# acg-team/ProGraphMSA

Hardware: AMD Instinct MI355X
Metric: DP cell-updates/sec (GCUPS) + wall-clock on 256 seqs × 1000 aa, WAG (higher is better)
Workload: dtype f32

## Files before the change

### include/pgm_hip.h

```cpp
#ifndef PGM_HIP_H_
#define PGM_HIP_H_

#include <stdint.h>
#include <stddef.h>

#ifdef __cplusplus
extern "C" {
#endif

#define PGM_OK 0
#define PGM_ERR_INVALID 1
#define PGM_ERR_DEVICE 2
#define PGM_ERR_BACKTRACK 3
#define PGM_ERR_NOMEM 4

#define PGM_GAP 0xFFFFFFFFu


typedef struct pgm_graph {
    uint32_t n;
    uint32_t dim;
    const double *sites;
    const int32_t *e_rowptr;
    const uint32_t *e_col;
    const float *e_val;
    const int32_t *r_rowptr;
    const uint32_t *r_col;
    const uint32_t *r_units;
} pgm_graph;

typedef struct pgm_model {
    const double *M;
    const double *pi;
} pgm_model;

typedef struct pgm_scores {
    float gap_init, gap_extend, match_init, end_match, end_gap, end_skip;
    float start_gap, start_init, repeat_init, repeat_ext;
} pgm_scores;

typedef struct pgm_align_out {
    float score;
    uint32_t n_tr_indels;
    uint32_t len;
    int32_t status;
    uint32_t *map1;
    uint32_t *map2;
} pgm_align_out;

typedef struct pgm_ctx pgm_ctx;
typedef struct pgm_align_batch pgm_align_batch;

int pgm_device_count(void);
int pgm_ctx_create(int device, pgm_ctx **out);
void pgm_ctx_destroy(pgm_ctx *ctx);
const char *pgm_last_error(void);
int pgm_ctx_device_info(pgm_ctx *ctx, char *name, size_t name_len, int *cu_count);

int pgm_align_graphs_batch(pgm_ctx *ctx, uint32_t njobs, const pgm_graph *const *g1,
                           const pgm_graph *const *g2, const pgm_model *const *model,
                           const pgm_scores *scores, pgm_align_out *out);

int pgm_align_batch_create(pgm_ctx *ctx, uint32_t njobs, const pgm_graph *const *g1,
                           const pgm_graph *const *g2, const pgm_model *const *model,
                           const pgm_scores *scores, pgm_align_batch **out);
#define PGM_BATCH_KEEP_MATRICES 1u
int pgm_align_batch_create_ex(pgm_ctx *ctx, uint32_t njobs, const pgm_graph *const *g1,
                              const pgm_graph *const *g2, const pgm_model *const *model,
                              const pgm_scores *scores, uint32_t flags, pgm_align_batch **out);
typedef struct pgm_site_ref {
    const double *dev_sites;
    const uint32_t *node_map;
    uint32_t ncols;
} pgm_site_ref;
int pgm_align_batch_create_res(pgm_ctx *ctx, uint32_t njobs, const pgm_graph *const *g1,
                               const pgm_graph *const *g2, const pgm_model *const *model,
                               const pgm_scores *scores, uint32_t flags, const pgm_site_ref *res1,
                               const pgm_site_ref *res2, pgm_align_batch **out);
int pgm_align_graphs_batch_res(pgm_ctx *ctx, uint32_t njobs, const pgm_graph *const *g1,
                               const pgm_graph *const *g2, const pgm_model *const *model,
                               const pgm_scores *scores, const pgm_site_ref *res1,
                               const pgm_site_ref *res2, pgm_align_out *out);
int pgm_align_batch_run(pgm_ctx *ctx, pgm_align_batch *b);
int pgm_align_batch_fetch(pgm_ctx *ctx, pgm_align_batch *b, pgm_align_out *out);
void pgm_align_batch_destroy(pgm_ctx *ctx, pgm_align_batch *b);
uint64_t pgm_align_batch_cells(const pgm_align_batch *b);
int pgm_align_batch_time(pgm_ctx *ctx, pgm_align_batch *b, int reps, float *ms_prep,
                         float *ms_emission, float *ms_fill, float *ms_traceback);
int pgm_align_batch_stage_times(pgm_align_batch *b, int reset, float *ms_prep, float *ms_emission, float *ms_fill,
                                uint32_t *launches);
int pgm_align_batch_job_times(pgm_ctx *ctx, pgm_align_batch *b, uint64_t *ticks);
int pgm_align_batch_test_stall(pgm_align_batch *b, uint32_t job, uint32_t band, uint32_t spin_limit);
int pgm_test_cu_shares(uint32_t cus, double lean_cost, uint32_t nlean, double band_cost, uint32_t nbands, double rest_cost,
                       uint32_t nrest, uint32_t ncrit, double longest_chain, uint32_t *out4);
#define PGM_PLAN_HEAD 23
#define PGM_PLAN_DHEAD 9
#define PGM_PLAN_JOB 19
int pgm_test_batch_plan(uint32_t njobs, const pgm_graph *const *g1, const pgm_graph *const *g2, const pgm_model *const *model,
                        const pgm_scores *scores, uint32_t flags, const pgm_site_ref *res1, const pgm_site_ref *res2, uint32_t cus,
                        uint32_t *head, double *dhead, uint32_t *job_fields, uint32_t *items, uint32_t *bands, uint32_t *lean_list, int32_t *tblist);
int pgm_align_batch_read_matrices(pgm_ctx *ctx, pgm_align_batch *b, uint32_t job, float *M,
                                  float *X, float *Y, float *W, float *S);

int pgm_nw_pairs_batch(pgm_ctx *ctx, uint32_t dim, const int32_t *score, int32_t gap_open,
                       int32_t gap_extend, uint32_t nseq, const int8_t *syms,
                       const uint32_t *offs, uint32_t npairs, const uint32_t *pi,
                       const uint32_t *pj, int32_t *counts, uint32_t *gaps);
#define PGM_NW_REDUCED 1u
int pgm_nw_pairs_submit(pgm_ctx *ctx, uint32_t dim, const int32_t *score, int32_t gap_open,
                        int32_t gap_extend, uint32_t nseq, const int8_t *syms,
                        const uint32_t *offs, uint32_t npairs, const uint32_t *pi,
                        const uint32_t *pj, uint32_t flags, int32_t *counts, uint32_t *gaps, int *ticket);
int pgm_nw_pairs_wait(pgm_ctx *ctx, int ticket);
float pgm_nw_last_kernel_ms(pgm_ctx *ctx);
void *pgm_host_alloc(size_t bytes);
void pgm_host_free(void *p);

int pgm_csprofile_load(pgm_ctx *ctx, uint32_t K, uint32_t ncols, const double *lprofiles,
                       const double *centre, const double *priors);
int pgm_csprofile_create_batch(pgm_ctx *ctx, uint32_t nseq, const int8_t *syms,
                               const uint32_t *offs, const double *tau, const double *pi,
                               const double *p_uniform, double *out, const uint64_t *out_offs);
int pgm_csprofile_create_batch_res(pgm_ctx *ctx, uint32_t nseq, const int8_t *syms,
                                   const uint32_t *offs, const double *tau, const double *pi,
                                   const double *p_uniform, const double **dev);
float pgm_csprofile_last_kernel_ms(pgm_ctx *ctx);

typedef struct pgm_mldist_model {
    uint32_t dim;
    const double *Q, *V, *Vi, *sigma;
    double dist_max, var_max, var_min, cutoff_dist, min_dist, max_dist, indel_rate;
    int32_t mldist, mldist_gap;
} pgm_mldist_model;
int pgm_mldist_batch(pgm_ctx *ctx, const pgm_mldist_model *model, uint32_t npairs, const int32_t *counts,
                     const uint32_t *gaps, const double *seqlen, double *dist, double *var);

int pgm_prealigned_counts_batch(pgm_ctx *ctx, uint32_t dim, uint32_t nrows, uint32_t ncols, const int8_t *rows,
                                uint32_t npairs, const uint32_t *pi, const uint32_t *pj, int32_t *counts,
                                uint32_t *gaps);
int pgm_kmer_cosine(pgm_ctx *ctx, uint32_t nseq, uint32_t ncols, const int32_t *counts, double *cosine);
int pgm_kmer_cosine_multi(pgm_ctx *ctx, uint32_t nfam, const uint32_t *nseq, uint32_t ncols, const int32_t *counts, double *cosine);
int pgm_prealigned_counts_multi(pgm_ctx *ctx, uint32_t dim, uint32_t nfam, const uint32_t *nrows, const uint32_t *ncols,
                                const int8_t *rows, uint32_t npairs, const uint32_t *fam, const uint32_t *pi, const uint32_t *pj,
                                int32_t *counts, uint32_t *gaps);
int pgm_prealigned_counts_resampled(pgm_ctx *ctx, uint32_t dim, uint32_t nrows, uint32_t ncols, const int8_t *rows, uint32_t nrep,
                                    const uint32_t *cols, uint32_t npairs, const uint32_t *pi, const uint32_t *pj, int32_t *counts,
                                    uint32_t *gaps);
float pgm_dist_last_kernel_ms(pgm_ctx *ctx);

typedef struct pgm_merge_job {
    uint32_t dim, n1, n2, nnodes;
    const double *sites1, *sites2;
    const double *P1, *P2;
    const uint32_t *k1, *k2;
    const uint8_t *g2_with_P1;
    double *profiles;
} pgm_merge_job;
int pgm_merge_profiles_batch(pgm_ctx *ctx, uint32_t njobs, const pgm_merge_job *jobs);
#define PGM_MERGE_RESIDENT 1u
int pgm_merge_profiles_batch_ex(pgm_ctx *ctx, uint32_t njobs, const pgm_merge_job *jobs, uint32_t flags,
                                const double **dev_profiles);
int pgm_resident_reset(pgm_ctx *ctx);
int pgm_resident_onehot(pgm_ctx *ctx, uint32_t dim, uint32_t nseq, const int8_t *syms, const uint32_t *offs,
                        const double **dev);
int pgm_resident_import(pgm_ctx *ctx, pgm_ctx *src_ctx, const double *src, uint64_t count, const double **dst);
float pgm_merge_last_kernel_ms(pgm_ctx *ctx);


typedef struct pgm_gapmask_job {
    const uint64_t *src;
    const uint32_t *mapping;
    uint64_t *dst;
    uint32_t nrows, ncols_in, ncols_out;
} pgm_gapmask_job;
int pgm_gapmask_extend_batch(pgm_ctx *ctx, uint32_t njobs, const pgm_gapmask_job *jobs);

typedef struct pgm_parsimony_job {
    const uint64_t *masks;
    const uint32_t *children;
    uint32_t nleaves, ncols;
} pgm_parsimony_job;
int pgm_gap_parsimony_batch(pgm_ctx *ctx, uint32_t njobs, const pgm_parsimony_job *jobs, uint32_t *scores);
float pgm_parsimony_last_kernel_ms(pgm_ctx *ctx);

#define PGM_WLS_MAX_N 32768
int pgm_wls_load(pgm_ctx *ctx, uint32_t n, const double *D, const double *W);

#define PGM_WLS_OUT 20
typedef struct pgm_wls_job {
    const int8_t *label;
    const double *offset;
    uint32_t nsub;
} pgm_wls_job;
int pgm_wls_pair_sums_batch(pgm_ctx *ctx, uint32_t njobs, const pgm_wls_job *jobs, double *out);
float pgm_wls_last_kernel_ms(pgm_ctx *ctx);
uint32_t pgm_wls_last_launches(pgm_ctx *ctx);

typedef struct pgm_bionj_join { uint32_t index1, index2; double dist1, dist2; } pgm_bionj_join;
#define PGM_BIONJ_MAX_N 32768
int pgm_bionj(pgm_ctx *ctx, uint32_t n, const double *D, const double *V, pgm_bionj_join *joins, double *final_d);
int pgm_bionj_multi(pgm_ctx *ctx, uint32_t nfam, const uint32_t *n, const double *D, const double *V,
                    pgm_bionj_join *joins, double *final_d);
uint32_t pgm_bionj_last_launches(pgm_ctx *ctx);
float pgm_bionj_last_kernel_ms(pgm_ctx *ctx);

typedef struct pgm_bionj_pair { uint32_t index1, index2; } pgm_bionj_pair;
int pgm_bionj_plan(pgm_ctx *ctx, uint32_t n, const double *D, const double *V, const pgm_bionj_pair *plan,
                   pgm_bionj_join *joins, double *final_d);
int pgm_bionj_plan_multi(pgm_ctx *ctx, uint32_t nfam, const uint32_t *n, const double *D, const double *V,
                         const pgm_bionj_pair *plan, pgm_bionj_join *joins, double *final_d);

int pgm_msa_agreement(pgm_ctx *ctx, uint32_t nrows, uint32_t ncols, uint32_t nrep, const int32_t *where,
                      uint32_t *res_hits , uint32_t *pair_hits );
float pgm_agreement_last_kernel_ms(pgm_ctx *ctx);

int pgm_transfer_min(pgm_ctx *ctx, uint32_t nleaves, uint32_t nref, const uint64_t *ref ,
                     uint32_t nrep, const uint32_t *rep_off ,
                     const uint64_t *rep , uint32_t *phi );
float pgm_transfer_last_kernel_ms(pgm_ctx *ctx);

#define PGM_TRANSFER_NONE 0xffffffffu
int pgm_transfer_taxa(pgm_ctx *ctx, uint32_t nleaves, uint32_t nref, const uint64_t *ref , const uint32_t *thr ,
                      uint32_t nrep, const uint32_t *rep_off , const uint64_t *rep ,
                      uint32_t *phi , uint32_t *arg , uint32_t *moved ,
                      uint32_t *counted );

#define PGM_TREELIK_CHUNK 16
int pgm_tree_likelihood(pgm_ctx *ctx, uint32_t dim, uint32_t nleaves, uint32_t nnodes, const uint32_t *parent ,
                        uint32_t ncols, const int8_t *rows , const double *pi ,
                        const double *P , int derivs,
                        double *site_l , int32_t *site_k , double *d1, double *d2 );
float pgm_treelik_last_kernel_ms(pgm_ctx *ctx);

#define PGM_TREELIK_MAXCAT 16
int pgm_tree_likelihood_rates(pgm_ctx *ctx, uint32_t dim, uint32_t nleaves, uint32_t nnodes, const uint32_t *parent, uint32_t ncols, const int8_t *rows,
                              const double *pi, uint32_t ncat, const double *w , const double *P ,
                              int derivs, double *site_l , int32_t *site_k , double *post ,
                              double *d1, double *d2 );

int pgm_tree_ancestral(pgm_ctx *ctx, uint32_t dim, uint32_t nleaves, uint32_t nnodes, const uint32_t *parent, uint32_t ncols, const int8_t *rows,
                       const double *pi, uint32_t ncat, const double *w , const double *P ,
                       double *site_l , int32_t *site_k , double *post ,
                       int8_t *anc_state , double *anc_prob ,
                       double *anc_post );
// ... 38 lines not shown
```

### prographmsa_amd/__init__.py

```python
import ctypes as C
import os

_HERE = os.path.dirname(os.path.abspath(__file__))
LIB_PATH = os.path.join(_HERE, "lib", "libpgm_hip.so")
PGMSA_PATH = os.path.join(_HERE, "bin", "pgmsa")

PGM_OK, PGM_ERR_INVALID, PGM_ERR_DEVICE, PGM_ERR_BACKTRACK, PGM_ERR_NOMEM = 0, 1, 2, 3, 4
PGM_GAP = 0xFFFFFFFF
PGM_BATCH_KEEP_MATRICES = 1
PGM_NW_REDUCED = 1
PGM_MERGE_RESIDENT = 1


class pgm_graph(C.Structure):
    _fields_ = [("n", C.c_uint32), ("dim", C.c_uint32), ("sites", C.POINTER(C.c_double)),
                ("e_rowptr", C.POINTER(C.c_int32)), ("e_col", C.POINTER(C.c_uint32)), ("e_val", C.POINTER(C.c_float)),
                ("r_rowptr", C.POINTER(C.c_int32)), ("r_col", C.POINTER(C.c_uint32)), ("r_units", C.POINTER(C.c_uint32))]


class pgm_model(C.Structure):
    _fields_ = [("M", C.POINTER(C.c_double)), ("pi", C.POINTER(C.c_double))]


class pgm_scores(C.Structure):
    _fields_ = [(n, C.c_float) for n in ("gap_init", "gap_extend", "match_init", "end_match", "end_gap", "end_skip",
                                         "start_gap", "start_init", "repeat_init", "repeat_ext")]


class pgm_mldist_model(C.Structure):
    _fields_ = [("dim", C.c_uint32), ("Q", C.POINTER(C.c_double)), ("V", C.POINTER(C.c_double)), ("Vi", C.POINTER(C.c_double)),
                ("sigma", C.POINTER(C.c_double))] + [(n, C.c_double) for n in ("dist_max", "var_max", "var_min", "cutoff_dist", "min_dist", "max_dist", "indel_rate")] \
        + [("mldist", C.c_int32), ("mldist_gap", C.c_int32)]


class pgm_merge_job(C.Structure):
    _fields_ = [("dim", C.c_uint32), ("n1", C.c_uint32), ("n2", C.c_uint32), ("nnodes", C.c_uint32),
                ("sites1", C.POINTER(C.c_double)), ("sites2", C.POINTER(C.c_double)), ("P1", C.POINTER(C.c_double)), ("P2", C.POINTER(C.c_double)),
                ("k1", C.POINTER(C.c_uint32)), ("k2", C.POINTER(C.c_uint32)), ("g2_with_P1", C.POINTER(C.c_uint8)), ("profiles", C.POINTER(C.c_double))]


class pgm_site_ref(C.Structure):
    _fields_ = [("dev_sites", C.POINTER(C.c_double)), ("node_map", C.POINTER(C.c_uint32)), ("ncols", C.c_uint32)]


class pgm_gapmask_job(C.Structure):
    _fields_ = [("src", C.POINTER(C.c_uint64)), ("mapping", C.POINTER(C.c_uint32)), ("dst", C.POINTER(C.c_uint64)),
                ("nrows", C.c_uint32), ("ncols_in", C.c_uint32), ("ncols_out", C.c_uint32)]


class pgm_parsimony_job(C.Structure):
    _fields_ = [("masks", C.POINTER(C.c_uint64)), ("children", C.POINTER(C.c_uint32)), ("nleaves", C.c_uint32), ("ncols", C.c_uint32)]


class pgm_wls_job(C.Structure):
    _fields_ = [("label", C.POINTER(C.c_int8)), ("offset", C.POINTER(C.c_double)), ("nsub", C.c_uint32)]


class pgm_bionj_join(C.Structure):
    _fields_ = [("index1", C.c_uint32), ("index2", C.c_uint32), ("dist1", C.c_double), ("dist2", C.c_double)]


class pgm_bionj_pair(C.Structure):
    _fields_ = [("index1", C.c_uint32), ("index2", C.c_uint32)]


class pgm_align_out(C.Structure):
    _fields_ = [("score", C.c_float), ("n_tr_indels", C.c_uint32), ("len", C.c_uint32), ("status", C.c_int32),
                ("map1", C.POINTER(C.c_uint32)), ("map2", C.POINTER(C.c_uint32))]


EXPORTS = [
    "pgm_device_count", "pgm_ctx_create", "pgm_ctx_destroy", "pgm_last_error", "pgm_ctx_device_info",
    "pgm_align_graphs_batch", "pgm_align_batch_create", "pgm_align_batch_create_ex", "pgm_align_batch_create_res", "pgm_align_graphs_batch_res", "pgm_align_batch_run", "pgm_align_batch_fetch",
    "pgm_align_batch_destroy", "pgm_align_batch_cells", "pgm_align_batch_test_stall", "pgm_test_cu_shares", "pgm_test_batch_plan", "pgm_align_batch_stage_times", "pgm_align_batch_job_times", "pgm_align_batch_time", "pgm_align_batch_read_matrices",
    "pgm_nw_pairs_batch", "pgm_nw_pairs_submit", "pgm_nw_pairs_wait", "pgm_nw_last_kernel_ms", "pgm_host_alloc", "pgm_host_free", "pgm_csprofile_load", "pgm_csprofile_create_batch", "pgm_csprofile_create_batch_res",
    "pgm_csprofile_last_kernel_ms", "pgm_mldist_batch", "pgm_prealigned_counts_batch", "pgm_kmer_cosine", "pgm_dist_last_kernel_ms",
    "pgm_kmer_cosine_multi", "pgm_prealigned_counts_multi", "pgm_prealigned_counts_resampled",
    "pgm_merge_profiles_batch", "pgm_merge_profiles_batch_ex", "pgm_resident_reset", "pgm_resident_onehot", "pgm_resident_import", "pgm_merge_last_kernel_ms",
    "pgm_gapmask_extend_batch", "pgm_gap_parsimony_batch", "pgm_parsimony_last_kernel_ms",
    "pgm_wls_load", "pgm_wls_pair_sums_batch", "pgm_wls_last_kernel_ms", "pgm_wls_last_launches",
    "pgm_bionj", "pgm_bionj_multi", "pgm_bionj_last_launches", "pgm_bionj_last_kernel_ms",
    "pgm_bionj_plan", "pgm_bionj_plan_multi",
    "pgm_msa_agreement", "pgm_agreement_last_kernel_ms",
    "pgm_transfer_min", "pgm_transfer_last_kernel_ms", "pgm_transfer_taxa",
    "pgm_tree_likelihood", "pgm_treelik_last_kernel_ms", "pgm_tree_likelihood_rates", "pgm_tree_ancestral", "pgm_tree_nni", "pgm_tree_nni_edge", "pgm_tree_spr",
    "pgm_tree_ancestral_joint", "pgm_tree_ancestral_sample",
    "pgm_resampled_sums", "pgm_resample_last_kernel_ms",
]


def _load():
    if not os.path.exists(LIB_PATH):
        raise ImportError("libpgm_hip.so is not built (%s); run `python -c 'import __graft_entry__ as g; g.build()'` "
                          "— there is no CPU fallback for the hot path" % LIB_PATH)
    lib = C.CDLL(LIB_PATH)
    vp, u32, i32 = C.c_void_p, C.c_uint32, C.c_int32
    PG, PM = C.POINTER(C.POINTER(pgm_graph)), C.POINTER(C.POINTER(pgm_model))
    sig = {
        "pgm_device_count": (C.c_int, []),
        "pgm_ctx_create": (C.c_int, [C.c_int, C.POINTER(vp)]),
        "pgm_ctx_destroy": (None, [vp]),
        "pgm_last_error": (C.c_char_p, []),
        "pgm_ctx_device_info": (C.c_int, [vp, C.c_char_p, C.c_size_t, C.POINTER(C.c_int)]),
        "pgm_align_graphs_batch": (C.c_int, [vp, u32, PG, PG, PM, C.POINTER(pgm_scores), C.POINTER(pgm_align_out)]),
        "pgm_align_batch_create": (C.c_int, [vp, u32, PG, PG, PM, C.POINTER(pgm_scores), C.POINTER(vp)]),
        "pgm_align_batch_create_ex": (C.c_int, [vp, u32, PG, PG, PM, C.POINTER(pgm_scores), u32, C.POINTER(vp)]),
        "pgm_align_batch_create_res": (C.c_int, [vp, u32, PG, PG, PM, C.POINTER(pgm_scores), u32, C.POINTER(pgm_site_ref), C.POINTER(pgm_site_ref), C.POINTER(vp)]),
        "pgm_align_graphs_batch_res": (C.c_int, [vp, u32, PG, PG, PM, C.POINTER(pgm_scores), C.POINTER(pgm_site_ref), C.POINTER(pgm_site_ref), C.POINTER(pgm_align_out)]),
        "pgm_align_batch_run": (C.c_int, [vp, vp]),
        "pgm_align_batch_fetch": (C.c_int, [vp, vp, C.POINTER(pgm_align_out)]),
        "pgm_align_batch_destroy": (None, [vp, vp]),
        "pgm_align_batch_cells": (C.c_uint64, [vp]),
        "pgm_align_batch_test_stall": (C.c_int, [vp, u32, u32, u32]),
        "pgm_test_cu_shares": (C.c_int, [u32, C.c_double, u32, C.c_double, u32, C.c_double, u32, u32, C.c_double, C.POINTER(C.c_uint32)]),
        "pgm_test_batch_plan": (C.c_int, [u32, PG, PG, PM, C.POINTER(pgm_scores), u32, C.POINTER(pgm_site_ref), C.POINTER(pgm_site_ref), u32,
                                          C.POINTER(u32), C.POINTER(C.c_double)] + [C.POINTER(u32)] * 4 + [C.POINTER(i32)]),
        "pgm_align_batch_stage_times": (C.c_int, [vp, C.c_int] + [C.POINTER(C.c_float)] * 3 + [C.POINTER(u32)]),
        "pgm_align_batch_job_times": (C.c_int, [vp, vp, C.POINTER(C.c_uint64)]),
        "pgm_align_batch_time": (C.c_int, [vp, vp, C.c_int] + [C.POINTER(C.c_float)] * 4),
        "pgm_align_batch_read_matrices": (C.c_int, [vp, vp, u32] + [C.POINTER(C.c_float)] * 5),
        "pgm_nw_pairs_batch": (C.c_int, [vp, u32, C.POINTER(i32), i32, i32, u32, C.POINTER(C.c_int8), C.POINTER(u32), u32,
                                         C.POINTER(u32), C.POINTER(u32), C.POINTER(i32), C.POINTER(u32)]),
        "pgm_nw_pairs_submit": (C.c_int, [vp, u32, C.POINTER(i32), i32, i32, u32, C.POINTER(C.c_int8), C.POINTER(u32), u32,
                                          C.POINTER(u32), C.POINTER(u32), u32, C.POINTER(i32), C.POINTER(u32), C.POINTER(C.c_int)]),
        "pgm_nw_pairs_wait": (C.c_int, [vp, C.c_int]),
        "pgm_host_alloc": (vp, [C.c_size_t]),
        "pgm_host_free": (None, [vp]),
        "pgm_nw_last_kernel_ms": (C.c_float, [vp]),
        "pgm_csprofile_load": (C.c_int, [vp, u32, u32] + [C.POINTER(C.c_double)] * 3),
        "pgm_csprofile_create_batch": (C.c_int, [vp, u32, C.POINTER(C.c_int8), C.POINTER(u32)] + [C.POINTER(C.c_double)] * 4
                                       + [C.POINTER(C.c_uint64)]),
        "pgm_csprofile_create_batch_res": (C.c_int, [vp, u32, C.POINTER(C.c_int8), C.POINTER(u32)] + [C.POINTER(C.c_double)] * 3
                                           + [C.POINTER(C.POINTER(C.c_double))]),
        "pgm_csprofile_last_kernel_ms": (C.c_float, [vp]),
        "pgm_mldist_batch": (C.c_int, [vp, C.POINTER(pgm_mldist_model), u32, C.POINTER(i32), C.POINTER(u32)] + [C.POINTER(C.c_double)] * 3),
        "pgm_prealigned_counts_batch": (C.c_int, [vp, u32, u32, u32, C.POINTER(C.c_int8), u32, C.POINTER(u32), C.POINTER(u32), C.POINTER(i32), C.POINTER(u32)]),
        "pgm_kmer_cosine": (C.c_int, [vp, u32, u32, C.POINTER(i32), C.POINTER(C.c_double)]),
        "pgm_dist_last_kernel_ms": (C.c_float, [vp]),
        "pgm_kmer_cosine_multi": (C.c_int, [vp, u32, C.POINTER(u32), u32, C.POINTER(i32), C.POINTER(C.c_double)]),
        "pgm_prealigned_counts_multi": (C.c_int, [vp, u32, u32, C.POINTER(u32), C.POINTER(u32), C.POINTER(C.c_int8), u32, C.POINTER(u32), C.POINTER(u32),
                                                  C.POINTER(u32), C.POINTER(i32), C.POINTER(u32)]),
        "pgm_prealigned_counts_resampled": (C.c_int, [vp, u32, u32, u32, C.POINTER(C.c_int8), u32, C.POINTER(u32), u32, C.POINTER(u32), C.POINTER(u32),
                                                      C.POINTER(i32), C.POINTER(u32)]),
        "pgm_merge_profiles_batch": (C.c_int, [vp, u32, C.POINTER(pgm_merge_job)]),
        "pgm_merge_profiles_batch_ex": (C.c_int, [vp, u32, C.POINTER(pgm_merge_job), u32, C.POINTER(C.POINTER(C.c_double))]),
        "pgm_resident_reset": (C.c_int, [vp]),
        "pgm_resident_onehot": (C.c_int, [vp, u32, u32, C.POINTER(C.c_int8), C.POINTER(u32), C.POINTER(C.POINTER(C.c_double))]),
        "pgm_resident_import": (C.c_int, [vp, vp, C.POINTER(C.c_double), C.c_uint64, C.POINTER(C.POINTER(C.c_double))]),
        "pgm_merge_last_kernel_ms": (C.c_float, [vp]),
        "pgm_gapmask_extend_batch": (C.c_int, [vp, u32, C.POINTER(pgm_gapmask_job)]),
        "pgm_gap_parsimony_batch": (C.c_int, [vp, u32, C.POINTER(pgm_parsimony_job), C.POINTER(u32)]),
        "pgm_parsimony_last_kernel_ms": (C.c_float, [vp]),
        "pgm_wls_load": (C.c_int, [vp, u32, C.POINTER(C.c_double), C.POINTER(C.c_double)]),
        "pgm_wls_pair_sums_batch": (C.c_int, [vp, u32, C.POINTER(pgm_wls_job), C.POINTER(C.c_double)]),
        "pgm_wls_last_kernel_ms": (C.c_float, [vp]),
        "pgm_wls_last_launches": (C.c_uint32, [vp]),
        "pgm_bionj": (C.c_int, [vp, u32, C.POINTER(C.c_double), C.POINTER(C.c_double), C.POINTER(pgm_bionj_join), C.POINTER(C.c_double)]),
        "pgm_bionj_multi": (C.c_int, [vp, u32, C.POINTER(u32), C.POINTER(C.c_double), C.POINTER(C.c_double), C.POINTER(pgm_bionj_join), C.POINTER(C.c_double)]),
        "pgm_bionj_last_launches": (C.c_uint32, [vp]),
        "pgm_bionj_last_kernel_ms": (C.c_float, [vp]),
        "pgm_bionj_plan": (C.c_int, [vp, u32, C.POINTER(C.c_double), C.POINTER(C.c_double), C.POINTER(pgm_bionj_pair), C.POINTER(pgm_bionj_join), C.POINTER(C.c_double)]),
        "pgm_bionj_plan_multi": (C.c_int, [vp, u32, C.POINTER(u32), C.POINTER(C.c_double), C.POINTER(C.c_double), C.POINTER(pgm_bionj_pair), C.POINTER(pgm_bionj_join), C.POINTER(C.c_double)]),
        "pgm_msa_agreement": (C.c_int, [vp, u32, u32, u32, C.POINTER(i32), C.POINTER(u32), C.POINTER(u32)]),
        "pgm_agreement_last_kernel_ms": (C.c_float, [vp]),
        "pgm_transfer_min": (C.c_int, [vp, u32, u32, C.POINTER(C.c_uint64), u32, C.POINTER(u32), C.POINTER(C.c_uint64), C.POINTER(u32)]),
        "pgm_transfer_last_kernel_ms": (C.c_float, [vp]),
        "pgm_transfer_taxa": (C.c_int, [vp, u32, u32, C.POINTER(C.c_uint64), C.POINTER(u32), u32, C.POINTER(u32), C.POINTER(C.c_uint64),
                                        C.POINTER(u32), C.POINTER(u32), C.POINTER(u32), C.POINTER(u32)]),
        "pgm_tree_likelihood": (C.c_int, [vp, u32, u32, u32, C.POINTER(u32), u32, C.POINTER(C.c_int8), C.POINTER(C.c_double), C.POINTER(C.c_double), C.c_int,
                                          C.POINTER(C.c_double), C.POINTER(i32), C.POINTER(C.c_double), C.POINTER(C.c_double)]),
        "pgm_treelik_last_kernel_ms": (C.c_float, [vp]),
        "pgm_tree_likelihood_rates": (C.c_int, [vp, u32, u32, u32, C.POINTER(u32), u32, C.POINTER(C.c_int8), C.POINTER(C.c_double), u32, C.POINTER(C.c_double),
                                                C.POINTER(C.c_double), C.c_int, C.POINTER(C.c_double), C.POINTER(i32), C.POINTER(C.c_double), C.POINTER(C.c_double),
                                                C.POINTER(C.c_double)]),
        "pgm_tree_ancestral": (C.c_int, [vp, u32, u32, u32, C.POINTER(u32), u32, C.POINTER(C.c_int8), C.POINTER(C.c_double), u32, C.POINTER(C.c_double),
                                         C.POINTER(C.c_double), C.POINTER(C.c_double), C.POINTER(i32), C.POINTER(C.c_double), C.POINTER(C.c_int8),
                                         C.POINTER(C.c_double), C.POINTER(C.c_double)]),
        "pgm_tree_nni": (C.c_int, [vp, u32, u32, u32, C.POINTER(u32), u32, C.POINTER(C.c_int8), C.POINTER(C.c_double), u32, C.POINTER(C.c_double),
                                   C.POINTER(C.c_double), u32, C.POINTER(u32), C.POINTER(u32), C.POINTER(u32), C.POINTER(C.c_double), C.POINTER(i32),
                                   C.POINTER(C.c_double), C.POINTER(C.c_double)]),
        "pgm_tree_nni_edge": (C.c_int, [vp, u32, u32, u32, C.POINTER(u32), u32, C.POINTER(C.c_int8), C.POINTER(C.c_double), u32, C.POINTER(C.c_double),
                                        C.POINTER(C.c_double), u32, C.POINTER(u32), C.POINTER(u32), C.POINTER(u32), C.POINTER(C.c_double), C.POINTER(C.c_double),
                                        C.POINTER(i32), C.POINTER(C.c_double), C.POINTER(C.c_double), C.POINTER(C.c_double), C.POINTER(C.c_double)]),
        "pgm_tree_spr": (C.c_int, [vp, u32, u32, u32, C.POINTER(u32), u32, C.POINTER(C.c_int8), C.POINTER(C.c_double), u32, C.POINTER(C.c_double),
                                   C.POINTER(C.c_double), C.POINTER(C.c_double), u32, C.POINTER(u32), C.POINTER(u32), C.POINTER(C.c_double), C.POINTER(i32),
                                   C.POINTER(C.c_double), C.POINTER(C.c_double)]),
        "pgm_tree_ancestral_joint": (C.c_int, [vp, u32, u32, u32, C.POINTER(u32), u32, C.POINTER(C.c_int8), C.POINTER(C.c_double), u32, C.POINTER(C.c_double),
                                               C.POINTER(C.c_double), C.POINTER(C.c_double), C.POINTER(i32), C.POINTER(C.c_double), C.POINTER(C.c_uint8),
                                               C.POINTER(C.c_int8), C.POINTER(C.c_double), C.POINTER(i32)]),
        "pgm_tree_ancestral_sample": (C.c_int, [vp, u32, u32, u32, C.POINTER(u32), u32, C.POINTER(C.c_int8), C.POINTER(C.c_double), u32, C.POINTER(C.c_double),
                                                C.POINTER(C.c_double), u32, C.c_uint64, C.c_uint64, C.POINTER(C.c_double), C.POINTER(i32), C.POINTER(C.c_double),
                                                C.POINTER(C.c_uint8), C.POINTER(C.c_int8)]),
        "pgm_resampled_sums": (C.c_int, [vp, u32, u32, C.POINTER(C.c_double), u32, C.POINTER(u32), C.POINTER(C.c_double)]),
        "pgm_resample_last_kernel_ms": (C.c_float, [vp]),
    }
    for name, (res, args) in sig.items():
        fn = getattr(lib, name)
        fn.restype = res
        fn.argtypes = args
    return lib


lib = _load()


class PgmError(RuntimeError):
    pass


def check(rc, what="libpgm_hip"):
    if rc != PGM_OK:
        raise PgmError("%s failed (%d): %s" % (what, rc, lib.pgm_last_error().decode()))


class Context:

    def __init__(self, device=0):
        self.handle = C.c_void_p()
        check(lib.pgm_ctx_create(device, C.byref(self.handle)), "pgm_ctx_create")

    def device_info(self):
        buf = C.create_string_buffer(256)
        cu = C.c_int()
        check(lib.pgm_ctx_device_info(self.handle, buf, 256, C.byref(cu)))
        return buf.value.decode(), cu.value

    def prealigned_counts_resampled(self, dim, rows, cols, pi, pj):
        import numpy as np
        rows = np.ascontiguousarray(rows, np.int8)
        cols = np.ascontiguousarray(cols, np.uint32)
        pi = np.ascontiguousarray(pi, np.uint32)
        pj = np.ascontiguousarray(pj, np.uint32)
        nrep, npairs = cols.shape[0], len(pi)
        counts = np.zeros((nrep, npairs, dim * dim), np.int32)
        gaps = np.zeros((nrep, npairs), np.uint32)
        P = lambda a, t: a.ctypes.data_as(C.POINTER(t))
        check(lib.pgm_prealigned_counts_resampled(self.handle, dim, rows.shape[0], rows.shape[1], P(rows, C.c_int8), nrep, P(cols, C.c_uint32), npairs,
                                                  P(pi, C.c_uint32), P(pj, C.c_uint32), P(counts, C.c_int32), P(gaps, C.c_uint32)), "pgm_prealigned_counts_resampled")
        return counts, gaps

    def msa_agreement(self, where, res_hits=None, pair_hits=None):
        import numpy as np
        where = np.ascontiguousarray(where, np.int32)
        nrep, nrows, ncols = where.shape
        if res_hits is None: res_hits = np.zeros((nrows, ncols), np.uint32)
        if pair_hits is None: pair_hits = np.zeros((nrows, nrows), np.uint32)
        for o, shape in ((res_hits, (nrows, ncols)), (pair_hits, (nrows, nrows))):
            if o.dtype != np.uint32 or o.shape != shape or not o.flags.c_contiguous: raise ValueError("msa_agreement: output array of the wrong kind")
        P = lambda a, t: a.ctypes.data_as(C.POINTER(t))
        check(lib.pgm_msa_agreement(self.handle, nrows, ncols, nrep, P(where, C.c_int32), P(res_hits, C.c_uint32), P(pair_hits, C.c_uint32)), "pgm_msa_agreement")
        return res_hits, pair_hits

    def transfer_min(self, nleaves, ref, rep_off, rep, phi=None):
        import numpy as np
        words = (nleaves + 63) // 64
        ref = np.ascontiguousarray(ref, np.uint64)
        rep_off = np.ascontiguousarray(rep_off, np.uint32)
        rep = np.ascontiguousarray(rep, np.uint64).reshape(-1, words)
        if ref.ndim != 2 or ref.shape[1] != words or rep_off.ndim != 1 or len(rep_off) < 1 or rep.shape[0] != int(rep_off[-1]):
            raise ValueError("transfer_min: input array of the wrong shape")
        nref, nrep = ref.shape[0], len(rep_off) - 1
        if phi is None: phi = np.zeros((nref, nrep), np.uint32)
        if phi.dtype != np.uint32 or phi.shape != (nref, nrep) or not phi.flags.c_contiguous: raise ValueError("transfer_min: output array of the wrong kind")
        P = lambda a, t: a.ctypes.data_as(C.POINTER(t))
        check(lib.pgm_transfer_min(self.handle, nleaves, nref, P(ref, C.c_uint64), nrep, P(rep_off, C.c_uint32), P(rep, C.c_uint64) if rep.size else None,
                                   P(phi, C.c_uint32)), "pgm_transfer_min")
        return phi

    def transfer_taxa(self, nleaves, ref, thr, rep_off, rep, out=None):
        import numpy as np
        words = (nleaves + 63) // 64
# ... 219 lines not shown
```

### prographmsa_amd/csrc/pgm_align_kernels.h

```cpp
#ifndef PGM_ALIGN_KERNELS_H_
#define PGM_ALIGN_KERNELS_H_

#include <hip/hip_runtime.h>
#include <math.h>
#include <type_traits>
#include "pgm_device.h"

#define PGM_NEG_INF (-INFINITY)

__device__ __forceinline__ float pgm_ls_log_add(float x, float add) {
    const float a = 2.44247459618085927548717403238913328776812604856113966238617812902399112761292613763080658235564f;
    const float b = -4.2040783745848554315883301529007786406310628696382695994938550046831869207082846248658671f;
    const float c = -0.72123729809042963774358701619456664388406302428056983119308906451199556380646306f;
    const uint32_t bits = __float_as_uint(x);
    const float e = (float)((int32_t)(bits >> 23) - 126);
    const float d = __uint_as_float(((bits << 9) >> 9) ^ 0x3f000000u);
    float t = __fdiv_rn(b, __fsub_rn(d, c));
    const float u = __fadd_rn(e, a);
    t = __fadd_rn(t, add);
    t = __fadd_rn(t, u);
    return t;
}

__device__ __forceinline__ float pgm_emission_finish(float num, float ay, float bx, float match_init) {
// ... 248 lines not shown
    }
    for (int i = threadIdx.x; i < COLS; i += 4 * PGM_ROWS) {
        const int col = cbase + i;
        bq[i] = (col >= 0 && col <= (int)J.ncol) ? J.b2[col] : 0.f;
    }
    __syncthreads();
    const uint32_t b0 = (4u * blockIdx.y + threadIdx.x / PGM_ROWS) * RB;
    const int l = PGM_HALO + (int)(threadIdx.x % PGM_ROWS);
    if (b0 >= nvb) return;
    float gy[RB][DP], ay[RB];
#pragma unroll
    for (int r = 0; r < RB; ++r) {
        const uint32_t y = row_of(b0 + (uint32_t)r, (uint32_t)(l - PGM_HALO));
        const uint32_t yc = (y + 1 < J.n1) ? y : 0u;
        const float4 *src = (const float4 *)(J.g1f + (size_t)DP * yc);
#pragma unroll
        for (int q = 0; q < NT; ++q) {
            const float4 v = src[q];
            gy[r][4 * q] = v.x; gy[r][4 * q + 1] = v.y; gy[r][4 * q + 2] = v.z; gy[r][4 * q + 3] = v.w;
        }
        ay[r] = J.a1[yc];
    }
    const float mi = J.sc.match_init;
    const uint32_t nblk = J.nblk;
    PGM_GLOBAL pgm_v4f *const Sq = (PGM_GLOBAL pgm_v4f *)(uintptr_t)J.S;
#pragma unroll 1
    for (int w = 0; w < PGM_EM_TB; ++w) {
        const uint32_t tb = tb0 + w;
        if (tb >= nblk) break;
        float out[RB][PGM_BLOCK];
#pragma unroll
        for (int i = 0; i < PGM_BLOCK; i += 2) {
            const int ci = (int)(tb * PGM_BLOCK) + i - l - cbase;
            const pgm_v2f *tc = tp + ci * STR;
            pgm_v2f acc[RB];
#pragma unroll
            for (int r = 0; r < RB; ++r) acc[r] = pgm_v2f{0.0f, 0.0f};
#pragma unroll
            for (int k = 0; k < DP; ++k) {
                const pgm_v2f tk = tc[k];
#pragma unroll
                for (int r = 0; r < RB; ++r) {
                    const pgm_v2f g = {gy[r][k], gy[r][k]};
                    acc[r] = acc[r] + g * tk;
                }
            }
#pragma unroll
            for (int r = 0; r < RB; ++r) {
                out[r][i] = pgm_emission_finish(acc[r].x, ay[r], bq[ci], mi);
                out[r][i + 1] = pgm_emission_finish(acc[r].y, ay[r], bq[ci + 1], mi);
            }
        }
#pragma unroll
        for (int r = 0; r < RB; ++r) {
            if (b0 + (uint32_t)r < nvb) {
                PGM_GLOBAL pgm_v4f *dst = Sq + (sblock_of(b0 + (uint32_t)r, tb) * 64u + (uint32_t)l) * (PGM_BLOCK / 4);
#pragma unroll
                for (int q = 0; q < PGM_BLOCK / 4; ++q) dst[q] = pgm_v4f{out[r][4 * q], out[r][4 * q + 1], out[r][4 * q + 2], out[r][4 * q + 3]};
            }
        }
    }
}

__device__ __forceinline__ int pgm_wave_max8(uint32_t v) {
    int m = __builtin_amdgcn_ballot_w64(v >= 8u) != 0 ? 8 : 0;
    m += __builtin_amdgcn_ballot_w64(v >= (uint32_t)(m + 4)) != 0 ? 4 : 0;
    m += __builtin_amdgcn_ballot_w64(v >= (uint32_t)(m + 2)) != 0 ? 2 : 0;
    m += __builtin_amdgcn_ballot_w64(v >= (uint32_t)(m + 1)) != 0 ? 1 : 0;
    return m;
}

__device__ __forceinline__ __amdgpu_buffer_rsrc_t pgm_band_rsrc(float4 *base, uint32_t bytes) {
    const uint64_t p = (uint64_t)base;
    const uint32_t lo = __builtin_amdgcn_readfirstlane((uint32_t)p), hi = __builtin_amdgcn_readfirstlane((uint32_t)(p >> 32));
    return __builtin_amdgcn_make_buffer_rsrc((void *)(((uint64_t)hi << 32) | lo), 0, __builtin_amdgcn_readfirstlane(bytes), 0x00020000);
}
__device__ __forceinline__ void pgm_store_cell_masked(__amdgpu_buffer_rsrc_t rsrc, uint32_t t, int lane, bool on, float Mv, float Xv, float Wv, float Yv) {
    typedef uint32_t pgm_v4u __attribute__((ext_vector_type(4)));
    pgm_v4u v;
    v.x = __float_as_uint(Mv); v.y = __float_as_uint(Xv); v.z = __float_as_uint(Wv); v.w = __float_as_uint(Yv);
    __builtin_amdgcn_raw_buffer_store_b128(v, rsrc, (on ? (uint32_t)lane * 16u : 0x80000000u) + t * 1024u, 0, 16);
}
__device__ __forceinline__ float4 pgm_gload4(const float4 *p) {
    const pgm_v4f v = *(const PGM_GLOBAL pgm_v4f *)(uintptr_t)p;
    return make_float4(v.x, v.y, v.z, v.w);
}
__device__ __forceinline__ float2 pgm_gload_cell_wy(const float4 *p) {
    const unsigned long long v = __hip_atomic_load((const PGM_GLOBAL unsigned long long *)(uintptr_t)p + 1, __ATOMIC_RELAXED, __HIP_MEMORY_SCOPE_AGENT);
    return make_float2(__uint_as_float((uint32_t)v), __uint_as_float((uint32_t)(v >> 32)));
}
__device__ __forceinline__ float2 pgm_load_cell_mx(const float4 *p) {
    const unsigned long long v = __hip_atomic_load((const PGM_GLOBAL unsigned long long *)(uintptr_t)p, __ATOMIC_RELAXED, __HIP_MEMORY_SCOPE_AGENT);
    return make_float2(__uint_as_float((uint32_t)v), __uint_as_float((uint32_t)(v >> 32)));
}
__device__ __forceinline__ float2 pgm_load_cell_wy(const float4 *p) {
    const unsigned long long v = __hip_atomic_load((const PGM_GLOBAL unsigned long long *)(uintptr_t)p + 1, __ATOMIC_RELAXED, __HIP_MEMORY_SCOPE_AGENT);
    return make_float2(__uint_as_float((uint32_t)v), __uint_as_float((uint32_t)(v >> 32)));
}

struct PgmPred {
    const int32_t *pp; const uint32_t *pc; const float *pv; const uint32_t *pu;
};
__device__ __forceinline__ float pgm_mark_value(const PgmPred &P, int32_t e) {
    const uint32_t u = P.pu[e];
    if (u == 0) return P.pv[e];
    const uint32_t units = u & 0x7fffffffu;
    if (units == 0) return INFINITY;
    return __fadd_rn(INFINITY, __fmul_rn(INFINITY, (float)(units - 1)));
}

struct PgmMapOut {
    uint32_t *m1, *m2;
    uint32_t len, cap;
    __device__ __forceinline__ void push(uint32_t y, uint32_t x) {
        if (len < cap) { m1[len] = y; m2[len] = x; }
        ++len;
    }
};

__device__ static void pgm_mark_alternative_path(const PgmJob &J, uint32_t start, uint32_t end, const PgmPred &P, PgmMapOut &mo, bool first) {
    const uint32_t len = end - start + 1;
    float *score = J.mark_score;
    uint32_t *prev = J.mark_prev;
    for (uint32_t i = 0; i < len; ++i) { score[i] = PGM_NEG_INF; prev[i] = 0xFFFFFFFFu; }
    score[0] = 0.0f;
    for (uint32_t i = 1; i < len; ++i) {
        const uint32_t real_ix = i + start;
        for (int32_t e = P.pp[real_ix]; e < P.pp[real_ix + 1]; ++e) {
            const uint32_t p = P.pc[e];
            if (p >= start && p <= end) {
                const uint32_t i2 = p - start;
                const float cand = __fsub_rn(score[i2], pgm_mark_value(P, e));
                if (score[i] <= cand) { score[i] = cand; prev[i] = i2; }
            }
        }
    }
    if (score[len - 1] > PGM_NEG_INF) {
        uint32_t i = prev[len - 1];
        while (i != 0) {
            if (first) mo.push(i + start, 0xFFFFFFFFu); else mo.push(0xFFFFFFFFu, i + start);
            i = prev[i];
        }
    }
}

__device__ __forceinline__ float pgm_emission_at(const PgmJob &J, uint32_t y, uint32_t x) {
    const uint32_t b = y / PGM_ROWS, l = PGM_HALO + (y - b * PGM_ROWS), t = x + l;
    return J.S[(((size_t)b * J.nblk + (t / PGM_BLOCK)) * 64u + l) * PGM_BLOCK + (t % PGM_BLOCK)];
}

#define PGM_TB_T 32
#define PGM_TB_BAND 6
#define PGM_TB_LK 4
struct PgmTbLds {
    float4 cell[PGM_TB_T * PGM_TB_T];
    float S[PGM_TB_T * PGM_TB_T];
    uint32_t p_cnt[2 * PGM_TB_T];
    uint32_t p_c[2 * PGM_TB_T * PGM_TB_PK];
    float p_v[2 * PGM_TB_T * PGM_TB_PK];
    uint32_t p_u[2 * PGM_TB_T * PGM_TB_PK];
    uint16_t succ[3 * PGM_TB_T * PGM_TB_T];
    uint32_t ty0, tx0;
    uint32_t ay, ax;
    int req;
    uint32_t len;
    int nbig;
    uint16_t big[128];
    uint16_t gtab[PGM_LK_NR][PGM_LK_W * PGM_LK_TAB] __attribute__((aligned(16)));
    uint2 mbuf[64];
    uint32_t grow, gcnt;
    uint32_t gnext[PGM_LK_NR];
};

#define PGM_LK_HW (PGM_LK_T + PGM_LK_H)
struct PgmLkLds {
    float4 cell[PGM_LK_HW * PGM_LK_HW];
    float S[PGM_LK_T * PGM_LK_T];
    uint32_t p_cnt[2 * PGM_LK_T];
    uint32_t p_c[2 * PGM_LK_T * PGM_TB_PK];
    float p_v[2 * PGM_LK_T * PGM_TB_PK];
    uint32_t p_u[2 * PGM_LK_T * PGM_TB_PK];
    uint16_t tab[PGM_LK_TAB] __attribute__((aligned(16)));
    int nbig;
    uint16_t big[PGM_LK_T * PGM_LK_T];
};
__device__ __forceinline__ uint16_t pgm_lk_code(uint32_t st, uint32_t dy, uint32_t dx) { return (uint16_t)(0x8000u | (st << 12) | (dy << 6) | dx); }

struct PgmPredView {
    uint32_t cnt;
    bool lds;
    uint32_t base;
};

__device__ static void pgm_traceback_publish(const PgmJob &J, const uint32_t len, const int tid, const int nthreads) {
    for (uint32_t i = (uint32_t)tid; i < len; i += (uint32_t)nthreads) {
        const uint32_t j = len - 1 - i;
        J.hmap1[i] = J.map1[j];
        J.hmap2[i] = J.map2[j];
    }
    __threadfence_system();
    __syncthreads();
    if (tid == 0) {
        const PgmJob::Result r = *J.result;
        J.hresult->score = r.score; J.hresult->n_tr_indels = r.n_tr_indels; J.hresult->len = r.len;
        __threadfence_system();
        __hip_atomic_store(&J.hresult->status, r.status, __ATOMIC_RELEASE, __HIP_MEMORY_SCOPE_SYSTEM);
    }
}

__device__ __attribute__((noinline)) static void pgm_traceback_job(const PgmJob &J, PgmTbLds &T, const int tid, const int nthreads,
                                         int *lq, int *lq_ids, const uint32_t jid) {
    constexpr uint32_t TT = PGM_TB_T;
    const uint32_t n1 = J.n1, n2 = J.n2;

    const PgmPred P1 = {J.pp1, J.pc1, J.pv1, J.pu1};
    const PgmPred P2 = {J.pp2, J.pc2, J.pv2, J.pu2};

    const bool loader = tid >= 64;
    auto stage = [&]() {
        const uint32_t ty0 = T.ty0, tx0 = T.tx0;
        constexpr uint32_t NT = 64u * PGM_WAVES;
        constexpr int NC = (int)((TT * TT) / NT), NP = (int)((2 * TT * PGM_TB_PK) / NT);
        static_assert(NC * NT == TT * TT && NP * NT == 2 * TT * PGM_TB_PK, "tile staging: whole rounds of the workgroup");
        float4 cv[NC];
        float sv[NC];
        uint32_t cslot[NC];
#pragma unroll
        for (int u = 0; u < NC; ++u) {
            const uint32_t i = (uint32_t)tid + NT * u;
            const uint32_t half = TT * (TT + 1u) / 2u;
            const bool up = i < half;
            const uint32_t m = up ? i : TT * TT - 1u - i;
            uint32_t d = (uint32_t)((sqrtf(8.0f * (float)m + 1.0f) - 1.0f) * 0.5f);
            while (d * (d + 1u) / 2u > m) --d;
            while ((d + 1u) * (d + 2u) / 2u <= m) ++d;
            const uint32_t k = m - d * (d + 1u) / 2u;
            const uint32_t ly = up ? k : TT - 1u - k, lx = up ? d - k : TT - 1u - (d - k);
            cslot[u] = ly * TT + lx;
            const uint32_t yy = min(ty0 + ly, n1 - 2), xx = min(tx0 + lx, n2 - 2);
            cv[u] = J.cells[pgm_cell_index(J, yy, xx)];
            const uint32_t ys = min(ty0 + i / TT, n1 - 2), xs = min(tx0 + i % TT, n2 - 2);
            sv[u] = pgm_emission_at(J, ys, xs);
        }
        uint32_t cnt[NP], ec[NP], eu[NP];
        float ev[NP];
#pragma unroll
        for (int u = 0; u < NP; ++u) {
            const uint32_t i = (uint32_t)tid + NT * u, slot = i / PGM_TB_PK, k = i % PGM_TB_PK;
            const bool row = slot < TT;
            const uint32_t v = min(row ? ty0 + slot : tx0 + (slot - TT), (row ? n1 : n2) - 1);
            const PgmTbNode *r = (row ? J.tb1 : J.tb2) + v;
            cnt[u] = r->cnt; ec[u] = r->c[k]; ev[u] = r->v[k]; eu[u] = r->u[k];
        }
#pragma unroll
        for (int u = 0; u < NC; ++u) {
            const uint32_t i = (uint32_t)tid + NT * u;
            T.cell[cslot[u]] = cv[u];
            T.S[i] = sv[u];
        }
        for (uint32_t i = (uint32_t)tid; i < 3u * TT * TT / 2u; i += NT) ((uint32_t *)T.succ)[i] = 0u;
        if (tid == 0) T.nbig = 0;
#pragma unroll
        for (int u = 0; u < NP; ++u) {
            const uint32_t i = (uint32_t)tid + NT * u, slot = i / PGM_TB_PK, k = i % PGM_TB_PK;
            const bool row = slot < TT;
            const bool inr = (row ? ty0 + slot : tx0 + (slot - TT)) < (row ? n1 : n2);
            if (k == 0) T.p_cnt[slot] = inr ? cnt[u] : 0xFFFFFFFFu;
            T.p_c[i] = ec[u]; T.p_v[i] = ev[u]; T.p_u[i] = eu[u];
        }
    };
    const pgm_scores sc = J.sc;
    const int band = J.has_extras ? PGM_TB_BAND : PGM_TB_BAND / 2;
    auto links = [&]() {
        const uint32_t ty0 = T.ty0, tx0 = T.tx0;
        const int adiag = (int)(T.ay - ty0) - (int)(T.ax - tx0);
        const uint32_t NDIAG = 2u * (uint32_t)band + 1u;
        for (uint32_t task = (uint32_t)tid; task < 3u * NDIAG * TT; task += (uint32_t)nthreads) {
            const uint32_t lx = task % TT, st_task = task / (NDIAG * TT);
            const int lyi = (int)lx + adiag + (int)((task / TT) % NDIAG) - band;
            if (lyi < 0 || lyi >= (int)TT) continue;
            const uint32_t ly = (uint32_t)lyi, ci = ly * TT + lx, y = ty0 + ly, x = tx0 + lx;
            uint16_t lm = 0, lxs = 0, lys = 0;
            if (y + 1 < n1 && x + 1 < n2 && (y | x) != 0u) {
                const float4 c0 = T.cell[ci];
                const uint32_t cy = T.p_cnt[ly], cx = T.p_cnt[TT + lx];
                auto pick = [&](const float4 &c, uint32_t yp, uint32_t xp) -> uint16_t {
                    uint32_t st;
                    if ((yp | xp) == 0u) st = 0u;
                    else if (c.z == c.x) st = 0u;
                    else if (c.z == c.w) st = 2u;
                    else if (c.z == c.y) st = 1u;
                    else return (uint16_t)0;
                    return (uint16_t)(0x8000u | (st << 10) | ((yp - ty0) << 5) | (xp - tx0));
                };
                const int doff = (int)((task / TT) % NDIAG) - band;
                if (st_task == 0u && doff >= -1 && doff <= 1 && (cy > PGM_TB_LK || cx > PGM_TB_LK) && cy <= PGM_TB_PK && cx <= PGM_TB_PK && cy != 0u && cx != 0u && c0.x > PGM_NEG_INF) {
                    const int slot = __hip_atomic_fetch_add(&T.nbig, 1, __ATOMIC_RELAXED, __HIP_MEMORY_SCOPE_WORKGROUP);
                    if (slot < 128) T.big[slot] = (uint16_t)ci;
                }
                if (st_task == 0u && cy <= PGM_TB_LK && cx <= PGM_TB_LK && cy != 0u && cx != 0u && c0.x > PGM_NEG_INF) {
                    const float S = T.S[ci];
                    uint32_t yp[PGM_TB_LK], xp[PGM_TB_LK];
                    float yv[PGM_TB_LK], xv[PGM_TB_LK];
                    bool ok = true;
#pragma unroll
                    for (int k = 0; k < PGM_TB_LK; ++k) {
                        yp[k] = T.p_c[ly * PGM_TB_PK + k]; yv[k] = T.p_v[ly * PGM_TB_PK + k];
                        xp[k] = T.p_c[(TT + lx) * PGM_TB_PK + k]; xv[k] = T.p_v[(TT + lx) * PGM_TB_PK + k];
                        ok = ok && ((uint32_t)k >= cy || yp[k] >= ty0) && ((uint32_t)k >= cx || xp[k] >= tx0);
                    }
                    float wz[PGM_TB_LK][PGM_TB_LK];
#pragma unroll
                    for (int ky = 0; ky < PGM_TB_LK; ++ky)
#pragma unroll
                        for (int kx = 0; kx < PGM_TB_LK; ++kx)
                            wz[ky][kx] = T.cell[min((yp[ky] - ty0) * TT + (xp[kx] - tx0), TT * TT - 1u)].z;
                    float best = INFINITY;
                    uint32_t wy = 0, wx = 0, wky = 0, wkx = 0;
#pragma unroll
                    for (int ky = 0; ky < PGM_TB_LK; ++ky)
#pragma unroll
                        for (int kx = 0; kx < PGM_TB_LK; ++kx) {
                            const float d = fabsf(__fsub_rn(c0.x, __fsub_rn(__fsub_rn(__fadd_rn(wz[ky][kx], S), yv[ky]), xv[kx])));
                            if ((uint32_t)ky < cy && (uint32_t)kx < cx && best > d) { best = d; wy = yp[ky]; wx = xp[kx]; wky = ky; wkx = kx; }
                        }
                    bool rep_edge = false;
                    float4 wc = c0;
                    if (ok && best < INFINITY) {
                        rep_edge = (T.p_u[ly * PGM_TB_PK + wky] | T.p_u[(TT + lx) * PGM_TB_PK + wkx]) != 0u;
                        wc = T.cell[(wy - ty0) * TT + (wx - tx0)];
                    }
                    if (ok && best < INFINITY && !rep_edge) lm = pick(wc, wy, wx);
                }
                if (st_task == 2u && cy == 1u && c0.w > PGM_NEG_INF) {
                    float best = INFINITY;
                    bool ok = true, rep_edge = false, open = false;
                    uint32_t wy = 0;
                    float4 wc = c0;
                    for (uint32_t k = 0; k < cy; ++k) {
                        const uint32_t yp = T.p_c[ly * PGM_TB_PK + k];
                        if (yp < ty0) { ok = false; break; }
                        const float yv = T.p_v[ly * PGM_TB_PK + k];
                        const float4 c = T.cell[(yp - ty0) * TT + lx];
                        const bool ru = T.p_u[ly * PGM_TB_PK + k] != 0u;
                        float d = fabsf(__fsub_rn(c0.w, __fsub_rn(__fadd_rn(c.w, sc.gap_extend), yv)));
                        if (best > d) { best = d; wy = yp; wc = c; rep_edge = ru; open = false; }
                        d = fabsf(__fsub_rn(c0.w, __fsub_rn(__fadd_rn(c.z, sc.gap_init), yv)));
                        if (best > d) { best = d; wy = yp; wc = c; rep_edge = ru; open = true; }
                    }
                    if (ok && best < INFINITY && !rep_edge)
                        lys = open ? pick(wc, wy, x) : (uint16_t)(0x8000u | (2u << 10) | ((wy - ty0) << 5) | lx);
                }
                if (st_task == 1u && cx == 1u && c0.y > PGM_NEG_INF) {
                    float best = INFINITY;
                    bool ok = true, rep_edge = false, open = false;
                    uint32_t wx = 0;
                    float4 wc = c0;
                    for (uint32_t k = 0; k < cx; ++k) {
                        const uint32_t xp = T.p_c[(TT + lx) * PGM_TB_PK + k];
                        if (xp < tx0) { ok = false; break; }
                        const float xv = T.p_v[(TT + lx) * PGM_TB_PK + k];
                        const float4 c = T.cell[ly * TT + (xp - tx0)];
                        const bool ru = T.p_u[(TT + lx) * PGM_TB_PK + k] != 0u;
                        float d = fabsf(__fsub_rn(c0.y, __fsub_rn(__fadd_rn(c.y, sc.gap_extend), xv)));
                        if (best > d) { best = d; wx = xp; wc = c; rep_edge = ru; open = false; }
                        d = fabsf(__fsub_rn(c0.y, __fsub_rn(__fadd_rn(c.z, sc.gap_init), xv)));
                        if (best > d) { best = d; wx = xp; wc = c; rep_edge = ru; open = true; }
                    }
                    if (ok && best < INFINITY && !rep_edge)
                        lxs = open ? pick(wc, y, wx) : (uint16_t)(0x8000u | (1u << 10) | (ly << 5) | (wx - tx0));
                }
            }
            T.succ[st_task * (TT * TT) + ci] = st_task == 0u ? lm : (st_task == 1u ? lxs : lys);
        }
    };
    auto links_big = [&]() {
        const int wave = tid >> 6, lane_b = tid & 63, nwaves = nthreads >> 6;
        const uint32_t ty0 = T.ty0, tx0 = T.tx0;
        const int nbig = min(T.nbig, 128);
        for (int i = wave; i < nbig; i += nwaves) {
            const uint32_t ci = T.big[i], ly = ci / TT, lx = ci % TT;
            const uint32_t cy = T.p_cnt[ly], cx = T.p_cnt[TT + lx];
            const uint32_t ky = (uint32_t)lane_b >> 3, kx = (uint32_t)lane_b & 7u;
            const bool valid = ky < cy && kx < cx;
            const uint32_t yp = T.p_c[ly * PGM_TB_PK + ky], xp = T.p_c[(TT + lx) * PGM_TB_PK + kx];
            const float yv = T.p_v[ly * PGM_TB_PK + ky], xv = T.p_v[(TT + lx) * PGM_TB_PK + kx];
            const uint32_t rep = T.p_u[ly * PGM_TB_PK + ky] | T.p_u[(TT + lx) * PGM_TB_PK + kx];
            const bool inside = yp >= ty0 && xp >= tx0;
            if (__builtin_amdgcn_ballot_w64(valid && !inside) != 0ull) continue;
            const float4 c0 = T.cell[ci];
            const float S = T.S[ci];
            const float4 c = T.cell[(valid && inside) ? (yp - ty0) * TT + (xp - tx0) : ci];
            const float d = fabsf(__fsub_rn(c0.x, __fsub_rn(__fsub_rn(__fadd_rn(c.z, S), yv), xv)));
            const unsigned long long zero = __builtin_amdgcn_ballot_w64(valid && d == 0.0f);
            if (zero == 0ull) continue;
            const int win = __ffsll((long long)zero) - 1;
            if (lane_b == win && rep == 0u) {
                uint32_t st = 3u;
                if ((yp | xp) == 0u) st = 0u;
                else if (c.z == c.x) st = 0u;
                else if (c.z == c.w) st = 2u;
                else if (c.z == c.y) st = 1u;
                if (st != 3u) T.succ[ci] = (uint16_t)(0x8000u | (st << 10) | ((yp - ty0) << 5) | (xp - tx0));
            }
        }
    };
    const bool use_links = true;
    auto load_rows = [&]() {
        const uint32_t gy = T.grow, cnt = T.gcnt;
        constexpr uint32_t NW = PGM_LK_W * PGM_LK_TAB * 2u / 8u, NT = 64u * PGM_WAVES, PER = NW / NT;
        static_assert(NW % NT == 0u, "row table: whole rounds of the workgroup");
        unsigned long long v[PGM_LK_NR][PER];
#pragma unroll
        for (uint32_t r = 0; r < PGM_LK_NR; ++r) {
            const PGM_GLOBAL unsigned long long *src = (const PGM_GLOBAL unsigned long long *)(uintptr_t)(J.ltab + (size_t)(gy - min(r, cnt - 1u)) * (PGM_LK_W * PGM_LK_TAB));
#pragma unroll
            for (uint32_t q = 0; q < PER; ++q) v[r][q] = r < cnt ? __hip_atomic_load(src + (uint32_t)tid + NT * q, __ATOMIC_RELAXED, __HIP_MEMORY_SCOPE_AGENT) : 0ull;
        }
        uint32_t nx = 0u;
        const uint32_t k = (uint32_t)tid - 64u;
        if (k < PGM_LK_NR && gy >= cnt + k) nx = (uint32_t)__hip_atomic_load(J.lready + (gy - cnt - k), __ATOMIC_RELAXED, __HIP_MEMORY_SCOPE_AGENT) >= min(J.lcols, PGM_LK_W) ? 1u : 0u;
#pragma unroll
        for (uint32_t r = 0; r < PGM_LK_NR; ++r)
            if (r < cnt) {
#pragma unroll
                for (uint32_t q = 0; q < PER; ++q) ((unsigned long long *)T.gtab[(gy - r) % PGM_LK_NR])[(uint32_t)tid + NT * q] = v[r][q];
            }
        if (k < PGM_LK_NR) T.gnext[k] = nx;
    };
    if (tid == 0) {
        T.grow = 0xFFFFFFFFu; T.gcnt = 0u;
        if (J.lrows != 0u) __hip_atomic_store(J.lready + J.lrows + 1, (int)(J.lrows - 1u), __ATOMIC_RELAXED, __HIP_MEMORY_SCOPE_AGENT);
        T.ty0 = n1 - 2 >= TT - 1 ? n1 - 2 - (TT - 1) : 0u;
        T.tx0 = n2 - 2 >= TT - 1 ? n2 - 2 - (TT - 1) : 0u;
        T.ay = n1 - 2; T.ax = n2 - 2;
        T.req = 1;
        if (J.lrows != 0u && lq) {
            const int slot = __hip_atomic_fetch_add(lq, 1, __ATOMIC_RELAXED, __HIP_MEMORY_SCOPE_AGENT);
            __hip_atomic_store(lq_ids + slot, (int)(jid + 1u), __ATOMIC_RELEASE, __HIP_MEMORY_SCOPE_AGENT);
        }
    }
    __syncthreads();
    stage();
    __syncthreads();
    if (use_links) {
        links();
        __syncthreads();
        links_big();
        __syncthreads();
    }

    if (loader) {
        for (;;) {
            __syncthreads();
            if (T.req == 2) break;
            if (T.req == 3) { load_rows(); __syncthreads(); continue; }
            stage();
            __syncthreads();
            if (use_links) {
                links();
                __syncthreads();
                links_big();
                __syncthreads();
            }
        }
    } else {
        const int lane = tid;
        const pgm_scores s = J.sc;
        uint32_t ty0 = T.ty0, tx0 = T.tx0, ay = T.ay, ax = T.ax;
        int adiag = (int)(ay - ty0) - (int)(ax - tx0);
        auto in_tile = [&](uint32_t y, uint32_t x) { return (y - ty0) < TT && (x - tx0) < TT; };
        auto cell_at = [&](uint32_t y, uint32_t x) -> float4 {
            if (in_tile(y, x)) return T.cell[(y - ty0) * TT + (x - tx0)];
            return pgm_load_cell(J, y, x);
        };
        auto s_at = [&](uint32_t y, uint32_t x) -> float {
            if (in_tile(y, x)) return T.S[(y - ty0) * TT + (x - tx0)];
            return pgm_emission_at(J, y, x);
        };
        auto preds = [&](bool row, uint32_t v) -> PgmPredView {
            const uint32_t slot = row ? v - ty0 : (v - tx0) + TT;
            if ((row ? v - ty0 : v - tx0) < TT) {
                const uint32_t cnt = T.p_cnt[slot];
                if (cnt <= PGM_TB_PK) return PgmPredView{cnt, true, slot * PGM_TB_PK};
            }
            const PgmPred &P = row ? P1 : P2;
            const int32_t eb = P.pp[v];
            return PgmPredView{(uint32_t)(P.pp[v + 1] - eb), false, (uint32_t)eb};
        };
        auto pc_of = [&](bool row, const PgmPredView &V, uint32_t k) { return V.lds ? T.p_c[V.base + k] : (row ? P1 : P2).pc[V.base + k]; };
        auto pv_of = [&](bool row, const PgmPredView &V, uint32_t k) { return V.lds ? T.p_v[V.base + k] : (row ? P1 : P2).pv[V.base + k]; };
        auto pu_of = [&](bool row, const PgmPredView &V, uint32_t k) { return V.lds ? T.p_u[V.base + k] : (row ? P1 : P2).pu[V.base + k]; };

        int status = PGM_OK;
        uint32_t n_tr = 0;
        enum { State_m = 0, State_x = 1, State_y = 2 };
        int current_state = State_m;
        float current_score = PGM_NEG_INF, Wend = PGM_NEG_INF;
        uint32_t y = n1 - 1, x = n2 - 1;
        PgmMapOut mo = {J.map1, J.map2, 0u, n1 + n2};
        if (lane == 0) {
            const PgmPredView Ey = preds(true, n1 - 1), Ex = preds(false, n2 - 1);
            for (uint32_t ky = 0; ky < Ey.cnt; ++ky) {
                for (uint32_t kx = 0; kx < Ex.cnt; ++kx) {
                    const uint32_t yp = pc_of(true, Ey, ky), xp = pc_of(false, Ex, kx);
                    const float yv = pv_of(true, Ey, ky), xv = pv_of(false, Ex, kx);
                    if (xp == 0 && yp == 0) {
                        Wend = fmaxf(__fsub_rn(__fsub_rn(s.end_skip, yv), xv), Wend);
                    } else {
                        const float4 c = cell_at(yp, xp);
                        Wend = fmaxf(__fsub_rn(__fsub_rn(__fadd_rn(c.y, s.end_gap), yv), xv), Wend);
                        Wend = fmaxf(__fsub_rn(__fsub_rn(__fadd_rn(c.w, s.end_gap), yv), xv), Wend);
                        Wend = fmaxf(__fsub_rn(__fsub_rn(__fadd_rn(c.x, s.end_match), yv), xv), Wend);
                    }
                }
            }
            mo.push(n1 - 1, n2 - 1);
            bool tr_x = false, tr_y = false;
            float best = INFINITY;
            for (uint32_t ky = 0; ky < Ey.cnt; ++ky) {
                for (uint32_t kx = 0; kx < Ex.cnt; ++kx) {
                    const uint32_t yp = pc_of(true, Ey, ky), xp = pc_of(false, Ex, kx);
                    const float yv = pv_of(true, Ey, ky), xv = pv_of(false, Ex, kx);
                    const bool ry = pu_of(true, Ey, ky) != 0, rx = pu_of(false, Ex, kx) != 0;
                    const float4 c = cell_at(yp, xp);
                    float d = fabsf(__fsub_rn(Wend, __fsub_rn(__fsub_rn(__fadd_rn(c.x, s.end_match), yv), xv)));
                    if (best > d) { best = d; tr_x = rx; tr_y = ry; current_score = c.x; current_state = State_m; y = yp; x = xp; }
                    d = fabsf(__fsub_rn(Wend, __fsub_rn(__fsub_rn(__fadd_rn(c.w, s.end_gap), yv), xv)));
                    if (best > d) { best = d; tr_x = rx; tr_y = ry; current_score = c.w; current_state = State_y; y = yp; x = xp; }
                    d = fabsf(__fsub_rn(Wend, __fsub_rn(__fsub_rn(__fadd_rn(c.y, s.end_gap), yv), xv)));
                    if (best > d) { best = d; tr_x = rx; tr_y = ry; current_score = c.y; current_state = State_x; y = yp; x = xp; }
                    d = fabsf(__fsub_rn(Wend, __fsub_rn(__fsub_rn(s.end_skip, yv), xv)));
                    if (xp == 0 && yp == 0 && best > d) { best = d; tr_x = rx; tr_y = ry; y = yp; x = xp; }
                }
            }
            n_tr += (uint32_t)tr_x + (uint32_t)tr_y;
            if (tr_y) pgm_mark_alternative_path(J, y, n1 - 1, P1, mo, true);
            if (tr_x) pgm_mark_alternative_path(J, x, n2 - 1, P2, mo, false);
            if (x != 0 || y != 0) {
                if (current_state == State_m) mo.push(y, x);
                else if (current_state == State_x) mo.push(0xFFFFFFFFu, x);
                else mo.push(y, 0xFFFFFFFFu);
            }
        }
        y = __builtin_amdgcn_readfirstlane(y); x = __builtin_amdgcn_readfirstlane(x);
        current_state = __builtin_amdgcn_readfirstlane(current_state);
        current_score = __uint_as_float(__builtin_amdgcn_readfirstlane(__float_as_uint(current_score)));
        Wend = __uint_as_float(__builtin_amdgcn_readfirstlane(__float_as_uint(Wend)));
        n_tr = __builtin_amdgcn_readfirstlane(n_tr);
        mo.len = __builtin_amdgcn_readfirstlane(mo.len);

        auto rl_u = [](uint32_t v, int l) { return (uint32_t)__builtin_amdgcn_readlane((int)v, l); };
        auto rl_f = [](float v, int l) { return __uint_as_float((uint32_t)__builtin_amdgcn_readlane((int)__float_as_uint(v), l)); };
        uint32_t nbuf = 0;
        auto buf_flush = [&]() {
            if (nbuf != 0u) {
                if ((uint32_t)lane < nbuf && mo.len + (uint32_t)lane < mo.cap) { const uint2 v = T.mbuf[lane]; mo.m1[mo.len + (uint32_t)lane] = v.x; mo.m2[mo.len + (uint32_t)lane] = v.y; }
                mo.len += nbuf;
                nbuf = 0u;
            }
        };
        auto buf_push = [&](uint32_t a, uint32_t b2) {
            if (lane == 0) T.mbuf[nbuf] = make_uint2(a, b2);
            if (++nbuf == 64u) buf_flush();
        };
        const uint32_t margin = J.has_extras ? 4u : 1u;
        uint32_t guard = 0;
        bool score_stale = false;
        uint32_t nl_y = 0xFFFFFFFFu, nl_x = 0xFFFFFFFFu;
        uint32_t glo = 1u, ghi = 0u;
        uint32_t known = 0u;
        while ((x != 0 || y != 0) && status == PGM_OK) {
            if (++guard > n1 + n2 + 4) { status = PGM_ERR_BACKTRACK; break; }
            y = __builtin_amdgcn_readfirstlane(y); x = __builtin_amdgcn_readfirstlane(x);
            current_state = __builtin_amdgcn_readfirstlane(current_state);
            const int offb = ((int)(y - ty0) - (int)(x - tx0)) - adiag;
            const bool reload = ((y - ty0) >= TT || ((y - ty0) < margin && ty0 != 0)) || ((x - tx0) >= TT || ((x - tx0) < margin && tx0 != 0)) ||
                                (use_links && (offb < -band || offb > band) && (y != ay || x != ax));
            bool nolink = false;
            if (reload && J.lrows != 0u && !(y == nl_y && x == nl_x)) {
                bool moved = false;
                uint32_t st = (uint32_t)(current_state == State_m ? 0 : (current_state == State_x ? 1 : 2));
                const uint32_t gw = min(J.lcols, PGM_LK_W);
                for (;;) {
                    const uint32_t gy = y >> 5;
                    if (gy >= J.lrows) break;
                    const uint32_t first = pgm_lk_first(n1, n2, J.lcols, gy);
                    if ((x >> 5) - first >= gw) break;
                    if (!(gy >= glo && gy <= ghi)) {
                        const bool cont = gy + 1u == glo && known != 0u;
                        if (!cont) {
                            if ((uint32_t)__hip_atomic_load(J.lready + gy, __ATOMIC_RELAXED, __HIP_MEMORY_SCOPE_AGENT) < gw) break;
                            known = 1u;
                        }
                        const uint32_t cnt = min(min(known, (uint32_t)PGM_LK_NR), gy + 1u);
                        if (lane == 0) {
                            T.grow = gy; T.gcnt = cnt; T.req = 3;
                            __hip_atomic_store(J.lready + J.lrows + 1, (int)(gy >= cnt ? gy - cnt : 0u), __ATOMIC_RELAXED, __HIP_MEMORY_SCOPE_AGENT);
                        }
                        __syncthreads();
                        load_rows();
                        __syncthreads();
                        ghi = gy; glo = gy + 1u - cnt;
                        known = 0u;
                        while (known < (uint32_t)PGM_LK_NR && T.gnext[known] != 0u) ++known;
                    }
                    bool left_row = false;
                    const uint16_t *tab = T.gtab[gy % PGM_LK_NR];
                    for (;;) {
                        const uint32_t j = (x >> 5) - first;
                        if (j >= gw) break;
                        const uint32_t code = tab[j * PGM_LK_TAB + st * (TT * TT) + (y & 31u) * TT + (x & 31u)];
                        if (!(code & 0x8000u)) { nolink = true; break; }
                        y -= (code >> 6) & 63u; x -= code & 63u; st = (code >> 12) & 3u;
                        moved = true;
                        if ((y | x) == 0u) break;
                        buf_push(st == 1u ? 0xFFFFFFFFu : y, st == 2u ? 0xFFFFFFFFu : x);
                        if ((y >> 5) != gy) { left_row = true; break; }
                    }
                    y = __builtin_amdgcn_readfirstlane(y); x = __builtin_amdgcn_readfirstlane(x); st = __builtin_amdgcn_readfirstlane(st);
                    if (!left_row) break;
                }
                buf_flush();
                if (moved) {
                    current_state = st == 0u ? State_m : (st == 1u ? State_x : State_y);
                    score_stale = true;
                    continue;
                }
                nl_y = y; nl_x = x;
            }
            if (reload && !(nolink && y == nl_y && x == nl_x)) {
                ty0 = y >= TT - 1 ? y - (TT - 1) : 0u;
                tx0 = x >= TT - 1 ? x - (TT - 1) : 0u;
                ay = y; ax = x; adiag = (int)(y - ty0) - (int)(x - tx0);
                if (lane == 0) { T.ty0 = ty0; T.tx0 = tx0; T.ay = y; T.ax = x; T.req = 1; }
                __syncthreads();
                stage();
                __syncthreads();
                if (use_links) {
                    links();
                    __syncthreads();
                    links_big();
                    __syncthreads();
                }
            }
            if (in_tile(y, x)) {
                uint32_t pos = (uint32_t)(current_state == State_m ? 0 : (current_state == State_x ? 1 : 2)) * (TT * TT) + (y - ty0) * TT + (x - tx0);
                bool moved = false;
                for (;;) {
                    const uint32_t code = T.succ[pos];
                    if (!(code & 0x8000u)) break;
                    pos = code & 0xfffu;
                    moved = true;
                    const uint32_t ny = ty0 + ((pos >> 5) & 31u), nx = tx0 + (pos & 31u), st = pos >> 10;
                    if ((ny | nx) == 0u) break;
                    buf_push(st == 1u ? 0xFFFFFFFFu : ny, st == 2u ? 0xFFFFFFFFu : nx);
                }
                buf_flush();
                if (moved) {
                    y = ty0 + ((pos >> 5) & 31u); x = tx0 + (pos & 31u);
                    const uint32_t st = pos >> 10;
                    current_state = st == 0u ? State_m : (st == 1u ? State_x : State_y);
                    score_stale = true;
                    continue;
                }
            }
            if (in_tile(y, x)) {
                const uint32_t ly = y - ty0, lx = x - tx0, ci = ly * TT + lx;
                const uint32_t cy = T.p_cnt[ly], cx = T.p_cnt[TT + lx];
                const bool in_m = current_state == State_m, in_y = current_state == State_y;
                if ((in_m || in_y ? cy - 1u < (uint32_t)PGM_TB_PK : true) && (in_m || !in_y ? cx - 1u < (uint32_t)PGM_TB_PK : true)) {
                    const float4 c0 = T.cell[ci];
                    const float S0 = T.S[ci];
                    const uint32_t ka = in_m ? (uint32_t)lane >> 3 : (uint32_t)lane >> 1, kb = in_m ? (uint32_t)lane & 7u : (uint32_t)lane & 1u;
                    const bool valid = in_m ? (ka < cy && kb < cx) : (ka < (in_y ? cy : cx));
                    const uint32_t yi = ly * PGM_TB_PK + (ka & 7u), xi = (TT + lx) * PGM_TB_PK + ((in_m ? kb : ka) & 7u);
                    uint32_t yp = y, xp = x, uu = 0u;
                    float yv = 0.0f, xv = 0.0f;
                    if (in_m || in_y) { yp = T.p_c[yi]; yv = T.p_v[yi]; uu |= T.p_u[yi]; }
                    if (in_m || !in_y) { xp = T.p_c[xi]; xv = T.p_v[xi]; uu |= T.p_u[xi]; }
                    const bool inside = yp >= ty0 && xp >= tx0;
                    if (__builtin_amdgcn_ballot_w64(valid && !inside) == 0ull) {
                        const float4 c = T.cell[valid ? (yp - ty0) * TT + (xp - tx0) : ci];
                        float d;
                        if (in_m) d = fabsf(__fsub_rn(c0.x, __fsub_rn(__fsub_rn(__fadd_rn(c.z, S0), yv), xv)));
                        else if (in_y) d = fabsf(__fsub_rn(c0.w, __fsub_rn(__fadd_rn(kb == 0u ? c.w : c.z, kb == 0u ? s.gap_extend : s.gap_init), yv)));
                        else d = fabsf(__fsub_rn(c0.y, __fsub_rn(__fadd_rn(kb == 0u ? c.y : c.z, kb == 0u ? s.gap_extend : s.gap_init), xv)));
                        const unsigned long long zero = __builtin_amdgcn_ballot_w64(valid && d == 0.0f);
                        if (zero != 0ull) {
                            const int win = __ffsll((long long)zero) - 1;
                            const uint32_t w_yp = rl_u(yp, win), w_xp = rl_u(xp, win), w_rep = rl_u(uu, win), w_kind = rl_u(kb, win);
                            const float wz = rl_f(c.z, win), wm = rl_f(c.x, win), wx = rl_f(c.y, win), wy = rl_f(c.w, win);
                            int next_state = current_state;
                            bool ok = w_rep == 0u;
                            if ((in_m || w_kind == 1u) && (w_yp | w_xp) != 0u) {
                                if (wz == wm) next_state = State_m;
                                else if (wz == wy) next_state = State_y;
                                else if (wz == wx) next_state = State_x;
                                else ok = false;
                            }
                            if (ok) {
                                y = w_yp; x = w_xp;
                                current_state = next_state;
                                score_stale = true;
                                if (x != 0 || y != 0) {
                                    if (lane == 0 && mo.len < mo.cap) {
                                        mo.m1[mo.len] = current_state == State_x ? 0xFFFFFFFFu : y;
                                        mo.m2[mo.len] = current_state == State_y ? 0xFFFFFFFFu : x;
                                    }
                                    ++mo.len;
                                }
                                continue;
                            }
                        }
                    }
                }
            }
            if (score_stale) {
                const float4 c = cell_at(y, x);
                current_score = current_state == State_m ? c.x : (current_state == State_x ? c.y : c.w);
                score_stale = false;
            }
            const bool need_y = current_state != State_x, need_x = current_state != State_y;
            PgmPredView Vy = {1u, false, 0u}, Vx = {1u, false, 0u};
            if (need_y) Vy = preds(true, y);
            if (need_x) Vx = preds(false, x);
            const float S = (current_state == State_m) ? s_at(y, x) : 0.0f;
            const uint32_t per = (current_state == State_m) ? Vx.cnt : 2u;
            const bool small = Vy.cnt <= 8u && Vx.cnt <= 8u;
            const uint32_t total = (current_state == State_m) ? (small ? (Vy.cnt && Vx.cnt ? 64u : 0u) : Vy.cnt * Vx.cnt) : 2u * (need_y ? Vy.cnt : Vx.cnt);
            float best = INFINITY;
            uint32_t w_yp = 0xFFFFFFFFu, w_xp = 0xFFFFFFFFu, w_uy = 0, w_ux = 0, w_kind = 0;
            float4 w_c = make_float4(0.f, 0.f, 0.f, 0.f);
            bool found = false;
            for (uint32_t base = 0; base < total; base += 64u) {
                const uint32_t i = base + (uint32_t)lane;
                const bool valid = (current_state == State_m && small) ? (((uint32_t)lane >> 3) < Vy.cnt && ((uint32_t)lane & 7u) < Vx.cnt) : i < total;
                uint32_t ka, kb;
                if (current_state != State_m) { ka = i >> 1; kb = i & 1u; }
                else if (small) { ka = (uint32_t)lane >> 3; kb = (uint32_t)lane & 7u; }
                else { ka = valid ? i / per : 0u; kb = valid ? i % per : 0u; }
                uint32_t yp = y, xp = x, uy = 0, ux = 0;
                float yv = 0.0f, xv = 0.0f;
                if (need_y) { const uint32_t k = ka; if (valid) { yp = pc_of(true, Vy, k); yv = pv_of(true, Vy, k); uy = pu_of(true, Vy, k); } }
                if (need_x) { const uint32_t k = (current_state == State_m) ? kb : ka; if (valid) { xp = pc_of(false, Vx, k); xv = pv_of(false, Vx, k); ux = pu_of(false, Vx, k); } }
                float4 c = make_float4(0.f, 0.f, 0.f, 0.f);
                if (valid) c = cell_at(yp, xp);
                float d;
                if (current_state == State_m) d = fabsf(__fsub_rn(current_score, __fsub_rn(__fsub_rn(__fadd_rn(c.z, S), yv), xv)));
                else if (current_state == State_y) d = fabsf(__fsub_rn(current_score, __fsub_rn(__fadd_rn(kb == 0 ? c.w : c.z, kb == 0 ? s.gap_extend : s.gap_init), yv)));
                else d = fabsf(__fsub_rn(current_score, __fsub_rn(__fadd_rn(kb == 0 ? c.y : c.z, kb == 0 ? s.gap_extend : s.gap_init), xv)));
                if (!valid) d = INFINITY;
                int win = -1;
                const unsigned long long zero = __builtin_amdgcn_ballot_w64(valid && d == 0.0f);
                if (zero != 0ull) {
                    if (best > 0.0f) { win = __ffsll((long long)zero) - 1; best = 0.0f; }
                } else {
                    float m = best;
                    for (int l = 0; l < 64; ++l) { const float dl = rl_f(d, l); if (m > dl) { m = dl; win = l; } }
                    best = m;
                }
                if (win >= 0) {
                    found = true;
                    w_yp = rl_u(yp, win); w_xp = rl_u(xp, win); w_uy = rl_u(uy, win); w_ux = rl_u(ux, win); w_kind = rl_u(kb, win);
                    w_c = make_float4(rl_f(c.x, win), rl_f(c.y, win), rl_f(c.z, win), rl_f(c.w, win));
                }
                if (best == 0.0f) break;
            }
            if (!found) { status = PGM_ERR_BACKTRACK; break; }
            const uint32_t next_y = w_yp, next_x = w_xp;
            int next_state = current_state;
            float next_score = INFINITY;
            bool tr_x = false, tr_y = false;
            const bool from_w = (current_state == State_m) || w_kind == 1u;
            if (current_state != State_x) tr_y = w_uy != 0;
            if (current_state != State_y) tr_x = w_ux != 0;
            if (!from_w) {
                next_score = (current_state == State_y) ? w_c.w : w_c.y;
            } else if (next_x != 0 || next_y != 0) {
                if (w_c.z == w_c.x) { next_score = w_c.x; next_state = State_m; }
                else if (w_c.z == w_c.w) { next_score = w_c.w; next_state = State_y; }
                else if (w_c.z == w_c.y) { next_score = w_c.y; next_state = State_x; }
                else { status = PGM_ERR_BACKTRACK; break; }
            }
            n_tr += (uint32_t)tr_x + (uint32_t)tr_y;
            if (tr_y || tr_x) {
                if (lane == 0) {
                    if (tr_y) pgm_mark_alternative_path(J, next_y, y, P1, mo, true);
                    if (tr_x) pgm_mark_alternative_path(J, next_x, x, P2, mo, false);
                }
                mo.len = __builtin_amdgcn_readfirstlane(mo.len);
            }
            x = next_x; y = next_y;
            current_state = next_state;
            current_score = next_score;
            if (x != 0 || y != 0) {
                uint32_t py = y, px = x;
                if (current_state == State_x) py = 0xFFFFFFFFu;
                else if (current_state == State_y) px = 0xFFFFFFFFu;
                if (lane == 0 && mo.len < mo.cap) { mo.m1[mo.len] = py; mo.m2[mo.len] = px; }
                ++mo.len;
            }
        }
        if (lane == 0 && mo.len < mo.cap) { mo.m1[mo.len] = 0u; mo.m2[mo.len] = 0u; }
        ++mo.len;
        if (mo.len > mo.cap) { status = PGM_ERR_BACKTRACK; mo.len = mo.cap; }
        if (lane == 0) {
            J.result->score = Wend;
            J.result->n_tr_indels = n_tr;
            J.result->len = mo.len;
            J.result->status = status;
            T.len = mo.len;
            T.req = 2;
        }
        __syncthreads();
    }
    __threadfence_block();
    __syncthreads();
    pgm_traceback_publish(J, T.len, tid, nthreads);
    if (tid == 0 && lq) {
        if (J.lrows != 0u) __hip_atomic_store(J.lready + J.lrows, (int)(J.lrows * PGM_LK_W), __ATOMIC_RELAXED, __HIP_MEMORY_SCOPE_AGENT);
        __hip_atomic_fetch_add(lq + (PGM_SY_TB_DONE - PGM_SY_LQ_N), 1, __ATOMIC_RELEASE, __HIP_MEMORY_SCOPE_AGENT);
    }
}

__device__ __attribute__((noinline)) static void pgm_prelink_tile(const PgmJob &J, PgmLkLds &G, const uint32_t k, const int tid) {
    constexpr uint32_t TT = PGM_LK_T, HW = PGM_LK_HW, NT = 64u * PGM_WAVES, PK = PGM_TB_PK;
    const uint32_t n1 = J.n1, n2 = J.n2;
    const uint32_t w = min(J.lcols, PGM_LK_W), r = k / PGM_LK_W, jj = k % PGM_LK_W;
    if (jj >= w || r >= J.lrows) return;
    const uint32_t gx = pgm_lk_first(n1, n2, J.lcols, r) + jj;
    const uint32_t cy0 = TT * r, cx0 = TT * gx;
    const uint32_t hy0 = cy0 >= PGM_LK_H ? cy0 - PGM_LK_H : 0u, hx0 = cx0 >= PGM_LK_H ? cx0 - PGM_LK_H : 0u;
    const pgm_scores sc = J.sc;
    __builtin_amdgcn_fence(__ATOMIC_ACQUIRE, "agent");
    __syncthreads();
    {
        constexpr int NC = (int)((HW * HW + NT - 1) / NT);
        float4 cv[NC];
        uint32_t cslot[NC];
#pragma unroll
        for (int u = 0; u < NC; ++u) {
            const uint32_t i = min((uint32_t)tid + NT * u, HW * HW - 1u);
            const uint32_t half = HW * (HW + 1u) / 2u;
            const bool up = i < half;
            const uint32_t m = up ? i : HW * HW - 1u - i;
            uint32_t d = (uint32_t)((sqrtf(8.0f * (float)m + 1.0f) - 1.0f) * 0.5f);
            while (d * (d + 1u) / 2u > m) --d;
            while ((d + 1u) * (d + 2u) / 2u <= m) ++d;
            const uint32_t kk = m - d * (d + 1u) / 2u;
            const uint32_t ly = up ? kk : HW - 1u - kk, lx = up ? d - kk : HW - 1u - (d - kk);
            cslot[u] = ly * HW + lx;
            cv[u] = J.cells[pgm_cell_index(J, min(hy0 + ly, n1 - 2), min(hx0 + lx, n2 - 2))];
        }
        float sv[2];
#pragma unroll
        for (int u = 0; u < 2; ++u) {
            const uint32_t i = (uint32_t)tid + NT * u;
            sv[u] = pgm_emission_at(J, min(cy0 + i / TT, n1 - 2), min(cx0 + i % TT, n2 - 2));
        }
        const uint32_t slot = (uint32_t)tid / PK, kk = (uint32_t)tid % PK;
        const bool row = slot < TT;
        const uint32_t v = row ? cy0 + slot : cx0 + (slot - TT);
        const PgmTbNode *rec = (row ? J.tb1 : J.tb2) + min(v, (row ? n1 : n2) - 1);
        const uint32_t cnt = rec->cnt, ec = rec->c[kk], eu = rec->u[kk];
        const float ev = rec->v[kk];
#pragma unroll
        for (int u = 0; u < NC; ++u)
            if ((uint32_t)tid + NT * u < HW * HW) G.cell[cslot[u]] = cv[u];
#pragma unroll
        for (int u = 0; u < 2; ++u) G.S[(uint32_t)tid + NT * u] = sv[u];
        if (kk == 0) G.p_cnt[slot] = v < (row ? n1 : n2) ? cnt : 0xFFFFFFFFu;
        G.p_c[tid] = ec; G.p_v[tid] = ev; G.p_u[tid] = eu;
        if (tid == 0) G.nbig = 0;
    }
    __syncthreads();
    auto hc = [&](uint32_t yy, uint32_t xx) { return min((yy - hy0) * HW + (xx - hx0), HW * HW - 1u); };
    auto pick = [&](const float4 &c, uint32_t y, uint32_t x, uint32_t yp, uint32_t xp) -> uint16_t {
        uint32_t st;
        if ((yp | xp) == 0u) st = 0u;
        else if (c.z == c.x) st = 0u;
        else if (c.z == c.w) st = 2u;
        else if (c.z == c.y) st = 1u;
        else return (uint16_t)0;
        return pgm_lk_code(st, y - yp, x - xp);
    };
    for (uint32_t task = (uint32_t)tid; task < PGM_LK_TAB; task += NT) {
        const uint32_t st_task = task / (TT * TT), ci = task % (TT * TT), ly = ci / TT, lx = ci % TT, y = cy0 + ly, x = cx0 + lx;
        uint16_t link = 0;
        if (y + 1 < n1 && x + 1 < n2 && (y | x) != 0u) {
            const float4 c0 = G.cell[hc(y, x)];
            const uint32_t cy = G.p_cnt[ly], cx = G.p_cnt[TT + lx];
            if (st_task == 0u && cy - 1u < PK && cx - 1u < PK && c0.x > PGM_NEG_INF) {
                if (cy > PGM_TB_LK || cx > PGM_TB_LK) {
                    const int slot = __hip_atomic_fetch_add(&G.nbig, 1, __ATOMIC_RELAXED, __HIP_MEMORY_SCOPE_WORKGROUP);
                    G.big[slot] = (uint16_t)ci;
                } else {
                    const float S = G.S[ci];
                    uint32_t yp[PGM_TB_LK], xp[PGM_TB_LK];
                    float yv[PGM_TB_LK], xv[PGM_TB_LK];
                    bool ok = true;
#pragma unroll
                    for (int q = 0; q < PGM_TB_LK; ++q) {
                        yp[q] = G.p_c[ly * PK + q]; yv[q] = G.p_v[ly * PK + q];
                        xp[q] = G.p_c[(TT + lx) * PK + q]; xv[q] = G.p_v[(TT + lx) * PK + q];
                        ok = ok && ((uint32_t)q >= cy || yp[q] >= hy0) && ((uint32_t)q >= cx || xp[q] >= hx0);
                    }
                    float wz[PGM_TB_LK][PGM_TB_LK];
#pragma unroll
                    for (int ky = 0; ky < PGM_TB_LK; ++ky)
#pragma unroll
                        for (int kx = 0; kx < PGM_TB_LK; ++kx) wz[ky][kx] = G.cell[hc(yp[ky], xp[kx])].z;
                    float best = INFINITY;
                    uint32_t wy = 0, wx = 0, wky = 0, wkx = 0;
#pragma unroll
                    for (int ky = 0; ky < PGM_TB_LK; ++ky)
#pragma unroll
                        for (int kx = 0; kx < PGM_TB_LK; ++kx) {
                            const float d = fabsf(__fsub_rn(c0.x, __fsub_rn(__fsub_rn(__fadd_rn(wz[ky][kx], S), yv[ky]), xv[kx])));
                            if ((uint32_t)ky < cy && (uint32_t)kx < cx && best > d) { best = d; wy = yp[ky]; wx = xp[kx]; wky = ky; wkx = kx; }
                        }
                    if (ok && best < INFINITY && (G.p_u[ly * PK + wky] | G.p_u[(TT + lx) * PK + wkx]) == 0u) link = pick(G.cell[hc(wy, wx)], y, x, wy, wx);
                }
            }
            if (st_task == 2u && cy - 1u < PK && c0.w > PGM_NEG_INF) {
                float best = INFINITY;
                bool ok = true, rep_edge = false, open = false;
                uint32_t wy = 0;
                float4 wc = c0;
                for (uint32_t q = 0; q < cy; ++q) {
                    const uint32_t yp = G.p_c[ly * PK + q];
                    if (yp < hy0) { ok = false; break; }
                    const float yv = G.p_v[ly * PK + q];
                    const float4 c = G.cell[hc(yp, x)];
                    const bool ru = G.p_u[ly * PK + q] != 0u;
                    float d = fabsf(__fsub_rn(c0.w, __fsub_rn(__fadd_rn(c.w, sc.gap_extend), yv)));
                    if (best > d) { best = d; wy = yp; wc = c; rep_edge = ru; open = false; }
                    d = fabsf(__fsub_rn(c0.w, __fsub_rn(__fadd_rn(c.z, sc.gap_init), yv)));
                    if (best > d) { best = d; wy = yp; wc = c; rep_edge = ru; open = true; }
                }
                if (ok && best < INFINITY && !rep_edge) link = open ? pick(wc, y, x, wy, x) : pgm_lk_code(2u, y - wy, 0u);
            }
            if (st_task == 1u && cx - 1u < PK && c0.y > PGM_NEG_INF) {
                float best = INFINITY;
                bool ok = true, rep_edge = false, open = false;
                uint32_t wx = 0;
                float4 wc = c0;
                for (uint32_t q = 0; q < cx; ++q) {
                    const uint32_t xp = G.p_c[(TT + lx) * PK + q];
                    if (xp < hx0) { ok = false; break; }
                    const float xv = G.p_v[(TT + lx) * PK + q];
                    const float4 c = G.cell[hc(y, xp)];
                    const bool ru = G.p_u[(TT + lx) * PK + q] != 0u;
                    float d = fabsf(__fsub_rn(c0.y, __fsub_rn(__fadd_rn(c.y, sc.gap_extend), xv)));
                    if (best > d) { best = d; wx = xp; wc = c; rep_edge = ru; open = false; }
                    d = fabsf(__fsub_rn(c0.y, __fsub_rn(__fadd_rn(c.z, sc.gap_init), xv)));
                    if (best > d) { best = d; wx = xp; wc = c; rep_edge = ru; open = true; }
                }
                if (ok && best < INFINITY && !rep_edge) link = open ? pick(wc, y, x, y, wx) : pgm_lk_code(1u, 0u, x - wx);
            }
        }
        G.tab[task] = link;
    }
    __syncthreads();
// ... 1359 lines not shown
```

### prographmsa_amd/csrc/pgm_capi.hip

```cpp
#include <hip/hip_runtime.h>

#include <algorithm>
#include <cmath>
#include <cstdio>
#include <thread>
#include <atomic>
#include <chrono>
#include <queue>
#include <cstdlib>
#include <cstring>
#include <numeric>
#include <optional>
#include <mutex>
#include <string>
#include <unordered_set>
#include <vector>
#include <sys/mman.h>

#include "pgm_align_kernels.h"
#include "pgm_crit_kernels.h"
#include "pgm_nw_kernels.h"
#include "pgm_csprofile_kernels.h"
#include "pgm_dist_kernels.h"
#include "pgm_merge_kernels.h"
// ... 1 lines not shown
#include "pgm_wls_kernels.h"
#include "pgm_bionj_kernels.h"
#include "pgm_agreement_kernels.h"
#include "pgm_transfer_kernels.h"
#include "pgm_treelik_kernels.h"
#include "pgm_resample_kernels.h"
#include "pgm_pool.h"
#include "pgm_plan.h"
#include "pgm_treelik_check.h"
#include "pgm_treelik_plan.h"
static_assert(kC3Bytes == PGM_C3_BYTES, "pgm_plan.h plans the LDS of a crit3 sweep with PGM_C3_BYTES");

static thread_local std::string g_err;
static int fail(int code, const std::string &m) { g_err = m; return code; }
#define HIPCHK(x)                                                                                   \
    do {                                                                                            \
        hipError_t e_ = (x);                                                                        \
        if (e_ != hipSuccess)                                                                       \
            return fail(PGM_ERR_DEVICE, std::string(#x) + ": " + hipGetErrorString(e_));            \
    } while (0)

struct PgmNwState;
struct pgm_ctx {
    int device = 0;
    PgmNwState *nw = nullptr;
    int nw_per_cu = 0;
    struct ResChunk { uint8_t *p; size_t cap; };
    std::vector<ResChunk> res_chunks;
    size_t res_chunk = 0, res_off = 0;
    hipStream_t stream = nullptr;
    hipStream_t stream2 = nullptr;
    hipStream_t stream3 = nullptr;
    hipStream_t stream4 = nullptr;
    enum { C_IN, C_WORK, C_CELLS, C_OUT, C_S, C_HOST, C_HIN, C_SMALL, C_SLOTS };
    void *cache_ptr[C_SLOTS] = {};
    size_t cache_bytes[C_SLOTS] = {};
    hipDeviceProp_t prop;
    float nw_ms = 0, cs_ms = 0, ml_ms = 0, merge_ms = 0, pars_ms = 0, wls_ms = 0;
    uint32_t wls_n = 0, wls_launches = 0;
    float bionj_ms = 0;
    float agree_ms = 0;
    float transfer_ms = 0;
    float treelik_ms = 0;
    float resample_ms = 0;
    uint32_t bionj_launches = 0;
    enum {
        SC_DIST,
        SC_DIST_END = SC_DIST + 9,
        SC_CS = SC_DIST_END,
        SC_CS_END = SC_CS + 8,
        SC_MERGE_OUT = SC_CS_END,
        SC_PARS_IN,
        SC_PARS_OUT,
        SC_WLS_MAT,
        SC_WLS_IN,
        SC_WLS_PART,
        SC_WLS_OUT,
        SC_BIONJ_MAT,
        SC_BIONJ_VEC,
        SC_BIONJ_OUT,
        SC_AGREE_IN,
        SC_AGREE_OUT,
        SC_TRANSFER_REF,
        SC_TRANSFER_REP,
        SC_TRANSFER_OUT,
        SC_TREELIK_TREE,
        SC_TREELIK_P,
        SC_TREELIK_U,
        SC_TREELIK_G,
        SC_TREELIK_OUT,
        SC_RESAMPLE_X,
        SC_RESAMPLE_XT,
        SC_RESAMPLE_COLS,
        SC_RESAMPLE_OUT,
        SC_DEV
    };
    enum {
        SH_PROFILES_OUT,
        SC_HOST
    };
    void *sc_dev[SC_DEV] = {};
    size_t sc_dev_bytes[SC_DEV] = {};
    void *sc_host[SC_HOST] = {};
    size_t sc_host_bytes[SC_HOST] = {};
    hipEvent_t sc_ev[2] = {nullptr, nullptr};
    uint32_t csK = 0, csC = 0;
    double *cs_lprofiles = nullptr, *cs_centre = nullptr, *cs_priors = nullptr;
};

static pgm_pool::Pool &lib_pool() {
    static pgm_pool::Pool pool(std::max(1u, std::min(16u, std::thread::hardware_concurrency())));
    return pool;
}

static std::mutex g_pinned_mu;
static std::unordered_set<void *> g_pinned_registered;
static hipError_t pinned_alloc(size_t bytes, void **out) {
    const size_t H = (size_t)2 << 20, len = (std::max<size_t>(bytes, 1) + H - 1) / H * H;
    void *p = getenv("PGM_PINNED_MALLOC") ? nullptr : aligned_alloc(H, len);
    if (p) {
        (void)madvise(p, len, MADV_HUGEPAGE);
        (void)lib_pool().run(len / H, len >= 8 * H ? 16u : 1u, [&](size_t c) { for (size_t o = 0; o < H; o += 4096) ((volatile char *)p)[c * H + o] = 0; });
        if (hipHostRegister(p, len, hipHostRegisterDefault) == hipSuccess) {
            std::lock_guard<std::mutex> g(g_pinned_mu);
            g_pinned_registered.insert(p);
            *out = p;
            return hipSuccess;
        }
        (void)hipGetLastError();
        free(p);
    }
    return hipHostMalloc(out, bytes, hipHostMallocDefault);
}
static void pinned_free(void *p) {
    if (!p) return;
    bool reg;
    { std::lock_guard<std::mutex> g(g_pinned_mu); reg = g_pinned_registered.erase(p) != 0; }
    if (reg) { (void)hipHostUnregister(p); free(p); }
    else (void)hipHostFree(p);
}
static void slot_free(int slot, void *p) {
    if (slot == pgm_ctx::C_HIN) pinned_free(p);
    else if (slot == pgm_ctx::C_HOST) (void)hipHostFree(p);
    else (void)hipFree(p);
}

struct pgm_align_batch {
    uint32_t njobs = 0;
    uint64_t cells = 0;
    uint32_t maxdim = 0, maxnb = 0, maxn = 0, maxnblk = 0;
    std::vector<PgmJob> jobs;
    std::vector<uint32_t> order;
    BatchSchedule sched;
    uint8_t *d_in = nullptr;
    uint8_t *d_work = nullptr;
    uint8_t *d_cells = nullptr;
    uint8_t *d_out = nullptr;
    uint8_t *d_S = nullptr;
    uint8_t *d_small = nullptr;
    size_t in_bytes = 0, work_bytes = 0, cell_bytes = 0, out_bytes = 0, s_bytes = 0, small_bytes = 0;
    size_t cap[8] = {0, 0, 0, 0, 0, 0, 0, 0};
    uint8_t *h_out = nullptr;
    uint8_t *h_in = nullptr;
    int *h_flag = nullptr;
    int *d_sync = nullptr;
    size_t sync_ints = 0;
    uint32_t lq_off = 0;
    PgmJob *d_jobs = nullptr;
    uint32_t *d_order = nullptr;
    PgmItem *d_items = nullptr;
    uint32_t *d_lean = nullptr;
    PgmItem *d_bands = nullptr;
    int2 *d_tblist = nullptr;
    unsigned long long *d_times = nullptr;
    int *d_tabhdr = nullptr;
    hipEvent_t ev_fork = nullptr, ev_join = nullptr;
    hipEvent_t ev_join_b = nullptr, ev_join_c = nullptr;
    uint32_t test_spin_limit = 0, test_stall_job = 0xFFFFFFFFu, test_stall_band = 0;
    double acc_ms[3] = {0, 0, 0};
    uint32_t acc_n = 0;
    bool ev_pending = false;
    std::vector<size_t> res_off, map1_off, map2_off;
    hipEvent_t ev[5] = {nullptr, nullptr, nullptr, nullptr, nullptr};
};
static const struct BatchBuffer { int slot; size_t reserve_mb; uint8_t *pgm_align_batch::*ptr; size_t pgm_align_batch::*bytes; } kBatchBuffers[6] = {
    {pgm_ctx::C_IN, 128, &pgm_align_batch::d_in, &pgm_align_batch::in_bytes}, {pgm_ctx::C_WORK, 256, &pgm_align_batch::d_work, &pgm_align_batch::work_bytes},
    {pgm_ctx::C_CELLS, 2048, &pgm_align_batch::d_cells, &pgm_align_batch::cell_bytes}, {pgm_ctx::C_OUT, 8, &pgm_align_batch::d_out, &pgm_align_batch::out_bytes},
    {pgm_ctx::C_S, 1024, &pgm_align_batch::d_S, &pgm_align_batch::s_bytes}, {pgm_ctx::C_SMALL, 4, &pgm_align_batch::d_small, &pgm_align_batch::small_bytes}};

extern "C" {

const char *pgm_last_error(void) { return g_err.c_str(); }

int pgm_device_count(void) {
    int n = 0;
    if (hipGetDeviceCount(&n) != hipSuccess) return 0;
    return n;
}

__global__ void pgm_warm_kernel() {}

int pgm_ctx_create(int device, pgm_ctx **out) {
    if (!out) return fail(PGM_ERR_INVALID, "null out");
    *out = nullptr;
    int n = 0;
    HIPCHK(hipGetDeviceCount(&n));
    if (device < 0 || device >= n) return fail(PGM_ERR_DEVICE, "no such HIP device");
    HIPCHK(hipSetDevice(device));
    pgm_ctx *c = new pgm_ctx;
    c->device = device;
    HIPCHK(hipGetDeviceProperties(&c->prop, device));
    HIPCHK(hipStreamCreateWithFlags(&c->stream, hipStreamNonBlocking));
    HIPCHK(hipStreamCreateWithFlags(&c->stream2, hipStreamNonBlocking));
    HIPCHK(hipStreamCreateWithFlags(&c->stream3, hipStreamNonBlocking));
    {
        int lo = 0, hi = 0;
        if (hipDeviceGetStreamPriorityRange(&lo, &hi) != hipSuccess) { (void)hipGetLastError(); lo = hi = 0; }
        if (hipStreamCreateWithPriority(&c->stream4, hipStreamNonBlocking, hi) != hipSuccess) {
            (void)hipGetLastError();
            HIPCHK(hipStreamCreateWithFlags(&c->stream4, hipStreamNonBlocking));
        }
    }
    hipLaunchKernelGGL(pgm_warm_kernel, dim3(1), dim3(64), 0, c->stream);
    HIPCHK(hipGetLastError());
    HIPCHK(hipStreamSynchronize(c->stream));
    {
        void *h = nullptr, *d = nullptr;
        const size_t wb = (size_t)1 << 20;
        if (hipHostMalloc(&h, wb, hipHostMallocDefault) == hipSuccess && hipMalloc(&d, wb) == hipSuccess) {
            (void)hipMemcpyAsync(d, h, wb, hipMemcpyHostToDevice, c->stream);
            (void)hipMemcpyAsync(h, d, wb, hipMemcpyDeviceToHost, c->stream);
            (void)hipStreamSynchronize(c->stream);
        }
        if (h) (void)hipHostFree(h);
        if (d) (void)hipFree(d);
    }
    (void)lib_pool().run(64, 16u, [](size_t) {});
    {
        void *p = nullptr;
        const size_t sb = (size_t)128 << 20;
        if (!getenv("PGM_NO_STAGING_RESERVE") && pinned_alloc(sb, &p) == hipSuccess) { c->cache_ptr[pgm_ctx::C_HIN] = p; c->cache_bytes[pgm_ctx::C_HIN] = sb; }
        else (void)hipGetLastError();
        const size_t rb = (size_t)8 << 20;
        if (!getenv("PGM_NO_STAGING_RESERVE") && hipHostMalloc(&p, rb, hipHostMallocDefault) == hipSuccess) { c->cache_ptr[pgm_ctx::C_HOST] = p; c->cache_bytes[pgm_ctx::C_HOST] = rb; }
        else (void)hipGetLastError();
        if (!getenv("PGM_NO_STAGING_RESERVE") && !getenv("PGM_NO_DEVICE_RESERVE")) {
            for (const BatchBuffer &e : kBatchBuffers) {
                void *d = nullptr;
                if (hipMalloc(&d, e.reserve_mb << 20) == hipSuccess) { c->cache_ptr[e.slot] = d; c->cache_bytes[e.slot] = e.reserve_mb << 20; }
                else { (void)hipGetLastError(); break; }
            }
        }
    }
    *out = c;
    return PGM_OK;
}

static void nw_state_free(PgmNwState *st);
void pgm_ctx_destroy(pgm_ctx *ctx) {
    if (!ctx) return;
    (void)hipSetDevice(ctx->device);
    nw_state_free(ctx->nw);
    for (auto &c : ctx->res_chunks) if (c.p) (void)hipFree(c.p);
    if (ctx->cs_lprofiles) (void)hipFree(ctx->cs_lprofiles);
    if (ctx->cs_centre) (void)hipFree(ctx->cs_centre);
    if (ctx->cs_priors) (void)hipFree(ctx->cs_priors);
    for (int k = 0; k < pgm_ctx::SC_DEV; ++k) if (ctx->sc_dev[k]) (void)hipFree(ctx->sc_dev[k]);
    for (int k = 0; k < pgm_ctx::SC_HOST; ++k) if (ctx->sc_host[k]) pinned_free(ctx->sc_host[k]);
    for (int k = 0; k < 2; ++k) if (ctx->sc_ev[k]) (void)hipEventDestroy(ctx->sc_ev[k]);
    for (int k = 0; k < pgm_ctx::C_SLOTS; ++k)
        if (ctx->cache_ptr[k]) slot_free(k, ctx->cache_ptr[k]);
    if (ctx->stream4) (void)hipStreamDestroy(ctx->stream4);
    if (ctx->stream3) (void)hipStreamDestroy(ctx->stream3);
    if (ctx->stream2) (void)hipStreamDestroy(ctx->stream2);
    if (ctx->stream) (void)hipStreamDestroy(ctx->stream);
    delete ctx;
}

int pgm_ctx_device_info(pgm_ctx *ctx, char *name, size_t name_len, int *cu_count) {
    if (!ctx) return fail(PGM_ERR_INVALID, "null ctx");
    if (name && name_len) snprintf(name, name_len, "%s (%s)", ctx->prop.name, ctx->prop.gcnArchName);
    if (cu_count) *cu_count = ctx->prop.multiProcessorCount;
    return PGM_OK;
}

}

namespace {
static hipError_t cache_take(pgm_ctx *ctx, int slot, size_t bytes, void **out, size_t *got) {
    if (ctx->cache_ptr[slot] && ctx->cache_bytes[slot] >= bytes) {
        *out = ctx->cache_ptr[slot]; *got = ctx->cache_bytes[slot];
        ctx->cache_ptr[slot] = nullptr; ctx->cache_bytes[slot] = 0;
        return hipSuccess;
    }
    if (ctx->cache_ptr[slot]) {
        slot_free(slot, ctx->cache_ptr[slot]);
        ctx->cache_ptr[slot] = nullptr; ctx->cache_bytes[slot] = 0;
    }
    *got = bytes;
    if (slot == pgm_ctx::C_HIN) return pinned_alloc(bytes, out);
    return slot == pgm_ctx::C_HOST ? hipHostMalloc(out, bytes, hipHostMallocDefault) : hipMalloc(out, bytes);
}
static void cache_give(pgm_ctx *ctx, int slot, void *p, size_t bytes) {
    if (!p) return;
    if (ctx && (!ctx->cache_ptr[slot] || ctx->cache_bytes[slot] < bytes)) {
        if (ctx->cache_ptr[slot]) slot_free(slot, ctx->cache_ptr[slot]);
        ctx->cache_ptr[slot] = p; ctx->cache_bytes[slot] = bytes;
    } else {
        slot_free(slot, p);
    }
}

static hipError_t scratch_dev(pgm_ctx *ctx, int slot, size_t bytes, void **out) {
    bytes = std::max<size_t>(bytes, 16);
    if (ctx->sc_dev_bytes[slot] < bytes) {
        if (ctx->sc_dev[slot]) (void)hipFree(ctx->sc_dev[slot]);
        ctx->sc_dev[slot] = nullptr; ctx->sc_dev_bytes[slot] = 0;
        const size_t want = bytes + bytes / 4;
        hipError_t e = hipMalloc(&ctx->sc_dev[slot], want);
        if (e != hipSuccess) return e;
        ctx->sc_dev_bytes[slot] = want;
    }
    *out = ctx->sc_dev[slot];
    return hipSuccess;
}
static hipError_t scratch_host(pgm_ctx *ctx, int slot, size_t bytes, void **out) {
// ... 14 lines not shown
        if (!ctx->sc_ev[k]) { hipError_t e = hipEventCreate(&ctx->sc_ev[k]); if (e != hipSuccess) return e; }
    return hipSuccess;
}

static hipError_t resident_alloc(pgm_ctx *ctx, size_t bytes, uint8_t **out) {
    bytes = (bytes + 255) / 256 * 256;
    while (ctx->res_chunk < ctx->res_chunks.size() && ctx->res_off + bytes > ctx->res_chunks[ctx->res_chunk].cap) { ++ctx->res_chunk; ctx->res_off = 0; }
    if (ctx->res_chunk == ctx->res_chunks.size()) {
        pgm_ctx::ResChunk c{nullptr, std::max<size_t>(bytes, (size_t)96 << 20)};
        const hipError_t e = hipMalloc((void **)&c.p, c.cap);
        if (e != hipSuccess) return e;
        ctx->res_chunks.push_back(c); ctx->res_off = 0;
    }
    *out = ctx->res_chunks[ctx->res_chunk].p + ctx->res_off;
    ctx->res_off += bytes;
    return hipSuccess;
}

struct HostImage {
    size_t align;
    std::vector<uint8_t> bytes;
    explicit HostImage(size_t a = 256) : align(a) {}
    size_t put(const void *src, size_t n) {
        const size_t o = bytes.size();
        bytes.resize(o + (n + align - 1) / align * align);
        if (src && n) memcpy(bytes.data() + o, src, n);
        return o;
    }
};

struct Buf { void **p; size_t bytes; const void *src; void *dst; bool zero; };

struct StageCall {
    pgm_ctx *ctx;
    const char *what;
    float *ms;
    hipStream_t s;
    hipError_t e;
    bool alloc_failed = false, queued = false, timed = false;
    StageCall(pgm_ctx *c, const char *w, float *t) : ctx(c), what(w), ms(t), s(c->stream), e(hipSetDevice(c->device)) {}
    bool ok() const { return e == hipSuccess; }
    void alloc(hipError_t r) { e = r; alloc_failed = r != hipSuccess; }
    template <class T> void buf(int slot, size_t bytes, T **p) { if (ok()) alloc(scratch_dev(ctx, slot, bytes, (void **)p)); }
    template <class T> void host(int slot, size_t bytes, T **p) { if (ok()) alloc(scratch_host(ctx, slot, bytes, (void **)p)); }
    template <class T> void resident(size_t bytes, T **p) { if (ok()) alloc(resident_alloc(ctx, bytes, (uint8_t **)p)); }
    void up(void *dst, const void *src, size_t bytes) { if (ok() && bytes) { queued = true; e = hipMemcpyAsync(dst, src, bytes, hipMemcpyHostToDevice, s); } }
    void zero(void *dst, size_t bytes) { if (ok() && bytes) { queued = true; e = hipMemsetAsync(dst, 0, bytes, s); } }
    void down(void *dst, const void *src, size_t bytes) { if (ok() && bytes) { queued = true; e = hipMemcpyAsync(dst, src, bytes, hipMemcpyDeviceToHost, s); } }
    void bufs(int first, int end, std::initializer_list<Buf> list) {
        if (ok() && (size_t)(end - first) < list.size()) e = hipErrorInvalidValue;
        for (const Buf &b : list) { buf(first++, b.bytes, b.p); if (b.src) up(*b.p, b.src, b.bytes); }
    }
    bool begin() {
        if (ok()) e = scratch_events(ctx);
        if (ok()) { queued = true; e = hipEventRecord(ctx->sc_ev[0], s); }
        return ok();
    }
    void end() {
        if (ok()) e = hipGetLastError();
        if (ok()) e = hipEventRecord(ctx->sc_ev[1], s);
        timed = ok();
    }
    int finish() {
        if (queued) { const hipError_t es = hipStreamSynchronize(s); if (ok()) e = es; }
        if (ok() && timed && ms) (void)hipEventElapsedTime(ms, ctx->sc_ev[0], ctx->sc_ev[1]);
        if (ok()) return PGM_OK;
        (void)hipGetLastError();
        return fail(alloc_failed && e == hipErrorOutOfMemory ? PGM_ERR_NOMEM : PGM_ERR_DEVICE, std::string(what) + ": " + hipGetErrorString(e));
    }
};

static hipError_t classify_lean_jobs(pgm_ctx *ctx, pgm_align_batch *b) {
    if (!b->d_tabhdr || b->njobs == 0) return hipSuccess;
    hipError_t e = hipMemsetAsync(b->d_tabhdr, 0, 4 * (size_t)PGM_TAB_HDR * b->njobs, ctx->stream);
    if (e != hipSuccess) return e;
    hipLaunchKernelGGL(pgm_classify_kernel, dim3(b->njobs, 2, (b->maxn + 1023) / 1024), dim3(256), 0, ctx->stream, b->d_jobs);
    return hipGetLastError();
}

#define PGM_STATUS_PENDING 0x7ffffff0
struct PrepTier { uint32_t tier, threads; size_t lds; };
static PrepTier prep_tier(uint32_t maxdim) {
    const uint32_t tier = alphabet_tier(maxdim), threads = tier == 64u ? 64u : 256u;
    return {tier, threads, ((size_t)maxdim * maxdim + maxdim + threads * ((size_t)maxdim + 1)) * sizeof(float)};
}
static hipError_t launch_all(pgm_ctx *ctx, pgm_align_batch *b, bool timed) {
    hipStream_t s = ctx->stream;
    const BatchSchedule &S = b->sched;
    hipError_t e;
    for (uint32_t i = 0; i < b->njobs; ++i) ((PgmJob::Result *)(b->h_out + b->res_off[i]))->status = PGM_STATUS_PENDING;
    if (timed && (e = hipEventRecord(b->ev[0], s)) != hipSuccess) return e;
    const PrepTier T = prep_tier(b->maxdim);
    const dim3 pg(b->njobs, 2, (b->maxn + T.threads - 1) / T.threads);
    if (T.tier == 4) hipLaunchKernelGGL((pgm_prep_kernel<4, 256>), pg, dim3(256), T.lds, s, b->d_jobs, b->d_sync, (uint32_t)b->sync_ints);
    else if (T.tier == 20) hipLaunchKernelGGL((pgm_prep_kernel<20, 256>), pg, dim3(256), T.lds, s, b->d_jobs, b->d_sync, (uint32_t)b->sync_ints);
    else hipLaunchKernelGGL((pgm_prep_kernel<64, 64>), pg, dim3(64), T.lds, s, b->d_jobs, b->d_sync, (uint32_t)b->sync_ints);
    if ((e = hipGetLastError()) != hipSuccess) return e;
    if (timed && (e = hipEventRecord(b->ev[1], s)) != hipSuccess) return e;
    const dim3 eg((b->maxnblk + PGM_EM_TB - 1) / PGM_EM_TB, (b->maxnb + 3) / 4, b->njobs);
    if (T.tier == 4) hipLaunchKernelGGL((pgm_emission_skew_kernel<4, 1>), eg, dim3(4 * PGM_ROWS), 0, s, b->d_jobs);
    else if (T.tier == 20) hipLaunchKernelGGL((pgm_emission_skew_kernel<20, 1>), eg, dim3(4 * PGM_ROWS), 0, s, b->d_jobs);
    else hipLaunchKernelGGL((pgm_emission_skew_kernel<64, 1>), eg, dim3(4 * PGM_ROWS), 0, s, b->d_jobs);
    if ((e = hipGetLastError()) != hipSuccess) return e;
    if (timed && (e = hipEventRecord(b->ev[2], s)) != hipSuccess) return e;
    const uint32_t spin_limit = b->test_spin_limit ? b->test_spin_limit : PGM_SPIN_LIMIT, stall_job = b->test_stall_job, stall_band = b->test_stall_band;
    const bool fork = S.nlean != 0;
    const bool bandk = S.nbands != 0;
    const bool tbk = (S.nitems != 0 || bandk) && (S.ntb + S.ntb_c + S.ntb_b) != 0;
    const bool critk = S.ncrit != 0;
    if ((fork || bandk || critk) && (e = hipEventRecord(b->ev_fork, s)) != hipSuccess) return e;
    if (critk && (e = hipStreamWaitEvent(ctx->stream4, b->ev_fork, 0)) != hipSuccess) return e;
    if (fork && (e = hipStreamWaitEvent(ctx->stream2, b->ev_fork, 0)) != hipSuccess) return e;
    if (bandk && (e = hipStreamWaitEvent(ctx->stream3, b->ev_fork, 0)) != hipSuccess) return e;
    const uint32_t nrest = S.nitems - S.ncrit;
    hipStream_t sc = critk ? s : ctx->stream4, sr = critk ? ctx->stream4 : s;
    auto sweep = [&](hipStream_t st, uint32_t workers, const PgmItem *list, uint32_t n, bool c3, uint32_t ticket_off) {
        if (c3) hipLaunchKernelGGL(pgm_crit_kernel, dim3(workers), dim3(64 * PGM_C3_WAVES), 0, st, b->d_jobs, list, n, b->d_sync, spin_limit, stall_job, stall_band, ticket_off);
        else hipLaunchKernelGGL(pgm_fill_kernel, dim3(workers), dim3(64 * PGM_WAVES), 0, st, b->d_jobs, list, n, b->d_sync, spin_limit, stall_job, stall_band, ticket_off);
    };
    auto tracebacks = [&](hipStream_t st, uint32_t workers, uint32_t first, uint32_t n, uint32_t lq_off, uint32_t sybase) {
        hipLaunchKernelGGL(pgm_tb_kernel, dim3(workers), dim3(64 * PGM_WAVES), 0, st, b->d_jobs, b->d_tblist + first, n, b->d_sync, b->test_spin_limit, lq_off, sybase, 1u);
    };
    if (critk) sweep(sc, S.ncrit_workers, b->d_items, S.ncrit, S.crit_c3, (uint32_t)PGM_SY_CRIT_TICKET);
    if (nrest != 0) sweep(sr, S.nworkers, b->d_items + S.ncrit, nrest, S.rest_c3, 1u);
    if ((e = hipGetLastError()) != hipSuccess) return e;
    if (fork) {
        hipLaunchKernelGGL((pgm_lean_kernel<2>), dim3(S.nlean_workers), dim3(64 * PGM_WAVES), 0, ctx->stream2, b->d_jobs, b->d_lean, S.nlean, b->d_sync, spin_limit);
        if ((e = hipGetLastError()) != hipSuccess) return e;
    }
    const uint32_t njp = (b->njobs + 3u) / 4u * 4u;
    if (bandk) {
        hipLaunchKernelGGL(pgm_band_kernel, dim3(S.nband_workers), dim3(64 * PGM_WAVES), 0, ctx->stream3, b->d_jobs, b->d_bands, S.nbands_narrow, S.nbands, S.nband_workers - S.nwide_workers, b->d_sync, spin_limit, stall_job, stall_band);
        if ((e = hipGetLastError()) != hipSuccess) return e;
        if (tbk && S.ntb_b) tracebacks(ctx->stream3, S.ntb_b_workers, S.ntb + S.ntb_c, S.ntb_b, b->lq_off + njp, 8u);
        if ((e = hipGetLastError()) != hipSuccess) return e;
        if ((e = hipEventRecord(b->ev_join_b, ctx->stream3)) != hipSuccess) return e;
    }
    if (critk) {
        if (tbk && S.ntb_c) tracebacks(sc, S.ncrit_workers, S.ntb, S.ntb_c, b->lq_off + 2 * njp, 16u);
        if ((e = hipGetLastError()) != hipSuccess) return e;
    }
    if (tbk && S.ntb) {
        tracebacks(sr, S.ntb_workers, 0u, S.ntb, b->lq_off, 0u);
        if ((e = hipGetLastError()) != hipSuccess) return e;
    }
    if (critk && (e = hipEventRecord(b->ev_join_c, ctx->stream4)) != hipSuccess) return e;
    if (bandk && (e = hipStreamWaitEvent(s, b->ev_join_b, 0)) != hipSuccess) return e;
    if (critk && (e = hipStreamWaitEvent(s, b->ev_join_c, 0)) != hipSuccess) return e;
    if (fork && ((e = hipEventRecord(b->ev_join, ctx->stream2)) != hipSuccess || (e = hipStreamWaitEvent(s, b->ev_join, 0)) != hipSuccess)) return e;
    if (timed && (e = hipEventRecord(b->ev[3], s)) != hipSuccess) return e;
    if (timed && (e = hipEventRecord(b->ev[4], s)) != hipSuccess) return e;
    return hipSuccess;
}
struct SmallLayout { size_t sync, jobs, order, items, lean, tblist, bands, times, tabhdr, total_bands; bool any_lean; };
static SmallLayout layout_small(pgm_align_batch *b) {
    SmallLayout s;
    const uint32_t njobs = b->njobs;
    s.total_bands = 0; s.any_lean = false;
    for (const PgmJob &J : b->jobs) { s.total_bands += J.nb; s.any_lean = s.any_lean || (J.lean && !J.keep_cells); }
    DevLayout SM;
    s.sync = SM.take(b->sync_ints * sizeof(int)); s.jobs = SM.take(sizeof(PgmJob) * std::max(1u, njobs));
    s.order = SM.take(4 * (size_t)std::max(1u, njobs)); s.items = SM.take(sizeof(PgmItem) * std::max<size_t>(1, s.total_bands));
    s.lean = SM.take(4 * (size_t)std::max(1u, njobs)); s.tblist = SM.take(8 * (size_t)std::max(1u, njobs));
    s.bands = SM.take(sizeof(PgmItem) * std::max<size_t>(1, s.total_bands)); s.times = SM.take(16 * (size_t)std::max(1u, njobs) + 16);
    s.tabhdr = SM.take(s.any_lean ? 4 * (size_t)PGM_TAB_HDR * njobs : 16);
    b->small_bytes = SM.bytes;
    return s;
}

static double now_ms() { return std::chrono::duration<double, std::milli>(std::chrono::steady_clock::now().time_since_epoch()).count(); }

struct BatchAlloc {
    std::atomic<int> state{0};
    hipError_t err = hipSuccess, host_err = hipSuccess;
    uint8_t *h_out_dev = nullptr;
    double ms_dev = 0, ms_host = 0, ms_slot[6] = {0, 0, 0, 0, 0, 0};
};
static void take_batch_buffers(pgm_ctx *ctx, pgm_align_batch *b, SmallLayout sm, BatchAlloc *A) {
    const double ta0 = now_ms();
    hipError_t e2 = hipSetDevice(ctx->device);
    double tprev = ta0;
    for (int k = 0; k < 6 && e2 == hipSuccess; ++k) {
        const BatchBuffer &s = kBatchBuffers[k];
        e2 = cache_take(ctx, s.slot, b->*s.bytes, (void **)&(b->*s.ptr), &b->cap[s.slot]);
        const double t = now_ms(); A->ms_slot[k] = t - tprev; tprev = t;
    }
    if (e2 == hipSuccess) {
        b->d_sync = (int *)(b->d_small + sm.sync);
        b->d_jobs = (PgmJob *)(b->d_small + sm.jobs);
        b->d_order = (uint32_t *)(b->d_small + sm.order);
        b->d_items = (PgmItem *)(b->d_small + sm.items);
        b->d_lean = (uint32_t *)(b->d_small + sm.lean);
        b->d_tblist = (int2 *)(b->d_small + sm.tblist);
        b->d_bands = (PgmItem *)(b->d_small + sm.bands);
        b->d_times = (unsigned long long *)(b->d_small + sm.times);
        b->d_tabhdr = sm.any_lean ? (int *)(b->d_small + sm.tabhdr) : nullptr;
    }
    A->err = e2;
    A->state.store(e2 == hipSuccess ? 1 : -1, std::memory_order_release);
    A->ms_dev = now_ms() - ta0;
    if (e2 == hipSuccess) {
        hipError_t e3 = cache_take(ctx, pgm_ctx::C_HOST, b->out_bytes + 64, (void **)&b->h_out, &b->cap[pgm_ctx::C_HOST]);
        if (e3 == hipSuccess) b->h_flag = (int *)(b->h_out + (b->out_bytes + 15) / 16 * 16);
        if (e3 == hipSuccess) e3 = hipHostGetDevicePointer((void **)&A->h_out_dev, b->h_out, 0);
        A->host_err = e3;
    }
    A->ms_host = now_ms() - ta0 - A->ms_dev;
}

struct CreateGuard {
    pgm_ctx *ctx;
    pgm_align_batch *b;
    std::thread alloc;
    ~CreateGuard() { if (alloc.joinable()) alloc.join(); if (b) pgm_align_batch_destroy(ctx, b); }
    pgm_align_batch *release() { pgm_align_batch *r = b; b = nullptr; return r; }
};

static void bind_job_pointers(pgm_align_batch *b, const std::vector<JobOff> &off, const pgm_site_ref *res1, const pgm_site_ref *res2, uint8_t *h_out_dev) {
    for (uint32_t i = 0; i < b->njobs; ++i) {
        PgmJob &J = b->jobs[i];
        const JobOff &o = off[i];
        uint8_t *in = b->d_in, *w = b->d_work, *ob = b->d_out;
        J.sites1 = site_ref_of(res1, i) ? res1[i].dev_sites : (const double *)(in + o.s1.sites);
        J.sites2 = site_ref_of(res2, i) ? res2[i].dev_sites : (const double *)(in + o.s2.sites);
        J.smap1 = o.s1.has_smap ? (const uint32_t *)(in + o.s1.smap) : nullptr;
        J.smap2 = o.s2.has_smap ? (const uint32_t *)(in + o.s2.smap) : nullptr;
        J.M = (const double *)(in + o.M); J.pi = (const double *)(in + o.pi);
        J.ni1 = (const PgmNode2 *)(in + o.s1.ni); J.ni2 = (const PgmNode2 *)(in + o.s2.ni);
        J.xp1 = (const int32_t *)(in + o.s1.xp); J.xp2 = (const int32_t *)(in + o.s2.xp);
        J.xc1 = (const uint32_t *)(in + o.s1.xc); J.xc2 = (const uint32_t *)(in + o.s2.xc);
        J.xv1 = (const float *)(in + o.s1.xv); J.xv2 = (const float *)(in + o.s2.xv);
        J.fp1 = (const int32_t *)(in + o.s1.fp); J.fe1 = (const uint2 *)(in + o.s1.fe);
        J.ov2 = (const uint2 *)(in + o.s2.ov);
        J.pp1 = (const int32_t *)(in + o.s1.pp); J.pp2 = (const int32_t *)(in + o.s2.pp);
        J.pc1 = (const uint32_t *)(in + o.s1.pc); J.pc2 = (const uint32_t *)(in + o.s2.pc);
        J.pv1 = (const float *)(in + o.s1.pv); J.pv2 = (const float *)(in + o.s2.pv);
        J.pu1 = (const uint32_t *)(in + o.s1.pu); J.pu2 = (const uint32_t *)(in + o.s2.pu);
        J.g1f = (float *)(w + o.g1f); J.a1 = (float *)(w + o.a1);
        J.t2 = (float *)(w + o.t2); J.b2 = (float *)(w + o.aux2);
        J.map1 = (uint32_t *)(ob + o.map1); J.map2 = (uint32_t *)(ob + o.map2);
        J.mark_score = (float *)(w + o.ms); J.mark_prev = (uint32_t *)(w + o.mp);
        J.tb1 = (PgmTbNode *)(w + o.tb1); J.tb2 = (PgmTbNode *)(w + o.tb2);
        J.result = (PgmJob::Result *)(ob + o.res);
        J.hmap1 = (uint32_t *)(h_out_dev + o.map1); J.hmap2 = (uint32_t *)(h_out_dev + o.map2);
        J.hresult = (PgmJob::Result *)(h_out_dev + o.res);
        J.cells = (float4 *)(b->d_cells + o.cells);
        J.codes = (uint32_t *)(w + o.codes);
        J.endcell = (float4 *)(w + o.endcell);
        if (J.lean && !J.keep_cells && b->d_tabhdr) { J.cls1 = w + o.cls; J.cls2 = w + o.cls + J.n1; J.tabhdr = b->d_tabhdr + (size_t)PGM_TAB_HDR * i; }
        else { J.cls1 = nullptr; J.cls2 = nullptr; J.tabhdr = nullptr; }
        J.S = (float *)(b->d_S + o.S);
        J.prog = b->d_sync + o.prog;
        J.ltab = (uint16_t *)(w + o.ltab); J.lready = b->d_sync + o.lready; J.lrows = o.lrows; J.lcols = o.lcols;
        J.times = b->d_times + 2 * (size_t)i;
    }
}

static std::vector<uint32_t> size_order(const std::vector<PgmJob> &jobs) {
    std::vector<uint32_t> order(jobs.size());
    std::iota(order.begin(), order.end(), 0u);
    std::stable_sort(order.begin(), order.end(), [&](uint32_t x, uint32_t y) { return (uint64_t)jobs[x].n1 * jobs[x].n2 > (uint64_t)jobs[y].n1 * jobs[y].n2; });
    return order;
}
}

extern "C" {

int pgm_test_cu_shares(uint32_t cus, double lean_cost, uint32_t nlean, double band_cost, uint32_t nbands, double rest_cost, uint32_t nrest,
                       uint32_t ncrit, double longest_chain, uint32_t *out4) {
    if (!out4) return fail(PGM_ERR_INVALID, "null argument");
    const CuShares r = cu_shares(cus, lean_cost, nlean, band_cost, nbands, rest_cost, nrest, ncrit, longest_chain);
    out4[0] = r.lean; out4[1] = r.band; out4[2] = r.crit; out4[3] = r.rest;
    return PGM_OK;
}

int pgm_test_batch_plan(uint32_t njobs, const pgm_graph *const *g1, const pgm_graph *const *g2, const pgm_model *const *model,
                        const pgm_scores *scores, uint32_t flags, const pgm_site_ref *res1, const pgm_site_ref *res2, uint32_t cus,
                        uint32_t *head, double *dhead, uint32_t *job_fields, uint32_t *items, uint32_t *bands, uint32_t *lean_list, int32_t *tblist) {
    if (!head || !dhead || !items || !bands || (njobs && (!g1 || !g2 || !model || !scores || !job_fields || !lean_list || !tblist))) return fail(PGM_ERR_INVALID, "null argument");
    std::vector<char> two_chains(njobs, 0);
    for (uint32_t i = 0; i < njobs; ++i) two_chains[i] = job_is_two_chains(g1[i], g2[i]) ? 1 : 0;
    std::vector<PgmJob> jobs;
    BatchSizes Z;
    const int invalid = plan_sizes(njobs, g1, g2, model, scores, flags, res1, res2, two_chains, cus, jobs, Z);
    if (invalid >= 0) return fail(PGM_ERR_INVALID, "invalid job " + std::to_string(invalid));
    std::vector<uint8_t> image(std::max<size_t>(Z.in_base[njobs], 16));
    for (uint32_t i = 0; i < njobs; ++i)
        if (!plan_flatten_job(image.data(), Z.in_base[i], Z.in_base[i + 1], g1[i], g2[i], model[i], site_ref_of(res1, i), site_ref_of(res2, i), Z.pro, jobs[i], Z.off[i]))
            return fail(PGM_ERR_INVALID, "invalid graph in job " + std::to_string(i));
    const BatchSchedule S = plan_schedule(jobs, size_order(jobs), cus);
    const uint32_t h[PGM_PLAN_HEAD] = {njobs ? Z.pro.batch_dp : 0u, Z.pro.promote_bands, S.nitems, S.ncrit, S.nbands, S.nbands_narrow, S.nlean, S.ntb, S.ntb_c, S.ntb_b,
                                       S.nworkers, S.nlean_workers, S.nband_workers, S.nwide_workers, S.ncrit_workers, S.ntb_workers, S.ntb_b_workers,
                                       S.crit_c3, S.rest_c3, S.capacity, (uint32_t)S.total_b, (uint32_t)S.total, (uint32_t)S.total_c};
    const double d[PGM_PLAN_DHEAD] = {S.rsweep, S.t_goal, S.lean_cost, S.band_cost, S.band_end, S.other_cost, S.fill_end, S.crit_end, Z.pro.longest_crit_chain};
    memcpy(head, h, sizeof h);
    memcpy(dhead, d, sizeof d);
    for (uint32_t i = 0; i < njobs; ++i) {
        const PgmJob &J = jobs[i];
        const uint32_t f[PGM_PLAN_JOB] = {J.lean, J.has_extras, J.mode2, J.hD, J.hDX, J.slot_bytes, J.aux_off, J.ov_off, J.rh_off, J.c3_off, J.nov2, J.has_far, J.long1, J.long2,
                                          J.crit3, J.far_slack, J.nslots, Z.off[i].s1.ngeneric + Z.off[i].s2.ngeneric, Z.off[i].s1.nkill + Z.off[i].s2.nkill};
        memcpy(job_fields + (size_t)PGM_PLAN_JOB * i, f, sizeof f);
    }
    if (S.nitems) memcpy(items, S.items.data(), sizeof(PgmItem) * S.nitems);
    if (S.nbands) memcpy(bands, S.bands.data(), sizeof(PgmItem) * S.nbands);
    if (S.nlean) memcpy(lean_list, S.lean_list.data(), 4 * (size_t)S.nlean);
    if (S.ntb + S.ntb_c + S.ntb_b) memcpy(tblist, S.tblist.data(), 8 * (size_t)(S.ntb + S.ntb_c + S.ntb_b));
    return PGM_OK;
}

int pgm_align_batch_create(pgm_ctx *ctx, uint32_t njobs, const pgm_graph *const *g1, const pgm_graph *const *g2,
                           const pgm_model *const *model, const pgm_scores *scores, pgm_align_batch **out) {
    return pgm_align_batch_create_ex(ctx, njobs, g1, g2, model, scores, 0u, out);
}

int pgm_align_batch_create_ex(pgm_ctx *ctx, uint32_t njobs, const pgm_graph *const *g1, const pgm_graph *const *g2,
                              const pgm_model *const *model, const pgm_scores *scores, uint32_t flags, pgm_align_batch **out) {
    return pgm_align_batch_create_res(ctx, njobs, g1, g2, model, scores, flags, nullptr, nullptr, out);
}

int pgm_align_batch_create_res(pgm_ctx *ctx, uint32_t njobs, const pgm_graph *const *g1, const pgm_graph *const *g2,
                               const pgm_model *const *model, const pgm_scores *scores, uint32_t flags,
                               const pgm_site_ref *res1, const pgm_site_ref *res2, pgm_align_batch **out) {
    if (!ctx || !out || (njobs && (!g1 || !g2 || !model || !scores))) return fail(PGM_ERR_INVALID, "null argument");
    *out = nullptr;
    HIPCHK(hipSetDevice(ctx->device));
    const double tcs = now_ms();
    const bool cprof = getenv("PGM_HOST_PROFILE") != nullptr;
    const uint32_t cus = (uint32_t)ctx->prop.multiProcessorCount;
    BatchAlloc A;
    CreateGuard G{ctx, new pgm_align_batch, {}};
    pgm_align_batch *b = G.b;
    b->njobs = njobs;
    std::vector<char> two_chains(njobs, 0);
    (void)lib_pool().run(njobs, njobs >= 16 ? 16u : 1u, [&](size_t i) { two_chains[i] = job_is_two_chains(g1[i], g2[i]) ? 1 : 0; });
    BatchSizes Z;
    const int invalid = plan_sizes(njobs, g1, g2, model, scores, flags, res1, res2, two_chains, cus, b->jobs, Z);
    if (invalid >= 0) return fail(PGM_ERR_INVALID, "invalid job " + std::to_string(invalid));
    const std::vector<size_t> &in_base = Z.in_base;
    b->maxdim = Z.maxdim; b->maxnb = Z.maxnb; b->maxn = Z.maxn; b->maxnblk = Z.maxnblk; b->cells = Z.cells;
    b->res_off.resize(njobs); b->map1_off.resize(njobs); b->map2_off.resize(njobs);
    for (uint32_t i = 0; i < njobs; ++i) { b->res_off[i] = Z.off[i].res; b->map1_off[i] = Z.off[i].map1; b->map2_off[i] = Z.off[i].map2; }
    b->in_bytes = std::max<size_t>(in_base[njobs], 16);
    b->work_bytes = std::max<size_t>(Z.L.W.bytes, 16);
    b->cell_bytes = std::max<size_t>(Z.L.C.bytes, 16);
    b->out_bytes = std::max<size_t>(Z.L.O.bytes, 16);
    b->s_bytes = std::max<size_t>(Z.L.SL.bytes, 16);
    b->lq_off = (uint32_t)Z.L.sync_ints;
    b->sync_ints = Z.L.sync_ints + 3 * (((size_t)njobs + 3) / 4 * 4);
    const double tc0 = now_ms();
    const SmallLayout sm = layout_small(b);
    G.alloc = std::thread(take_batch_buffers, ctx, b, sm, &A);
    hipError_t e;
    if ((e = cache_take(ctx, pgm_ctx::C_HIN, b->in_bytes, (void **)&b->h_in, &b->cap[pgm_ctx::C_HIN])) != hipSuccess)
        return fail(PGM_ERR_DEVICE, std::string("hipHostMalloc: ") + hipGetErrorString(e));
    const double tc1 = now_ms();
    std::atomic<int> bad(-1), upload_err((int)hipSuccess);
    const uint32_t chunk_jobs = (uint32_t)std::max<size_t>(1, ((size_t)8 << 20) / std::max<size_t>(1, in_base[njobs] / std::max(1u, njobs)));
    std::vector<std::atomic<uint32_t>> chunk_done((njobs + chunk_jobs - 1) / chunk_jobs + 1);
    for (auto &cd : chunk_done) cd.store(0);
    (void)lib_pool().run(njobs, 16, [&](size_t job_index) {
        const uint32_t i = (uint32_t)job_index;
        if (!plan_flatten_job(b->h_in, in_base[i], in_base[i + 1], g1[i], g2[i], model[i], site_ref_of(res1, i), site_ref_of(res2, i), Z.pro, b->jobs[i], Z.off[i])) { bad.store((int)i); return; }
        const uint32_t c = i / chunk_jobs, c0 = c * chunk_jobs, c1 = std::min(njobs, c0 + chunk_jobs);
        if (chunk_done[c].fetch_add(1, std::memory_order_acq_rel) + 1 == c1 - c0) {
            int st;
            while ((st = A.state.load(std::memory_order_acquire)) == 0) std::this_thread::yield();
            if (st == 1) {
                (void)hipSetDevice(ctx->device);
                const hipError_t eu = hipMemcpyAsync(b->d_in + in_base[c0], b->h_in + in_base[c0], in_base[c1] - in_base[c0], hipMemcpyHostToDevice, ctx->stream);
                if (eu != hipSuccess) upload_err.store((int)eu);
            }
        }
    });
    if (bad.load() >= 0) return fail(PGM_ERR_INVALID, "invalid graph in job " + std::to_string(bad.load()));
    const double tc2 = now_ms();
    G.alloc.join();
    const double tc3 = now_ms();
    if (A.err != hipSuccess) return fail(A.err == hipErrorOutOfMemory ? PGM_ERR_NOMEM : PGM_ERR_DEVICE, std::string("hipMalloc: ") + hipGetErrorString(A.err));
    if (A.host_err != hipSuccess) return fail(PGM_ERR_DEVICE, std::string("hipHostMalloc: ") + hipGetErrorString(A.host_err));
    bind_job_pointers(b, Z.off, res1, res2, A.h_out_dev);
    b->order = size_order(b->jobs);
    b->sched = plan_schedule(b->jobs, b->order, cus);
    const BatchSchedule &S = b->sched;
    if (cprof && njobs)
        fprintf(stderr, "    work lists: longest chain of sweeps %.0f us, goal %.0f us; lean %zu jobs %.0f us-worker on %u CUs; bands %zu, %.0f us-worker on %u CUs (simulated end %.0f us); items %zu, %.0f us-worker on %u CUs (simulated end %.0f us), of the longest chains %zu on %u CUs (%.0f us)\n",
                S.rsweep, S.t_goal, (size_t)S.nlean, S.lean_cost, S.nlean_workers, S.total_b, S.band_cost, S.nband_workers, S.band_end, S.total, S.other_cost, S.capacity, S.fill_end, S.total_c, S.ncrit_workers, S.crit_end);
    const double tc4 = now_ms();
    if (S.nitems > std::max<size_t>(1, sm.total_bands)) return fail(PGM_ERR_DEVICE, "work list longer than the number of bands");
    if ((e = (hipError_t)upload_err.load()) != hipSuccess ||
        (e = hipMemcpyAsync(b->d_tblist, S.tblist.data(), 8 * S.tblist.size(), hipMemcpyHostToDevice, ctx->stream)) != hipSuccess ||
        (e = hipMemcpyAsync(b->d_jobs, b->jobs.data(), sizeof(PgmJob) * njobs, hipMemcpyHostToDevice, ctx->stream)) != hipSuccess ||
        (e = hipMemcpyAsync(b->d_order, b->order.data(), 4 * (size_t)njobs, hipMemcpyHostToDevice, ctx->stream)) != hipSuccess ||
        (e = hipMemcpyAsync(b->d_items, S.items.data(), sizeof(PgmItem) * S.items.size(), hipMemcpyHostToDevice, ctx->stream)) != hipSuccess ||
        (e = hipMemcpyAsync(b->d_lean, S.lean_list.data(), 4 * S.lean_list.size(), hipMemcpyHostToDevice, ctx->stream)) != hipSuccess ||
        (e = hipMemcpyAsync(b->d_bands, S.bands.data(), sizeof(PgmItem) * S.bands.size(), hipMemcpyHostToDevice, ctx->stream)) != hipSuccess ||
        (e = classify_lean_jobs(ctx, b)) != hipSuccess ||
        (e = hipStreamSynchronize(ctx->stream)) != hipSuccess)
        return fail(PGM_ERR_DEVICE, std::string("upload: ") + hipGetErrorString(e));
    for (int k = 0; k < 5; ++k) (void)hipEventCreate(&b->ev[k]);
    (void)hipEventCreateWithFlags(&b->ev_fork, hipEventDisableTiming);
    (void)hipEventCreateWithFlags(&b->ev_join, hipEventDisableTiming);
    (void)hipEventCreateWithFlags(&b->ev_join_b, hipEventDisableTiming);
    (void)hipEventCreateWithFlags(&b->ev_join_c, hipEventDisableTiming);
    if (cprof)
        fprintf(stderr, "    create: sizes %.2f ms, pinned input block %.2f, flatten %.2f, wait for the allocations %.2f (device %.2f, pinned results %.2f), work list %.2f, upload of %.1f MB %.2f\n",
                tc0 - tcs, tc1 - tc0, tc2 - tc1, tc3 - tc2, A.ms_dev, A.ms_host, tc4 - tc3, b->in_bytes / 1e6, now_ms() - tc4);
    if (cprof)
        fprintf(stderr, "    device buffers: inputs %.1f MB %.2f ms, work %.1f MB %.2f, cells %.1f MB %.2f, results %.1f MB %.2f, S %.1f MB %.2f, small %.2f\n",
                b->in_bytes / 1e6, A.ms_slot[0], b->work_bytes / 1e6, A.ms_slot[1], b->cell_bytes / 1e6, A.ms_slot[2], b->out_bytes / 1e6, A.ms_slot[3], b->s_bytes / 1e6, A.ms_slot[4], A.ms_slot[5]);
    *out = G.release();
    return PGM_OK;
}

int pgm_align_batch_run(pgm_ctx *ctx, pgm_align_batch *b) {
    if (!ctx || !b) return fail(PGM_ERR_INVALID, "null argument");
    if (b->njobs == 0) return PGM_OK;
    HIPCHK(hipSetDevice(ctx->device));
    HIPCHK(launch_all(ctx, b, true));
    b->ev_pending = true;
    return PGM_OK;
}

int pgm_align_batch_time(pgm_ctx *ctx, pgm_align_batch *b, int reps, float *ms_prep, float *ms_emission, float *ms_fill,
                         float *ms_traceback) {
    if (!ctx || !b || reps <= 0) return fail(PGM_ERR_INVALID, "bad argument");
    HIPCHK(hipSetDevice(ctx->device));
    double acc[4] = {0, 0, 0, 0};
    for (int r = 0; r < reps && b->njobs; ++r) {
        HIPCHK(launch_all(ctx, b, true));
        b->ev_pending = false;
        HIPCHK(hipEventSynchronize(b->ev[4]));
        for (int k = 0; k < 4; ++k) {
            float ms = 0;
            HIPCHK(hipEventElapsedTime(&ms, b->ev[k], b->ev[k + 1]));
            acc[k] += ms;
        }
    }
    if (ms_prep) *ms_prep = (float)(acc[0] / reps);
    if (ms_emission) *ms_emission = (float)(acc[1] / reps);
    if (ms_fill) *ms_fill = (float)(acc[2] / reps);
    if (ms_traceback) *ms_traceback = (float)(acc[3] / reps);
    return PGM_OK;
}

int pgm_align_batch_job_times(pgm_ctx *ctx, pgm_align_batch *b, uint64_t *ticks) {
    if (!ctx || !b || !ticks) return fail(PGM_ERR_INVALID, "null argument");
    HIPCHK(hipSetDevice(ctx->device));
    HIPCHK(hipStreamSynchronize(ctx->stream));
    if (b->njobs) HIPCHK(hipMemcpy(ticks, b->d_times, 16 * (size_t)b->njobs, hipMemcpyDeviceToHost));
    return PGM_OK;
}

int pgm_align_batch_fetch(pgm_ctx *ctx, pgm_align_batch *b, pgm_align_out *out) {
    if (!ctx || !b || (b->njobs && !out)) return fail(PGM_ERR_INVALID, "null argument");
    HIPCHK(hipSetDevice(ctx->device));
    if (b->njobs == 0) { HIPCHK(hipStreamSynchronize(ctx->stream)); return PGM_OK; }
    int rc = PGM_OK;
    HIPCHK(hipMemcpyAsync(b->h_flag, b->d_sync, sizeof(int), hipMemcpyDeviceToHost, ctx->stream));
    std::vector<uint8_t> copied(b->njobs, 0);
    auto collect = [&]() -> int {
        uint32_t n = 0;
        for (uint32_t i = 0; i < b->njobs; ++i) {
            if (copied[i]) { ++n; continue; }
            const PgmJob::Result *hr = (const PgmJob::Result *)(b->h_out + b->res_off[i]);
            const int32_t st = __atomic_load_n(&hr->status, __ATOMIC_ACQUIRE);
            if (st == PGM_STATUS_PENDING) continue;
            if (!out[i].map1 || !out[i].map2) return -1;
            const uint32_t len = hr->len;
            if (len > b->jobs[i].n1 + b->jobs[i].n2) return -2;
            out[i].score = hr->score; out[i].n_tr_indels = hr->n_tr_indels; out[i].len = len; out[i].status = st;
            memcpy(out[i].map1, b->h_out + b->map1_off[i], 4 * (size_t)len);
            memcpy(out[i].map2, b->h_out + b->map2_off[i], 4 * (size_t)len);
            copied[i] = 1; ++n;
        }
        return (int)n;
    };
    for (;;) {
        const int n = collect();
        if (n < 0) { (void)hipStreamSynchronize(ctx->stream); return fail(n == -1 ? PGM_ERR_INVALID : PGM_ERR_DEVICE, n == -1 ? "null mapping buffer" : "corrupt result length"); }
        if ((uint32_t)n == b->njobs) break;
        const hipError_t q = hipStreamQuery(ctx->stream);
        if (q == hipSuccess) break;
        if (q != hipErrorNotReady) return fail(PGM_ERR_DEVICE, std::string("fill kernel: ") + hipGetErrorString(q));
    }
    HIPCHK(hipStreamSynchronize(ctx->stream));
    if (b->ev_pending) {
        b->ev_pending = false;
        float ms[3] = {0, 0, 0};
        bool ok = true;
        for (int k = 0; k < 3; ++k) ok = ok && hipEventElapsedTime(&ms[k], b->ev[k], b->ev[k + 1]) == hipSuccess;
        if (ok) { for (int k = 0; k < 3; ++k) b->acc_ms[k] += ms[k]; ++b->acc_n; }
        else (void)hipGetLastError();
    }
    const int aborted = *b->h_flag;
    if (aborted) return fail(PGM_ERR_DEVICE, "fill kernel: a band hand-off timed out");
    for (uint32_t i = 0; i < b->njobs; ++i) {
        PgmJob::Result res;
        memcpy(&res, b->h_out + b->res_off[i], sizeof res);
        if (res.status == PGM_STATUS_PENDING) return fail(PGM_ERR_DEVICE, "fill kernel: a job's result record was never written");
        if (res.status != PGM_OK) rc = res.status;
        if (copied[i]) continue;
        out[i].score = res.score;
        out[i].n_tr_indels = res.n_tr_indels;
        out[i].len = res.len;
        out[i].status = res.status;
        if (res.status != PGM_OK) rc = res.status;
        if (!out[i].map1 || !out[i].map2) return fail(PGM_ERR_INVALID, "null mapping buffer");
        if (res.len > b->jobs[i].n1 + b->jobs[i].n2) return fail(PGM_ERR_DEVICE, "corrupt result length");
        memcpy(out[i].map1, b->h_out + b->map1_off[i], 4 * (size_t)res.len);
        memcpy(out[i].map2, b->h_out + b->map2_off[i], 4 * (size_t)res.len);
    }
    if (rc != PGM_OK) g_err = "backtracking failed";
    return rc;
}

void pgm_align_batch_destroy(pgm_ctx *ctx, pgm_align_batch *b) {
    if (!b) return;
    if (ctx) { (void)hipSetDevice(ctx->device); (void)hipStreamSynchronize(ctx->stream); }
    if (ctx && ctx->stream2) (void)hipStreamSynchronize(ctx->stream2);
    if (ctx && ctx->stream3) (void)hipStreamSynchronize(ctx->stream3);
    if (ctx && ctx->stream4) (void)hipStreamSynchronize(ctx->stream4);
    for (int k = 0; k < 5; ++k)
        if (b->ev[k]) (void)hipEventDestroy(b->ev[k]);
    if (b->ev_fork) (void)hipEventDestroy(b->ev_fork);
    if (b->ev_join) (void)hipEventDestroy(b->ev_join);
    if (b->ev_join_b) (void)hipEventDestroy(b->ev_join_b);
    if (b->ev_join_c) (void)hipEventDestroy(b->ev_join_c);
    for (const BatchBuffer &e : kBatchBuffers) cache_give(ctx, e.slot, b->*e.ptr, b->cap[e.slot]);
    cache_give(ctx, pgm_ctx::C_HOST, b->h_out, b->cap[pgm_ctx::C_HOST]);
    cache_give(ctx, pgm_ctx::C_HIN, b->h_in, b->cap[pgm_ctx::C_HIN]);
    delete b;
}

uint64_t pgm_align_batch_cells(const pgm_align_batch *b) { return b ? b->cells : 0; }

int pgm_align_batch_stage_times(pgm_align_batch *b, int reset, float *ms_prep, float *ms_emission, float *ms_fill, uint32_t *launches) {
    if (!b) return fail(PGM_ERR_INVALID, "null batch");
    const double n = b->acc_n ? (double)b->acc_n : 1.0;
    if (ms_prep) *ms_prep = (float)(b->acc_ms[0] / n);
    if (ms_emission) *ms_emission = (float)(b->acc_ms[1] / n);
    if (ms_fill) *ms_fill = (float)(b->acc_ms[2] / n);
    if (launches) *launches = b->acc_n;
    if (reset) { b->acc_ms[0] = b->acc_ms[1] = b->acc_ms[2] = 0; b->acc_n = 0; }
    return PGM_OK;
}

int pgm_align_batch_test_stall(pgm_align_batch *b, uint32_t job, uint32_t band, uint32_t spin_limit) {
    if (!b) return fail(PGM_ERR_INVALID, "null batch");
    b->test_stall_job = job; b->test_stall_band = band; b->test_spin_limit = spin_limit;
    return PGM_OK;
}

int pgm_align_graphs_batch(pgm_ctx *ctx, uint32_t njobs, const pgm_graph *const *g1, const pgm_graph *const *g2,
                           const pgm_model *const *model, const pgm_scores *scores, pgm_align_out *out) {
    return pgm_align_graphs_batch_res(ctx, njobs, g1, g2, model, scores, nullptr, nullptr, out);
}

int pgm_align_graphs_batch_res(pgm_ctx *ctx, uint32_t njobs, const pgm_graph *const *g1, const pgm_graph *const *g2,
                               const pgm_model *const *model, const pgm_scores *scores, const pgm_site_ref *res1, const pgm_site_ref *res2,
                               pgm_align_out *out) {
    pgm_align_batch *b = nullptr;
    const bool prof = getenv("PGM_HOST_PROFILE") != nullptr;
    const auto t0 = std::chrono::steady_clock::now();
    int rc = pgm_align_batch_create_res(ctx, njobs, g1, g2, model, scores, 0u, res1, res2, &b);
    if (rc != PGM_OK) return rc;
    const auto t1 = std::chrono::steady_clock::now();
    {
        static std::mutex device_turn[64];
        std::lock_guard<std::mutex> turn(device_turn[(unsigned)ctx->device % 64u]);
        rc = pgm_align_batch_run(ctx, b);
        if (rc == PGM_OK) rc = pgm_align_batch_fetch(ctx, b, out);
    }
    const auto t2 = std::chrono::steady_clock::now();
    pgm_align_batch_destroy(ctx, b);
    if (prof)
        fprintf(stderr, "  pgm_align_graphs_batch: %u jobs, create (flatten, allocate, upload, work list) %.2f ms, run + fetch %.2f ms, destroy %.2f ms\n", njobs,
                std::chrono::duration<double, std::milli>(t1 - t0).count(), std::chrono::duration<double, std::milli>(t2 - t1).count(),
                std::chrono::duration<double, std::milli>(std::chrono::steady_clock::now() - t2).count());
    return rc;
}

int pgm_align_batch_read_matrices(pgm_ctx *ctx, pgm_align_batch *b, uint32_t job, float *M, float *X, float *Y, float *W, float *S) {
    if (!ctx || !b || job >= b->njobs) return fail(PGM_ERR_INVALID, "bad argument");
    HIPCHK(hipSetDevice(ctx->device));
    HIPCHK(hipStreamSynchronize(ctx->stream));
    const PgmJob &J = b->jobs[job];
    const size_t N = (size_t)J.n1 * J.n2;
    if ((M || X || Y || W) && !J.keep_cells)
        return fail(PGM_ERR_INVALID, "the DP matrices of a chain-only job are only kept for a batch created with PGM_BATCH_KEEP_MATRICES");
    if (S && J.tabhdr) {
        int bad = 1;
        HIPCHK(hipMemcpy(&bad, J.tabhdr, sizeof(int), hipMemcpyDeviceToHost));
        if (bad == 0) return fail(PGM_ERR_INVALID, "the score matrix of a job of two sequence graphs is only stored for a batch created with PGM_BATCH_KEEP_MATRICES");
    }
    if (M || X || Y || W) {
        const uint32_t sh = J.rshift, R = 1u << sh;
        const size_t ncell = (size_t)J.nb * J.tsteps * 64u * R;
        std::vector<float4> cells(ncell);
        HIPCHK(hipMemcpy(cells.data(), J.cells, ncell * sizeof(float4), hipMemcpyDeviceToHost));
        float *dst[4] = {M, X, Y, W};
        for (int k = 0; k < 4; ++k)
            if (dst[k]) std::fill(dst[k], dst[k] + N, -INFINITY);
// ... 41 lines not shown
```

### prographmsa_amd/csrc/pgm_device.h

```cpp
#ifndef PGM_DEVICE_H_
#define PGM_DEVICE_H_

#include <stdint.h>
#include "../../include/pgm_hip.h"

#define PGM_MAX_DIM 64
#define PGM_HALO 0
#define PGM_ROWS 64
#define PGM_VL 16
#define PGM_BLOCK 8
#define PGM_NRING 128
#define PGM_KF 4
#define PGM_KF8 8
#define PGM_DCAP 28
#define PGM_PF 4
#define PGM_REMOTE_MAX 128
#define PGM_WAVES 8
#define PGM_WIDE_WAVES 4
#define PGM_POOL 163584
#define PGM_CPARTS 3
#define PGM_AUX_RES 0
#define PGM_AUX_SBLK 3072
#define PGM_AUX_EL 9216
#define PGM_AUX_CNT 13312
#define PGM_AUX_BYTES 13328

#define PGM_NF_COUNT 15u
#define PGM_NF_GENERIC 16u
#define PGM_NF_KILL 32u
#define PGM_NF_NLONG(f) (((f) >> 16) & 3u)
#define PGM_NF_NOV(f) (((f) >> 20) & 31u)
#define PGM_NF_OVI(f) (((f) >> 25) & 127u)
#define PGM_OV_ENT 16
#define PGM_OV_REC 128
#define PGM_NLONG 3
struct PgmNode2 {
    float cc, c2, c3;
    uint32_t flags;
    uint32_t fd[PGM_KF8];
    float fc[PGM_KF8];
};

#define PGM_TB_PK 8
struct PgmTbNode {
    uint32_t cnt;
    uint32_t c[PGM_TB_PK];
    float v[PGM_TB_PK];
    uint32_t u[PGM_TB_PK];
    uint32_t pad[7];
};

struct PgmJob {
    uint32_t n1, n2;
    uint32_t dim, dp;
    uint32_t nb;
    uint32_t ncol;
    uint32_t tsteps;
    uint32_t maxn;
    uint32_t has_extras;
    uint32_t has_far;
    uint32_t mode2;
    uint32_t far_slack;
    uint32_t aux_off;
    uint32_t hD, hDX;
    uint32_t slot_bytes;
    uint32_t nslots;
    uint32_t rshift;
    uint32_t lean;
    uint32_t crit3;
    uint32_t c3_off;
    uint32_t long1, long2;
    pgm_scores sc;

    const double *sites1, *sites2;
    const uint32_t *smap1, *smap2;
    const double *M, *pi;
    const PgmNode2 *ni1, *ni2;
    const int32_t *xp1, *xp2;
    const uint32_t *xc1, *xc2;
    const float *xv1, *xv2;
    const int32_t *fp1;
    const uint2 *fe1;
    const uint2 *ov2;
    uint32_t nov2, ov_off;
    uint32_t rh_off;
    const int32_t *pp1, *pp2;
    const uint32_t *pc1, *pc2;
    const float *pv1, *pv2;
    const uint32_t *pu1, *pu2;

    PgmTbNode *tb1, *tb2;
    float *g1f;
    float *a1;
    float *t2;
    float *b2;

    float *S;
    uint32_t nblk;
    const uint8_t *cls1, *cls2;
    int *tabhdr;

    uint32_t *codes;
    float4 *endcell;
    uint32_t keep_cells;

    uint16_t *ltab;
    int *lready;
    uint32_t lrows, lcols;

    unsigned long long *times;

    float4 *cells;
    int *prog;

    uint32_t *map1, *map2;
    float *mark_score;
    uint32_t *mark_prev;
    struct Result { float score; uint32_t n_tr_indels; uint32_t len; int32_t status; } *result;
    uint32_t *hmap1, *hmap2;
    Result *hresult;
};


#define PGM_SY_BAND_TICKET 3
#define PGM_SY_CRIT_TICKET 4
#define PGM_SY_WIDE_TICKET 5
#define PGM_SY_LQ_N 32
#define PGM_SY_TB_DONE 33
#define PGM_SY_TBQ_N 34
#define PGM_LK_W 4u
#define PGM_LK_T 32u
#define PGM_LK_NR 4u
#define PGM_LK_MIN_ROWS 1216u
#define PGM_LK_H 16u
#define PGM_LK_TAB (3u * PGM_LK_T * PGM_LK_T)
__host__ __device__ inline uint32_t pgm_lk_first(uint32_t n1, uint32_t n2, uint32_t lcols, uint32_t r) {
    const uint32_t w = lcols < PGM_LK_W ? lcols : PGM_LK_W;
    const uint64_t xc = ((uint64_t)(PGM_LK_T * r + PGM_LK_T / 2u) * (n2 - 1u)) / (n1 - 1u);
    const uint32_t g = (uint32_t)(xc / PGM_LK_T);
    const uint32_t lo = g >= w / 2u ? g - w / 2u : 0u;
    return lo + w > lcols ? lcols - w : lo;
}

struct PgmItem {
    uint32_t job, band;
    uint32_t prio, count;
};

#endif
```

Baseline: 81.20.

## Stage two traceback tiles at once and batch diagonal runs in walk

The traceback worker now stages a second 32x32 tile into LDS, overlaid in a union with the lookup table, when no lookup table is in use. This aims to cut the number of serial stage/link rounds along the traceback path. The cell-slot mapping is hoisted out of the staging lambda. The walk also detects straight diagonal runs with a wavefront ballot and pushes them in bulk instead of one step at a time. Walk statistics counters and an API to read them are added, at the cost of more LDS, more registers and extra complexity.

```diff
diff --git a/include/pgm_hip.h b/include/pgm_hip.h
--- a/include/pgm_hip.h
+++ b/include/pgm_hip.h
@@ -90,6 +90,7 @@
 int pgm_align_batch_stage_times(pgm_align_batch *b, int reset, float *ms_prep, float *ms_emission, float *ms_fill,
                                 uint32_t *launches);
 int pgm_align_batch_job_times(pgm_ctx *ctx, pgm_align_batch *b, uint64_t *ticks);
+int pgm_align_batch_walk_stats(pgm_ctx *ctx, pgm_align_batch *b, uint32_t *out);
 int pgm_align_batch_test_stall(pgm_align_batch *b, uint32_t job, uint32_t band, uint32_t spin_limit);
 int pgm_test_cu_shares(uint32_t cus, double lean_cost, uint32_t nlean, double band_cost, uint32_t nbands, double rest_cost,
                        uint32_t nrest, uint32_t ncrit, double longest_chain, uint32_t *out4);
diff --git a/prographmsa_amd/__init__.py b/prographmsa_amd/__init__.py
--- a/prographmsa_amd/__init__.py
+++ b/prographmsa_amd/__init__.py
@@ -72,7 +72,7 @@
 EXPORTS = [
     "pgm_device_count", "pgm_ctx_create", "pgm_ctx_destroy", "pgm_last_error", "pgm_ctx_device_info",
     "pgm_align_graphs_batch", "pgm_align_batch_create", "pgm_align_batch_create_ex", "pgm_align_batch_create_res", "pgm_align_graphs_batch_res", "pgm_align_batch_run", "pgm_align_batch_fetch",
-    "pgm_align_batch_destroy", "pgm_align_batch_cells", "pgm_align_batch_test_stall", "pgm_test_cu_shares", "pgm_test_batch_plan", "pgm_align_batch_stage_times", "pgm_align_batch_job_times", "pgm_align_batch_time", "pgm_align_batch_read_matrices",
+    "pgm_align_batch_destroy", "pgm_align_batch_cells", "pgm_align_batch_test_stall", "pgm_test_cu_shares", "pgm_test_batch_plan", "pgm_align_batch_stage_times", "pgm_align_batch_job_times", "pgm_align_batch_walk_stats", "pgm_align_batch_time", "pgm_align_batch_read_matrices",
     "pgm_nw_pairs_batch", "pgm_nw_pairs_submit", "pgm_nw_pairs_wait", "pgm_nw_last_kernel_ms", "pgm_host_alloc", "pgm_host_free", "pgm_csprofile_load", "pgm_csprofile_create_batch", "pgm_csprofile_create_batch_res",
     "pgm_csprofile_last_kernel_ms", "pgm_mldist_batch", "pgm_prealigned_counts_batch", "pgm_kmer_cosine", "pgm_dist_last_kernel_ms",
     "pgm_kmer_cosine_multi", "pgm_prealigned_counts_multi", "pgm_prealigned_counts_resampled",
@@ -117,6 +117,7 @@
                                           C.POINTER(u32), C.POINTER(C.c_double)] + [C.POINTER(u32)] * 4 + [C.POINTER(i32)]),
         "pgm_align_batch_stage_times": (C.c_int, [vp, C.c_int] + [C.POINTER(C.c_float)] * 3 + [C.POINTER(u32)]),
         "pgm_align_batch_job_times": (C.c_int, [vp, vp, C.POINTER(C.c_uint64)]),
+        "pgm_align_batch_walk_stats": (C.c_int, [vp, vp, C.POINTER(u32)]),
         "pgm_align_batch_time": (C.c_int, [vp, vp, C.c_int] + [C.POINTER(C.c_float)] * 4),
         "pgm_align_batch_read_matrices": (C.c_int, [vp, vp, u32] + [C.POINTER(C.c_float)] * 5),
         "pgm_nw_pairs_batch": (C.c_int, [vp, u32, C.POINTER(i32), i32, i32, u32, C.POINTER(C.c_int8), C.POINTER(u32), u32,
diff --git a/prographmsa_amd/csrc/pgm_align_kernels.h b/prographmsa_amd/csrc/pgm_align_kernels.h
--- a/prographmsa_amd/csrc/pgm_align_kernels.h
+++ b/prographmsa_amd/csrc/pgm_align_kernels.h
@@ -424,7 +424,7 @@
 #define PGM_TB_T 32
 #define PGM_TB_BAND 6
 #define PGM_TB_LK 4
-struct PgmTbLds {
+struct PgmTbTile {
     float4 cell[PGM_TB_T * PGM_TB_T];
     float S[PGM_TB_T * PGM_TB_T];
     uint32_t p_cnt[2 * PGM_TB_T];
@@ -433,16 +433,24 @@
     uint32_t p_u[2 * PGM_TB_T * PGM_TB_PK];
     uint16_t succ[3 * PGM_TB_T * PGM_TB_T];
     uint32_t ty0, tx0;
+    int nbig;
+    uint16_t big[128];
+};
+struct PgmTbLds {
+    PgmTbTile t0;
     uint32_t ay, ax;
     int req;
+    uint32_t two;
     uint32_t len;
-    int nbig;
-    uint16_t big[128];
-    uint16_t gtab[PGM_LK_NR][PGM_LK_W * PGM_LK_TAB] __attribute__((aligned(16)));
+    union U {
+        uint16_t gtab[PGM_LK_NR][PGM_LK_W * PGM_LK_TAB] __attribute__((aligned(16)));
+        PgmTbTile t1;
+    } u;
     uint2 mbuf[64];
     uint32_t grow, gcnt;
     uint32_t gnext[PGM_LK_NR];
 };
+static_assert(sizeof(PgmTbLds) + 64 <= 160 * 1024, "traceback worker: one per CU, within the CU's 160 KB of LDS");
 
 #define PGM_LK_HW (PGM_LK_T + PGM_LK_H)
 struct PgmLkLds {
@@ -489,73 +497,91 @@
     const PgmPred P2 = {J.pp2, J.pc2, J.pv2, J.pu2};
 
     const bool loader = tid >= 64;
+    uint32_t cslot[(TT * TT) / (64u * PGM_WAVES)];
+#pragma unroll
+    for (int u = 0; u < (int)((TT * TT) / (64u * PGM_WAVES)); ++u) {
+        const uint32_t i = (uint32_t)tid + 64u * PGM_WAVES * u;
+        const uint32_t half = TT * (TT + 1u) / 2u;
+        const bool up = i < half;
+        const uint32_t m = up ? i : TT * TT - 1u - i;
+        uint32_t d = (uint32_t)((sqrtf(8.0f * (float)m + 1.0f) - 1.0f) * 0.5f);
+        while (d * (d + 1u) / 2u > m) --d;
+        while ((d + 1u) * (d + 2u) / 2u <= m) ++d;
+        const uint32_t k = m - d * (d + 1u) / 2u;
+        cslot[u] = (up ? k : TT - 1u - k) * TT + (up ? d - k : TT - 1u - (d - k));
+    }
     auto stage = [&]() {
-        const uint32_t ty0 = T.ty0, tx0 = T.tx0;
+        const uint32_t nt = T.two != 0u ? 2u : 1u;
         constexpr uint32_t NT = 64u * PGM_WAVES;
         constexpr int NC = (int)((TT * TT) / NT), NP = (int)((2 * TT * PGM_TB_PK) / NT);
         static_assert(NC * NT == TT * TT && NP * NT == 2 * TT * PGM_TB_PK, "tile staging: whole rounds of the workgroup");
-        float4 cv[NC];
-        float sv[NC];
-        uint32_t cslot[NC];
-#pragma unroll
-        for (int u = 0; u < NC; ++u) {
-            const uint32_t i = (uint32_t)tid + NT * u;
-            const uint32_t half = TT * (TT + 1u) / 2u;
-            const bool up = i < half;
-            const uint32_t m = up ? i : TT * TT - 1u - i;
-            uint32_t d = (uint32_t)((sqrtf(8.0f * (float)m + 1.0f) - 1.0f) * 0.5f);
-            while (d * (d + 1u) / 2u > m) --d;
-            while ((d + 1u) * (d + 2u) / 2u <= m) ++d;
-            const uint32_t k = m - d * (d + 1u) / 2u;
-            const uint32_t ly = up ? k : TT - 1u - k, lx = up ? d - k : TT - 1u - (d - k);
-            cslot[u] = ly * TT + lx;
-            const uint32_t yy = min(ty0 + ly, n1 - 2), xx = min(tx0 + lx, n2 - 2);
-            cv[u] = J.cells[pgm_cell_index(J, yy, xx)];
-            const uint32_t ys = min(ty0 + i / TT, n1 - 2), xs = min(tx0 + i % TT, n2 - 2);
-            sv[u] = pgm_emission_at(J, ys, xs);
-        }
-        uint32_t cnt[NP], ec[NP], eu[NP];
-        float ev[NP];
-#pragma unroll
-        for (int u = 0; u < NP; ++u) {
-            const uint32_t i = (uint32_t)tid + NT * u, slot = i / PGM_TB_PK, k = i % PGM_TB_PK;
-            const bool row = slot < TT;
-            const uint32_t v = min(row ? ty0 + slot : tx0 + (slot - TT), (row ? n1 : n2) - 1);
-            const PgmTbNode *r = (row ? J.tb1 : J.tb2) + v;
-            cnt[u] = r->cnt; ec[u] = r->c[k]; ev[u] = r->v[k]; eu[u] = r->u[k];
-        }
-#pragma unroll
-        for (int u = 0; u < NC; ++u) {
-            const uint32_t i = (uint32_t)tid + NT * u;
-            T.cell[cslot[u]] = cv[u];
-            T.S[i] = sv[u];
-        }
-        for (uint32_t i = (uint32_t)tid; i < 3u * TT * TT / 2u; i += NT) ((uint32_t *)T.succ)[i] = 0u;
-        if (tid == 0) T.nbig = 0;
-#pragma unroll
-        for (int u = 0; u < NP; ++u) {
-            const uint32_t i = (uint32_t)tid + NT * u, slot = i / PGM_TB_PK, k = i % PGM_TB_PK;
-            const bool row = slot < TT;
-            const bool inr = (row ? ty0 + slot : tx0 + (slot - TT)) < (row ? n1 : n2);
-            if (k == 0) T.p_cnt[slot] = inr ? cnt[u] : 0xFFFFFFFFu;
-            T.p_c[i] = ec[u]; T.p_v[i] = ev[u]; T.p_u[i] = eu[u];
+        float4 cv[2][NC];
+        float sv[2][NC];
+        uint32_t cnt[2][NP], ec[2][NP], eu[2][NP];
+        float ev[2][NP];
+#pragma unroll
+        for (uint32_t t = 0; t < 2u; ++t) if (t < nt) {
+            const PgmTbTile &X = t ? T.u.t1 : T.t0;
+            const uint32_t ty0 = X.ty0, tx0 = X.tx0;
+#pragma unroll
+            for (int u = 0; u < NC; ++u) {
+                const uint32_t i = (uint32_t)tid + NT * u;
+                const uint32_t yy = min(ty0 + (cslot[u] / TT), n1 - 2), xx = min(tx0 + (cslot[u] % TT), n2 - 2);
+                cv[t][u] = J.cells[pgm_cell_index(J, yy, xx)];
+                const uint32_t ys = min(ty0 + i / TT, n1 - 2), xs = min(tx0 + i % TT, n2 - 2);
+                sv[t][u] = pgm_emission_at(J, ys, xs);
+            }
+#pragma unroll
+            for (int u = 0; u < NP; ++u) {
+                const uint32_t i = (uint32_t)tid + NT * u, slot = i / PGM_TB_PK, k = i % PGM_TB_PK;
+                const bool row = slot < TT;
+                const uint32_t v = min(row ? ty0 + slot : tx0 + (slot - TT), (row ? n1 : n2) - 1);
+                const PgmTbNode *r = (row ? J.tb1 : J.tb2) + v;
+                cnt[t][u] = r->cnt; ec[t][u] = r->c[k]; ev[t][u] = r->v[k]; eu[t][u] = r->u[k];
+            }
+        }
+#pragma unroll
+        for (uint32_t t = 0; t < 2u; ++t) if (t < nt) {
+            PgmTbTile &X = t ? T.u.t1 : T.t0;
+            const uint32_t ty0 = X.ty0, tx0 = X.tx0;
+#pragma unroll
+            for (int u = 0; u < NC; ++u) {
+                const uint32_t i = (uint32_t)tid + NT * u;
+                X.cell[cslot[u]] = cv[t][u];
+                X.S[i] = sv[t][u];
+            }
+            for (uint32_t i = (uint32_t)tid; i < 3u * TT * TT / 2u; i += NT) ((uint32_t *)X.succ)[i] = 0u;
+            if (tid == 0) X.nbig = 0;
+#pragma unroll
+            for (int u = 0; u < NP; ++u) {
+                const uint32_t i = (uint32_t)tid + NT * u, slot = i / PGM_TB_PK, k = i % PGM_TB_PK;
+                const bool row = slot < TT;
+                const bool inr = (row ? ty0 + slot : tx0 + (slot - TT)) < (row ? n1 : n2);
+                if (k == 0) X.p_cnt[slot] = inr ? cnt[t][u] : 0xFFFFFFFFu;
+                X.p_c[i] = ec[t][u]; X.p_v[i] = ev[t][u]; X.p_u[i] = eu[t][u];
+            }
         }
     };
     const pgm_scores sc = J.sc;
     const int band = J.has_extras ? PGM_TB_BAND : PGM_TB_BAND / 2;
     auto links = [&]() {
-        const uint32_t ty0 = T.ty0, tx0 = T.tx0;
-        const int adiag = (int)(T.ay - ty0) - (int)(T.ax - tx0);
+        const uint32_t nt = T.two != 0u ? 2u : 1u;
         const uint32_t NDIAG = 2u * (uint32_t)band + 1u;
-        for (uint32_t task = (uint32_t)tid; task < 3u * NDIAG * TT; task += (uint32_t)nthreads) {
-            const uint32_t lx = task % TT, st_task = task / (NDIAG * TT);
-            const int lyi = (int)lx + adiag + (int)((task / TT) % NDIAG) - band;
+        const uint32_t lx = (uint32_t)tid % TT;
+        uint32_t dg = (uint32_t)tid / TT, ti = 0u, st_task = 0u;
+        auto carry = [&]() { while (dg >= NDIAG) { dg -= NDIAG; if (++ti == nt) { ti = 0u; ++st_task; } } };
+        carry();
+        for (; st_task < 3u; dg += (uint32_t)nthreads / TT, carry()) {
+            PgmTbTile &X = ti ? T.u.t1 : T.t0;
+            const uint32_t ty0 = X.ty0, tx0 = X.tx0;
+            const int adiag = (int)(T.ay - ty0) - (int)(T.ax - tx0);
+            const int lyi = (int)lx + adiag + (int)dg - band;
             if (lyi < 0 || lyi >= (int)TT) continue;
             const uint32_t ly = (uint32_t)lyi, ci = ly * TT + lx, y = ty0 + ly, x = tx0 + lx;
             uint16_t lm = 0, lxs = 0, lys = 0;
             if (y + 1 < n1 && x + 1 < n2 && (y | x) != 0u) {
-                const float4 c0 = T.cell[ci];
-                const uint32_t cy = T.p_cnt[ly], cx = T.p_cnt[TT + lx];
+                const float4 c0 = X.cell[ci];
+                const uint32_t cy = X.p_cnt[ly], cx = X.p_cnt[TT + lx];
                 auto pick = [&](const float4 &c, uint32_t yp, uint32_t xp) -> uint16_t {
                     uint32_t st;
                     if ((yp | xp) == 0u) st = 0u;
@@ -565,20 +591,20 @@
                     else return (uint16_t)0;
                     return (uint16_t)(0x8000u | (st << 10) | ((yp - ty0) << 5) | (xp - tx0));
                 };
-                const int doff = (int)((task / TT) % NDIAG) - band;
+                const int doff = (int)dg - band;
                 if (st_task == 0u && doff >= -1 && doff <= 1 && (cy > PGM_TB_LK || cx > PGM_TB_LK) && cy <= PGM_TB_PK && cx <= PGM_TB_PK && cy != 0u && cx != 0u && c0.x > PGM_NEG_INF) {
-                    const int slot = __hip_atomic_fetch_add(&T.nbig, 1, __ATOMIC_RELAXED, __HIP_MEMORY_SCOPE_WORKGROUP);
-                    if (slot < 128) T.big[slot] = (uint16_t)ci;
+                    const int slot = __hip_atomic_fetch_add(&X.nbig, 1, __ATOMIC_RELAXED, __HIP_MEMORY_SCOPE_WORKGROUP);
+                    if (slot < 128) X.big[slot] = (uint16_t)ci;
                 }
                 if (st_task == 0u && cy <= PGM_TB_LK && cx <= PGM_TB_LK && cy != 0u && cx != 0u && c0.x > PGM_NEG_INF) {
-                    const float S = T.S[ci];
+                    const float S = X.S[ci];
                     uint32_t yp[PGM_TB_LK], xp[PGM_TB_LK];
                     float yv[PGM_TB_LK], xv[PGM_TB_LK];
                     bool ok = true;
 #pragma unroll
                     for (int k = 0; k < PGM_TB_LK; ++k) {
-                        yp[k] = T.p_c[ly * PGM_TB_PK + k]; yv[k] = T.p_v[ly * PGM_TB_PK + k];
-                        xp[k] = T.p_c[(TT + lx) * PGM_TB_PK + k]; xv[k] = T.p_v[(TT + lx) * PGM_TB_PK + k];
+                        yp[k] = X.p_c[ly * PGM_TB_PK + k]; yv[k] = X.p_v[ly * PGM_TB_PK + k];
+                        xp[k] = X.p_c[(TT + lx) * PGM_TB_PK + k]; xv[k] = X.p_v[(TT + lx) * PGM_TB_PK + k];
                         ok = ok && ((uint32_t)k >= cy || yp[k] >= ty0) && ((uint32_t)k >= cx || xp[k] >= tx0);
                     }
                     float wz[PGM_TB_LK][PGM_TB_LK];
@@ -586,7 +612,7 @@
                     for (int ky = 0; ky < PGM_TB_LK; ++ky)
 #pragma unroll
                         for (int kx = 0; kx < PGM_TB_LK; ++kx)
-                            wz[ky][kx] = T.cell[min((yp[ky] - ty0) * TT + (xp[kx] - tx0), TT * TT - 1u)].z;
+                            wz[ky][kx] = X.cell[min((yp[ky] - ty0) * TT + (xp[kx] - tx0), TT * TT - 1u)].z;
                     float best = INFINITY;
                     uint32_t wy = 0, wx = 0, wky = 0, wkx = 0;
 #pragma unroll
@@ -599,8 +625,8 @@
                     bool rep_edge = false;
                     float4 wc = c0;
                     if (ok && best < INFINITY) {
-                        rep_edge = (T.p_u[ly * PGM_TB_PK + wky] | T.p_u[(TT + lx) * PGM_TB_PK + wkx]) != 0u;
-                        wc = T.cell[(wy - ty0) * TT + (wx - tx0)];
+                        rep_edge = (X.p_u[ly * PGM_TB_PK + wky] | X.p_u[(TT + lx) * PGM_TB_PK + wkx]) != 0u;
+                        wc = X.cell[(wy - ty0) * TT + (wx - tx0)];
                     }
                     if (ok && best < INFINITY && !rep_edge) lm = pick(wc, wy, wx);
                 }
@@ -610,11 +636,11 @@
                     uint32_t wy = 0;
                     float4 wc = c0;
                     for (uint32_t k = 0; k < cy; ++k) {
-                        const uint32_t yp = T.p_c[ly * PGM_TB_PK + k];
+                        const uint32_t yp = X.p_c[ly * PGM_TB_PK + k];
                         if (yp < ty0) { ok = false; break; }
-                        const float yv = T.p_v[ly * PGM_TB_PK + k];
-                        const float4 c = T.cell[(yp - ty0) * TT + lx];
-                        const bool ru = T.p_u[ly * PGM_TB_PK + k] != 0u;
+                        const float yv = X.p_v[ly * PGM_TB_PK + k];
+                        const float4 c = X.cell[(yp - ty0) * TT + lx];
+                        const bool ru = X.p_u[ly * PGM_TB_PK + k] != 0u;
                         float d = fabsf(__fsub_rn(c0.w, __fsub_rn(__fadd_rn(c.w, sc.gap_extend), yv)));
                         if (best > d) { best = d; wy = yp; wc = c; rep_edge = ru; open = false; }
                         d = fabsf(__fsub_rn(c0.w, __fsub_rn(__fadd_rn(c.z, sc.gap_init), yv)));
@@ -629,11 +655,11 @@
                     uint32_t wx = 0;
                     float4 wc = c0;
                     for (uint32_t k = 0; k < cx; ++k) {
-                        const uint32_t xp = T.p_c[(TT + lx) * PGM_TB_PK + k];
+                        const uint32_t xp = X.p_c[(TT + lx) * PGM_TB_PK + k];
                         if (xp < tx0) { ok = false; break; }
-                        const float xv = T.p_v[(TT + lx) * PGM_TB_PK + k];
-                        const float4 c = T.cell[ly * TT + (xp - tx0)];
-                        const bool ru = T.p_u[(TT + lx) * PGM_TB_PK + k] != 0u;
+                        const float xv = X.p_v[(TT + lx) * PGM_TB_PK + k];
+                        const float4 c = X.cell[ly * TT + (xp - tx0)];
+                        const bool ru = X.p_u[(TT + lx) * PGM_TB_PK + k] != 0u;
                         float d = fabsf(__fsub_rn(c0.y, __fsub_rn(__fadd_rn(c.y, sc.gap_extend), xv)));
                         if (best > d) { best = d; wx = xp; wc = c; rep_edge = ru; open = false; }
                         d = fabsf(__fsub_rn(c0.y, __fsub_rn(__fadd_rn(c.z, sc.gap_init), xv)));
@@ -643,26 +669,29 @@
                         lxs = open ? pick(wc, y, wx) : (uint16_t)(0x8000u | (1u << 10) | (ly << 5) | (wx - tx0));
                 }
             }
-            T.succ[st_task * (TT * TT) + ci] = st_task == 0u ? lm : (st_task == 1u ? lxs : lys);
+            X.succ[st_task * (TT * TT) + ci] = st_task == 0u ? lm : (st_task == 1u ? lxs : lys);
         }
     };
     auto links_big = [&]() {
         const int wave = tid >> 6, lane_b = tid & 63, nwaves = nthreads >> 6;
-        const uint32_t ty0 = T.ty0, tx0 = T.tx0;
-        const int nbig = min(T.nbig, 128);
+        const uint32_t nt = T.two != 0u ? 2u : 1u;
+        for (uint32_t ti = 0; ti < nt; ++ti) {
+        PgmTbTile &X = ti ? T.u.t1 : T.t0;
+        const uint32_t ty0 = X.ty0, tx0 = X.tx0;
+        const int nbig = min(X.nbig, 128);
         for (int i = wave; i < nbig; i += nwaves) {
-            const uint32_t ci = T.big[i], ly = ci / TT, lx = ci % TT;
-            const uint32_t cy = T.p_cnt[ly], cx = T.p_cnt[TT + lx];
+            const uint32_t ci = X.big[i], ly = ci / TT, lx = ci % TT;
+            const uint32_t cy = X.p_cnt[ly], cx = X.p_cnt[TT + lx];
             const uint32_t ky = (uint32_t)lane_b >> 3, kx = (uint32_t)lane_b & 7u;
             const bool valid = ky < cy && kx < cx;
-            const uint32_t yp = T.p_c[ly * PGM_TB_PK + ky], xp = T.p_c[(TT + lx) * PGM_TB_PK + kx];
-            const float yv = T.p_v[ly * PGM_TB_PK + ky], xv = T.p_v[(TT + lx) * PGM_TB_PK + kx];
-            const uint32_t rep = T.p_u[ly * PGM_TB_PK + ky] | T.p_u[(TT + lx) * PGM_TB_PK + kx];
+            const uint32_t yp = X.p_c[ly * PGM_TB_PK + ky], xp = X.p_c[(TT + lx) * PGM_TB_PK + kx];
+            const float yv = X.p_v[ly * PGM_TB_PK + ky], xv = X.p_v[(TT + lx) * PGM_TB_PK + kx];
+            const uint32_t rep = X.p_u[ly * PGM_TB_PK + ky] | X.p_u[(TT + lx) * PGM_TB_PK + kx];
             const bool inside = yp >= ty0 && xp >= tx0;
             if (__builtin_amdgcn_ballot_w64(valid && !inside) != 0ull) continue;
-            const float4 c0 = T.cell[ci];
-            const float S = T.S[ci];
-            const float4 c = T.cell[(valid && inside) ? (yp - ty0) * TT + (xp - tx0) : ci];
+            const float4 c0 = X.cell[ci];
+            const float S = X.S[ci];
+            const float4 c = X.cell[(valid && inside) ? (yp - ty0) * TT + (xp - tx0) : ci];
             const float d = fabsf(__fsub_rn(c0.x, __fsub_rn(__fsub_rn(__fadd_rn(c.z, S), yv), xv)));
             const unsigned long long zero = __builtin_amdgcn_ballot_w64(valid && d == 0.0f);
             if (zero == 0ull) continue;
@@ -673,8 +702,9 @@
                 else if (c.z == c.x) st = 0u;
                 else if (c.z == c.w) st = 2u;
                 else if (c.z == c.y) st = 1u;
-                if (st != 3u) T.succ[ci] = (uint16_t)(0x8000u | (st << 10) | ((yp - ty0) << 5) | (xp - tx0));
-            }
+                if (st != 3u) X.succ[ci] = (uint16_t)(0x8000u | (st << 10) | ((yp - ty0) << 5) | (xp - tx0));
+            }
+        }
         }
     };
     const bool use_links = true;
@@ -696,17 +726,24 @@
         for (uint32_t r = 0; r < PGM_LK_NR; ++r)
             if (r < cnt) {
 #pragma unroll
-                for (uint32_t q = 0; q < PER; ++q) ((unsigned long long *)T.gtab[(gy - r) % PGM_LK_NR])[(uint32_t)tid + NT * q] = v[r][q];
+                for (uint32_t q = 0; q < PER; ++q) ((unsigned long long *)T.u.gtab[(gy - r) % PGM_LK_NR])[(uint32_t)tid + NT * q] = v[r][q];
             }
         if (k < PGM_LK_NR) T.gnext[k] = nx;
+    };
+    const uint32_t margin = J.has_extras ? 4u : 1u;
+    auto request = [&](uint32_t y, uint32_t x) {
+        const uint32_t ty0 = y >= TT - 1 ? y - (TT - 1) : 0u, tx0 = x >= TT - 1 ? x - (TT - 1) : 0u;
+        T.t0.ty0 = ty0; T.t0.tx0 = tx0;
+        const bool two = J.lrows == 0u && ty0 != 0u && tx0 != 0u;
+        T.two = two ? 1u : 0u;
+        if (two) { T.u.t1.ty0 = ty0 > TT - margin ? ty0 - (TT - margin) : 0u; T.u.t1.tx0 = tx0 > TT - margin ? tx0 - (TT - margin) : 0u; }
+        T.req = 1;
     };
     if (tid == 0) {
         T.grow = 0xFFFFFFFFu; T.gcnt = 0u;
         if (J.lrows != 0u) __hip_atomic_store(J.lready + J.lrows + 1, (int)(J.lrows - 1u), __ATOMIC_RELAXED, __HIP_MEMORY_SCOPE_AGENT);
-        T.ty0 = n1 - 2 >= TT - 1 ? n1 - 2 - (TT - 1) : 0u;
-        T.tx0 = n2 - 2 >= TT - 1 ? n2 - 2 - (TT - 1) : 0u;
         T.ay = n1 - 2; T.ax = n2 - 2;
-        T.req = 1;
+        request(n1 - 2, n2 - 2);
         if (J.lrows != 0u && lq) {
             const int slot = __hip_atomic_fetch_add(lq, 1, __ATOMIC_RELAXED, __HIP_MEMORY_SCOPE_AGENT);
             __hip_atomic_store(lq_ids + slot, (int)(jid + 1u), __ATOMIC_RELEASE, __HIP_MEMORY_SCOPE_AGENT);
@@ -739,30 +776,34 @@
     } else {
         const int lane = tid;
         const pgm_scores s = J.sc;
-        uint32_t ty0 = T.ty0, tx0 = T.tx0, ay = T.ay, ax = T.ax;
+        const uint32_t t1_off = (uint32_t)((char *)&T.u.t1 - (char *)&T.t0);
+        uint32_t toff = 0u;
+        auto Cur = [&]() -> PgmTbTile * { return (PgmTbTile *)((char *)&T.t0 + toff); };
+        uint32_t ty0 = T.t0.ty0, tx0 = T.t0.tx0, ay = T.ay, ax = T.ax;
         int adiag = (int)(ay - ty0) - (int)(ax - tx0);
+        bool two = T.two != 0u;
         auto in_tile = [&](uint32_t y, uint32_t x) { return (y - ty0) < TT && (x - tx0) < TT; };
         auto cell_at = [&](uint32_t y, uint32_t x) -> float4 {
-            if (in_tile(y, x)) return T.cell[(y - ty0) * TT + (x - tx0)];
+            if (in_tile(y, x)) return Cur()->cell[(y - ty0) * TT + (x - tx0)];
             return pgm_load_cell(J, y, x);
         };
         auto s_at = [&](uint32_t y, uint32_t x) -> float {
-            if (in_tile(y, x)) return T.S[(y - ty0) * TT + (x - tx0)];
+            if (in_tile(y, x)) return Cur()->S[(y - ty0) * TT + (x - tx0)];
             return pgm_emission_at(J, y, x);
         };
         auto preds = [&](bool row, uint32_t v) -> PgmPredView {
             const uint32_t slot = row ? v - ty0 : (v - tx0) + TT;
             if ((row ? v - ty0 : v - tx0) < TT) {
-                const uint32_t cnt = T.p_cnt[slot];
+                const uint32_t cnt = Cur()->p_cnt[slot];
                 if (cnt <= PGM_TB_PK) return PgmPredView{cnt, true, slot * PGM_TB_PK};
             }
             const PgmPred &P = row ? P1 : P2;
             const int32_t eb = P.pp[v];
             return PgmPredView{(uint32_t)(P.pp[v + 1] - eb), false, (uint32_t)eb};
         };
-        auto pc_of = [&](bool row, const PgmPredView &V, uint32_t k) { return V.lds ? T.p_c[V.base + k] : (row ? P1 : P2).pc[V.base + k]; };
-        auto pv_of = [&](bool row, const PgmPredView &V, uint32_t k) { return V.lds ? T.p_v[V.base + k] : (row ? P1 : P2).pv[V.base + k]; };
-        auto pu_of = [&](bool row, const PgmPredView &V, uint32_t k) { return V.lds ? T.p_u[V.base + k] : (row ? P1 : P2).pu[V.base + k]; };
+        auto pc_of = [&](bool row, const PgmPredView &V, uint32_t k) { return V.lds ? Cur()->p_c[V.base + k] : (row ? P1 : P2).pc[V.base + k]; };
+        auto pv_of = [&](bool row, const PgmPredView &V, uint32_t k) { return V.lds ? Cur()->p_v[V.base + k] : (row ? P1 : P2).pv[V.base + k]; };
+        auto pu_of = [&](bool row, const PgmPredView &V, uint32_t k) { return V.lds ? Cur()->p_u[V.base + k] : (row ? P1 : P2).pu[V.base + k]; };
 
         int status = PGM_OK;
         uint32_t n_tr = 0;
@@ -836,7 +877,20 @@
             if (lane == 0) T.mbuf[nbuf] = make_uint2(a, b2);
             if (++nbuf == 64u) buf_flush();
         };
-        const uint32_t margin = J.has_extras ? 4u : 1u;
+        auto buf_push_run = [&](uint32_t r, uint32_t a, uint32_t b2) {
+            if (nbuf + r > 64u) buf_flush();
+            if ((uint32_t)lane < r) T.mbuf[nbuf + (uint32_t)lane] = make_uint2(a, b2);
+            nbuf += r;
+            if (nbuf == 64u) buf_flush();
+        };
+        uint32_t wc_tile = 1u, wc_saved = 0u, wc_run = 0u, wc_rows = 0u;
+        const bool runs = J.lrows == 0u;
+        bool run_hint = runs;
+        auto leaves = [&](uint32_t oy, uint32_t ox, int diag) {
+            const int offb = ((int)(y - oy) - (int)(x - ox)) - diag;
+            return ((y - oy) >= TT || ((y - oy) < margin && oy != 0)) || ((x - ox) >= TT || ((x - ox) < margin && ox != 0)) ||
+                   (use_links && (offb < -band || offb > band) && (y != ay || x != ax));
+        };
         uint32_t guard = 0;
         bool score_stale = false;
         uint32_t nl_y = 0xFFFFFFFFu, nl_x = 0xFFFFFFFFu;
@@ -846,9 +900,17 @@
             if (++guard > n1 + n2 + 4) { status = PGM_ERR_BACKTRACK; break; }
             y = __builtin_amdgcn_readfirstlane(y); x = __builtin_amdgcn_readfirstlane(x);
             current_state = __builtin_amdgcn_readfirstlane(current_state);
-            const int offb = ((int)(y - ty0) - (int)(x - tx0)) - adiag;
-            const bool reload = ((y - ty0) >= TT || ((y - ty0) < margin && ty0 != 0)) || ((x - tx0) >= TT || ((x - tx0) < margin && tx0 != 0)) ||
-                                (use_links && (offb < -band || offb > band) && (y != ay || x != ax));
+            bool reload = leaves(ty0, tx0, adiag);
+            if (reload && two) {
+                two = false;
+                const uint32_t ty1 = T.u.t1.ty0, tx1 = T.u.t1.tx0;
+                const int adiag1 = (int)(ay - ty1) - (int)(ax - tx1);
+                if (!leaves(ty1, tx1, adiag1)) {
+                    toff = t1_off; ty0 = ty1; tx0 = tx1; adiag = adiag1;
+                    ++wc_saved;
+                    reload = false;
+                }
+            }
             bool nolink = false;
             if (reload && J.lrows != 0u && !(y == nl_y && x == nl_x)) {
                 bool moved = false;
@@ -873,12 +935,13 @@
                         __syncthreads();
                         load_rows();
                         __syncthreads();
+                        ++wc_rows;
                         ghi = gy; glo = gy + 1u - cnt;
                         known = 0u;
                         while (known < (uint32_t)PGM_LK_NR && T.gnext[known] != 0u) ++known;
                     }
                     bool left_row = false;
-                    const uint16_t *tab = T.gtab[gy % PGM_LK_NR];
+                    const uint16_t *tab = T.u.gtab[gy % PGM_LK_NR];
                     for (;;) {
                         const uint32_t j = (x >> 5) - first;
                         if (j >= gw) break;
@@ -905,7 +968,10 @@
                 ty0 = y >= TT - 1 ? y - (TT - 1) : 0u;
                 tx0 = x >= TT - 1 ? x - (TT - 1) : 0u;
                 ay = y; ax = x; adiag = (int)(y - ty0) - (int)(x - tx0);
-                if (lane == 0) { T.ty0 = ty0; T.tx0 = tx0; T.ay = y; T.ax = x; T.req = 1; }
+                toff = 0u;
+                two = J.lrows == 0u && ty0 != 0u && tx0 != 0u;
+                if (lane == 0) { T.ay = y; T.ax = x; request(y, x); }
+                ++wc_tile;
                 __syncthreads();
                 stage();
                 __syncthreads();
@@ -920,8 +986,31 @@
                 uint32_t pos = (uint32_t)(current_state == State_m ? 0 : (current_state == State_x ? 1 : 2)) * (TT * TT) + (y - ty0) * TT + (x - tx0);
                 bool moved = false;
                 for (;;) {
-                    const uint32_t code = T.succ[pos];
+                    uint32_t code;
+                    if (!runs) {
+                        code = Cur()->succ[pos];
+                    } else if (pos < TT * TT && run_hint) {
+                        const uint32_t k = (uint32_t)lane;
+                        const bool ex = k < min(pos >> 5, pos & 31u);
+                        const uint32_t pk = ex ? pos - (TT + 1u) * k : pos;
+                        const uint32_t ck = Cur()->succ[pk];
+                        const uint32_t ny = ty0 + (pk >> 5) - 1u, nx = tx0 + (pk & 31u) - 1u;
+                        const bool plain = ex && ck == (0x8000u | (pk - (TT + 1u))) && (ny | nx) != 0u;
+                        const uint32_t r = (uint32_t)__builtin_amdgcn_readfirstlane(__ffsll((long long)__builtin_amdgcn_ballot_w64(!plain)) - 1);
+                        if (r != 0u) {
+                            buf_push_run(r, ny, nx);
+                            pos -= (TT + 1u) * r;
+                            if (r > 1u) wc_run += r;
+                            moved = true;
+                            run_hint = false;
+                            continue;
+                        }
+                        code = (uint32_t)__builtin_amdgcn_readfirstlane((int)ck);
+                    } else {
+                        code = (uint32_t)__builtin_amdgcn_readfirstlane((int)Cur()->succ[pos]);
+                    }
                     if (!(code & 0x8000u)) break;
+                    if (runs) run_hint = pos >= TT + 1u && code == (0x8000u | (pos - (TT + 1u)));
                     pos = code & 0xfffu;
                     moved = true;
                     const uint32_t ny = ty0 + ((pos >> 5) & 31u), nx = tx0 + (pos & 31u), st = pos >> 10;
@@ -939,21 +1028,21 @@
             }
             if (in_tile(y, x)) {
                 const uint32_t ly = y - ty0, lx = x - tx0, ci = ly * TT + lx;
-                const uint32_t cy = T.p_cnt[ly], cx = T.p_cnt[TT + lx];
+                const uint32_t cy = Cur()->p_cnt[ly], cx = Cur()->p_cnt[TT + lx];
                 const bool in_m = current_state == State_m, in_y = current_state == State_y;
                 if ((in_m || in_y ? cy - 1u < (uint32_t)PGM_TB_PK : true) && (in_m || !in_y ? cx - 1u < (uint32_t)PGM_TB_PK : true)) {
-                    const float4 c0 = T.cell[ci];
-                    const float S0 = T.S[ci];
+                    const float4 c0 = Cur()->cell[ci];
+                    const float S0 = Cur()->S[ci];
                     const uint32_t ka = in_m ? (uint32_t)lane >> 3 : (uint32_t)lane >> 1, kb = in_m ? (uint32_t)lane & 7u : (uint32_t)lane & 1u;
                     const bool valid = in_m ? (ka < cy && kb < cx) : (ka < (in_y ? cy : cx));
                     const uint32_t yi = ly * PGM_TB_PK + (ka & 7u), xi = (TT + lx) * PGM_TB_PK + ((in_m ? kb : ka) & 7u);
                     uint32_t yp = y, xp = x, uu = 0u;
                     float yv = 0.0f, xv = 0.0f;
-                    if (in_m || in_y) { yp = T.p_c[yi]; yv = T.p_v[yi]; uu |= T.p_u[yi]; }
-                    if (in_m || !in_y) { xp = T.p_c[xi]; xv = T.p_v[xi]; uu |= T.p_u[xi]; }
+                    if (in_m || in_y) { yp = Cur()->p_c[yi]; yv = Cur()->p_v[yi]; uu |= Cur()->p_u[yi]; }
+                    if (in_m || !in_y) { xp = Cur()->p_c[xi]; xv = Cur()->p_v[xi]; uu |= Cur()->p_u[xi]; }
                     const bool inside = yp >= ty0 && xp >= tx0;
                     if (__builtin_amdgcn_ballot_w64(valid && !inside) == 0ull) {
-                        const float4 c = T.cell[valid ? (yp - ty0) * TT + (xp - tx0) : ci];
+                        const float4 c = Cur()->cell[valid ? (yp - ty0) * TT + (xp - tx0) : ci];
                         float d;
                         if (in_m) d = fabsf(__fsub_rn(c0.x, __fsub_rn(__fsub_rn(__fadd_rn(c.z, S0), yv), xv)));
                         else if (in_y) d = fabsf(__fsub_rn(c0.w, __fsub_rn(__fadd_rn(kb == 0u ? c.w : c.z, kb == 0u ? s.gap_extend : s.gap_init), yv)));
@@ -1082,6 +1171,7 @@
             J.result->n_tr_indels = n_tr;
             J.result->len = mo.len;
             J.result->status = status;
+            *(uint4 *)J.walk = make_uint4(wc_tile, wc_saved, wc_run, wc_rows);
             T.len = mo.len;
             T.req = 2;
         }
diff --git a/prographmsa_amd/csrc/pgm_capi.hip b/prographmsa_amd/csrc/pgm_capi.hip
--- a/prographmsa_amd/csrc/pgm_capi.hip
+++ b/prographmsa_amd/csrc/pgm_capi.hip
@@ -177,6 +177,7 @@
     uint32_t *d_lean = nullptr;
     PgmItem *d_bands = nullptr;
     int2 *d_tblist = nullptr;
+    uint32_t *d_walk = nullptr;
     unsigned long long *d_times = nullptr;
     int *d_tabhdr = nullptr;
     hipEvent_t ev_fork = nullptr, ev_join = nullptr;
@@ -497,7 +498,7 @@
     if (timed && (e = hipEventRecord(b->ev[4], s)) != hipSuccess) return e;
     return hipSuccess;
 }
-struct SmallLayout { size_t sync, jobs, order, items, lean, tblist, bands, times, tabhdr, total_bands; bool any_lean; };
+struct SmallLayout { size_t sync, jobs, order, items, lean, tblist, bands, times, tabhdr, walk, total_bands; bool any_lean; };
 static SmallLayout layout_small(pgm_align_batch *b) {
     SmallLayout s;
     const uint32_t njobs = b->njobs;
@@ -509,6 +510,7 @@
     s.lean = SM.take(4 * (size_t)std::max(1u, njobs)); s.tblist = SM.take(8 * (size_t)std::max(1u, njobs));
     s.bands = SM.take(sizeof(PgmItem) * std::max<size_t>(1, s.total_bands)); s.times = SM.take(16 * (size_t)std::max(1u, njobs) + 16);
     s.tabhdr = SM.take(s.any_lean ? 4 * (size_t)PGM_TAB_HDR * njobs : 16);
+    s.walk = SM.take(16 * (size_t)std::max(1u, njobs));
     b->small_bytes = SM.bytes;
     return s;
 }
@@ -540,6 +542,7 @@
         b->d_bands = (PgmItem *)(b->d_small + sm.bands);
         b->d_times = (unsigned long long *)(b->d_small + sm.times);
         b->d_tabhdr = sm.any_lean ? (int *)(b->d_small + sm.tabhdr) : nullptr;
+        b->d_walk = (uint32_t *)(b->d_small + sm.walk);
     }
     A->err = e2;
     A->state.store(e2 == hipSuccess ? 1 : -1, std::memory_order_release);
@@ -598,6 +601,7 @@
         J.prog = b->d_sync + o.prog;
         J.ltab = (uint16_t *)(w + o.ltab); J.lready = b->d_sync + o.lready; J.lrows = o.lrows; J.lcols = o.lcols;
         J.times = b->d_times + 2 * (size_t)i;
+        J.walk = b->d_walk + 4 * (size_t)i;
     }
 }
 
@@ -739,6 +743,7 @@
         (e = hipMemcpyAsync(b->d_items, S.items.data(), sizeof(PgmItem) * S.items.size(), hipMemcpyHostToDevice, ctx->stream)) != hipSuccess ||
         (e = hipMemcpyAsync(b->d_lean, S.lean_list.data(), 4 * S.lean_list.size(), hipMemcpyHostToDevice, ctx->stream)) != hipSuccess ||
         (e = hipMemcpyAsync(b->d_bands, S.bands.data(), sizeof(PgmItem) * S.bands.size(), hipMemcpyHostToDevice, ctx->stream)) != hipSuccess ||
+        (e = hipMemsetAsync(b->d_walk, 0, 16 * (size_t)njobs, ctx->stream)) != hipSuccess ||
         (e = classify_lean_jobs(ctx, b)) != hipSuccess ||
         (e = hipStreamSynchronize(ctx->stream)) != hipSuccess)
         return fail(PGM_ERR_DEVICE, std::string("upload: ") + hipGetErrorString(e));
@@ -793,6 +798,14 @@
     HIPCHK(hipSetDevice(ctx->device));
     HIPCHK(hipStreamSynchronize(ctx->stream));
     if (b->njobs) HIPCHK(hipMemcpy(ticks, b->d_times, 16 * (size_t)b->njobs, hipMemcpyDeviceToHost));
+    return PGM_OK;
+}
+
+int pgm_align_batch_walk_stats(pgm_ctx *ctx, pgm_align_batch *b, uint32_t *out) {
+    if (!ctx || !b || !out) return fail(PGM_ERR_INVALID, "null argument");
+    HIPCHK(hipSetDevice(ctx->device));
+    HIPCHK(hipStreamSynchronize(ctx->stream));
+    if (b->njobs) HIPCHK(hipMemcpy(out, b->d_walk, 16 * (size_t)b->njobs, hipMemcpyDeviceToHost));
     return PGM_OK;
 }
 
diff --git a/prographmsa_amd/csrc/pgm_device.h b/prographmsa_amd/csrc/pgm_device.h
--- a/prographmsa_amd/csrc/pgm_device.h
+++ b/prographmsa_amd/csrc/pgm_device.h
@@ -119,6 +119,7 @@
     struct Result { float score; uint32_t n_tr_indels; uint32_t len; int32_t status; } *result;
     uint32_t *hmap1, *hmap2;
     Result *hresult;
+    uint32_t *walk;
 };
 
 
```

Measured after the change: 80.17. 1.3% lower.
